# kmurf1999/RustSolver

Hardware: NVIDIA B200
Metric: cfr_iterations_per_sec (higher is better)
Workload: dtype f32

## Files before the change

### include/b200cfr.h

```cpp
#ifndef B200CFR_H
#define B200CFR_H

#include <stddef.h>
#include <stdint.h>

#ifdef __cplusplus
extern "C" {
#endif

#define RS_OK 0
#define RS_ERR_INVALID -1
#define RS_ERR_CUDA -2
#define RS_ERR_NCCL -3
#define RS_ERR_CAPACITY -4
#define RS_ERR_UNSUPPORTED -5

#define RS_NODE_ACTION 0
#define RS_NODE_TERMINAL 1
#define RS_NODE_PUBLIC_CHANCE 2
#define RS_NODE_PRIVATE_CHANCE 3
#define RS_TERM_ALLIN 0
#define RS_TERM_SHOWDOWN 1
#define RS_TERM_UNCONTESTED 2
#define RS_ROUND_FLOP 0
#define RS_ROUND_TURN 1
#define RS_ROUND_RIVER 2

typedef struct rs_tree {
    uint32_t n_nodes;
    const uint8_t* type;
    const int32_t* parent;
    const uint32_t* child_offset;
    const uint32_t* children;
    const uint8_t* player;
    const uint32_t* an_index;
    const uint8_t* round_idx;
    const uint32_t* value;
    const uint8_t* ttype;
    const uint8_t* last_to_act;
} rs_tree;

typedef struct rs_ranges {
    uint32_t n_hands[2];
    const uint8_t* hands[2];
} rs_ranges;

#define RS_ABS_NONE 0
#define RS_ABS_ISOMORPHIC 1
#define RS_ABS_CLUSTER_ARR 2
#define RS_ABS_BUCKET_TABLE 3
typedef struct rs_round_abstraction {
    uint32_t kind;
    const uint32_t* cluster_arr;
    uint64_t cluster_arr_len;
    const uint32_t* bucket_table[2];
} rs_round_abstraction;
typedef struct rs_abstraction {
    uint32_t n_rounds;
    rs_round_abstraction rounds[3];
} rs_abstraction;

#define RS_NCCL_ID_BYTES 128
typedef struct rs_config {
    uint64_t board_mask;
    int32_t device;
    int32_t rank;
    int32_t world_size;
    uint8_t nccl_id[RS_NCCL_ID_BYTES];
    uint32_t flags;
    uint32_t threads_per_block;
    uint64_t discount_interval;
    uint64_t discount_cap;
} rs_config;
#define RS_FLAG_NO_GRAPH 1u
#define RS_FLAG_NO_CHAIN_SPLIT 2u
#define RS_FLAG_STREET_KERNEL 4u
#define RS_FLAG_SHARD_ISOLATED 8u
#define RS_FLAG_ALL (RS_FLAG_NO_GRAPH | RS_FLAG_NO_CHAIN_SPLIT | RS_FLAG_STREET_KERNEL | RS_FLAG_SHARD_ISOLATED)

typedef struct rs_engine rs_engine;

typedef struct rs_stats {
    uint64_t iterations;
    uint64_t updates_per_iteration;
    uint64_t updates_per_iteration_global;
    double device_ms;
    uint64_t kernel_launches;
    uint64_t table_bytes;
    uint32_t n_rounds;
    uint32_t n_boards[3];
    uint32_t n_boards_local[3];
    uint32_t n_hands[2];
    uint64_t n_combos;
} rs_stats;

const char* rs_last_error(void);
int rs_version(void);
int rs_device_count(void);
int rs_nccl_unique_id(uint8_t* out);

int rs_gpu_index_hands(uint32_t n_board_cards, const uint8_t* cards, size_t n, uint64_t* out, float* kernel_ms);

#define RS_DIST_EMD_1D 0u
#define RS_DIST_L2 1u
int rs_kmeans_assign(const float* points, size_t n, uint32_t dim, const float* centers, uint32_t k, uint32_t dist_kind,
                     uint32_t* cluster, float* min_dist, double* inertia, float* kernel_ms);
int rs_histogram_distances(const float* p, const float* q, size_t n, uint32_t dim, uint32_t dist_kind, float* out);
int rs_kmeans_fit_regular(const float* points, size_t n, uint32_t dim, float* centers, uint32_t k, uint32_t dist_kind,
                          uint32_t rounds, uint32_t* cluster, float* inertia);
int rs_generate_histograms(uint32_t round, uint64_t first_index, size_t count, uint32_t samples, uint32_t bins, uint64_t seed,
                           float* out, uint8_t* cards_out, float* kernel_ms);
int rs_kmeans_fit_growbatch(const float* points, size_t n, uint32_t dim, float* centers, uint32_t k, uint32_t dist_kind,
                            uint32_t initial_batch_size, uint64_t seed, uint32_t* batch_index_out, uint32_t* cluster_out,
                            float* stats_out);
int rs_kmeans_update_min_dists(const float* points, size_t n, uint32_t dim, const float* new_center, uint32_t dist_kind,
                               float* min_dists);
int rs_kmeans_init_pp(const float* points, size_t n, uint32_t dim, uint32_t k, uint32_t dist_kind, uint64_t seed, uint32_t* chosen_out,
                      float* centers_out);
int rs_kmeans_init_random(const float* points, size_t n, uint32_t dim, uint32_t k, uint32_t n_restarts, uint32_t dist_kind, uint64_t seed,
                          uint32_t* chosen_out, float* centers_out);

#define RS_EXCHANGE_HANDLE_BYTES 64
int rs_exchange_export(rs_engine* e, uint8_t* out );
int rs_exchange_import(rs_engine* e, const uint8_t* handles , uint32_t n_ranks);
int rs_exchange_disable(rs_engine* e);


int rs_create(const rs_tree* tree, const rs_ranges* ranges, const rs_abstraction* abs,
              const rs_config* cfg, rs_engine** out);
int rs_create_batch(const rs_tree* tree, const rs_ranges* ranges, const rs_abstraction* abs,
                    const rs_config* cfg, const uint64_t* board_masks, uint32_t n_subgames,
                    rs_engine** out);
void rs_destroy(rs_engine* e);

int rs_iterate(rs_engine* e, uint64_t n_iters);
int rs_iterate_sampled(rs_engine* e, const uint8_t* dealt, uint32_t n_paths);
int rs_sample_runouts(uint64_t seed, uint64_t board_mask, uint32_t n_cards, uint32_t n_paths, int distinct_first, uint8_t* dealt_out);
int rs_discount(rs_engine* e, float d);
int rs_set_wait_timeout_ms(rs_engine* e, uint64_t ms);
int rs_abort(rs_engine* e);
int rs_set_prune_threshold(rs_engine* e, float threshold);
#define RS_OPP_FULL 0u
#define RS_OPP_SAMPLE 1u
#define RS_OPP_SAMPLE_TIMES_SIGMA 2u
int rs_set_opponent_sampling(rs_engine* e, uint32_t mode, uint64_t seed);
#define RS_RULE_VANILLA 0u
#define RS_RULE_DCFR 1u
#define RS_RULE_LCFR 2u
#define RS_RULE_CFR_PLUS 3u
typedef struct rs_update_rule {
    uint32_t kind;
    float alpha, beta, gamma;
} rs_update_rule;
int rs_set_update_rule(rs_engine* e, const rs_update_rule* rule);
int rs_get_update_rule(rs_engine* e, rs_update_rule* out, uint64_t* t_out);
int rs_reset(rs_engine* e);

int rs_read_infoset(rs_engine* e, uint32_t an_index, uint32_t board_id, float* regrets,
                    float* strategy_sum, size_t cap_floats, uint32_t* n_rows_out,
                    uint32_t* n_actions_out);
int rs_write_infoset(rs_engine* e, uint32_t an_index, uint32_t board_id, const float* regrets,
                     const float* strategy_sum, size_t n_floats);
int rs_average_strategy(rs_engine* e, uint32_t an_index, uint32_t board_id, float* out,
                        size_t cap_floats, uint32_t* n_rows_out, uint32_t* n_actions_out);
int rs_current_strategy(rs_engine* e, uint32_t an_index, uint32_t board_id, float* out,
                        size_t cap_floats, uint32_t* n_rows_out, uint32_t* n_actions_out);
int rs_dump_average_strategy(rs_engine* e, const char* path, uint64_t* n_floats_out);

int rs_board_id(rs_engine* e, uint32_t round_idx, const uint8_t* dealt, uint32_t n_dealt,
                uint32_t* board_id_out);
int rs_card_table(rs_engine* e, uint32_t round_idx, uint32_t player, uint32_t board_id,
                  uint16_t* rows_out, size_t cap, uint32_t* n_rows_out);

int rs_best_response(rs_engine* e, double out[2]);
int rs_average_value(rs_engine* e, double out[2]);
int rs_root_values(rs_engine* e, uint32_t player, float* out, size_t cap);

int rs_stats_get(rs_engine* e, rs_stats* out);

int rs_set_range_weights(rs_engine* e, uint32_t player, const float* weights, size_t n);

#define RS_KERNEL_TRAVERSAL 0
#define RS_KERNEL_STREET 1
#define RS_KERNEL_ALLREDUCE 3
typedef struct rs_kernel_time {
    uint32_t kind;
    uint32_t phase;
    uint32_t traverser;
    uint32_t grid;
    float ms;
    uint64_t table_bytes;
    uint64_t vector_bytes;
} rs_kernel_time;
int rs_profile_iteration(rs_engine* e, rs_kernel_time* out, size_t cap, uint32_t* n_out);

int rs_debug_task_timing(rs_engine* e, unsigned long long* out32, int reset);

typedef struct rs_plan rs_plan;
int rs_plan_create(const rs_tree* tree, const rs_ranges* ranges, const rs_abstraction* abs,
                   const rs_config* cfg, const uint64_t* board_masks, uint32_t n_subgames,
                   rs_plan** out);
void rs_plan_destroy(rs_plan* p);
int rs_plan_stats(const rs_plan* p, rs_stats* out);
int rs_plan_board_id(const rs_plan* p, uint32_t round_idx, const uint8_t* dealt, uint32_t n_dealt,
                     uint32_t* board_id_out);
int rs_plan_card_table(const rs_plan* p, uint32_t round_idx, uint32_t player, uint32_t board_id,
                       uint16_t* rows_out, size_t cap, uint32_t* n_rows_out);
int rs_plan_infoset_offset(const rs_plan* p, uint32_t an_index, uint32_t board_id,
                           uint64_t* offset_out, uint32_t* n_rows_out, uint32_t* n_actions_out);
int rs_plan_showdown_order(const rs_plan* p, uint32_t player, uint32_t board_id,
                           uint16_t* order_out, uint32_t* class_out, size_t cap,
                           uint32_t* n_live_out);

int rs_plan_local_tables(const rs_plan* p, uint32_t round_idx, uint32_t player, uint32_t board_id, uint32_t* hrec_words_out,
                         uint16_t* cl_pos_out, uint16_t* slot_of_pos_out, uint32_t dims_out[2]);
int rs_plan_check_execution_order(const rs_plan* p, uint32_t traverser, int force_board_major, uint32_t* n_tickets_out,
                                  uint32_t* n_moved_out);
int rs_plan_street_info(const rs_plan* p, uint32_t traverser, uint32_t out[8]);
int rs_plan_street_program(const rs_plan* p, uint32_t traverser, uint32_t board_id, uint32_t* words_out, size_t cap,
                           uint32_t* n_words_out, uint32_t* hinfo_out, size_t hinfo_cap, uint32_t dims_out[4]);

#ifdef __cplusplus
}
#endif
#endif
```

### rustsolver_b200/_lib.py

```python
from __future__ import annotations

import ctypes as C
import os
from pathlib import Path

_HERE = Path(__file__).resolve().parent
LIB_PATH = Path(os.environ.get("RS_ENGINE_LIB", str(_HERE / "libb200cfr.so")))

u8p = C.POINTER(C.c_uint8)
u16p = C.POINTER(C.c_uint16)
u32p = C.POINTER(C.c_uint32)
u64p = C.POINTER(C.c_uint64)
i32p = C.POINTER(C.c_int32)
f32p = C.POINTER(C.c_float)
f64p = C.POINTER(C.c_double)

RS_NCCL_ID_BYTES = 128
RS_EXCHANGE_HANDLE_BYTES = 64


class rs_tree(C.Structure):
    _fields_ = [("n_nodes", C.c_uint32), ("type", u8p), ("parent", i32p), ("child_offset", u32p),
                ("children", u32p), ("player", u8p), ("an_index", u32p), ("round_idx", u8p),
                ("value", u32p), ("ttype", u8p), ("last_to_act", u8p)]


class rs_ranges(C.Structure):
    _fields_ = [("n_hands", C.c_uint32 * 2), ("hands", u8p * 2)]


class rs_round_abstraction(C.Structure):
    _fields_ = [("kind", C.c_uint32), ("cluster_arr", u32p), ("cluster_arr_len", C.c_uint64),
                ("bucket_table", u32p * 2)]


class rs_abstraction(C.Structure):
    _fields_ = [("n_rounds", C.c_uint32), ("rounds", rs_round_abstraction * 3)]


class rs_config(C.Structure):
    _fields_ = [("board_mask", C.c_uint64), ("device", C.c_int32), ("rank", C.c_int32),
                ("world_size", C.c_int32), ("nccl_id", C.c_uint8 * RS_NCCL_ID_BYTES),
                ("flags", C.c_uint32), ("threads_per_block", C.c_uint32),
                ("discount_interval", C.c_uint64), ("discount_cap", C.c_uint64)]


class rs_stats(C.Structure):
    _fields_ = [("iterations", C.c_uint64), ("updates_per_iteration", C.c_uint64),
                ("updates_per_iteration_global", C.c_uint64), ("device_ms", C.c_double),
                ("kernel_launches", C.c_uint64), ("table_bytes", C.c_uint64), ("n_rounds", C.c_uint32),
                ("n_boards", C.c_uint32 * 3), ("n_boards_local", C.c_uint32 * 3),
                ("n_hands", C.c_uint32 * 2), ("n_combos", C.c_uint64)]


class rs_update_rule(C.Structure):
    _fields_ = [("kind", C.c_uint32), ("alpha", C.c_float), ("beta", C.c_float), ("gamma", C.c_float)]


class rs_kernel_time(C.Structure):
    _fields_ = [("kind", C.c_uint32), ("phase", C.c_uint32), ("traverser", C.c_uint32), ("grid", C.c_uint32),
                ("ms", C.c_float), ("table_bytes", C.c_uint64), ("vector_bytes", C.c_uint64)]


VP = C.c_void_p
ENGINE_API = {
    "rs_last_error": (C.c_char_p, []),
    "rs_version": (C.c_int, []),
    "rs_device_count": (C.c_int, []),
    "rs_nccl_unique_id": (C.c_int, [u8p]),
    "rs_kmeans_assign": (C.c_int, [f32p, C.c_size_t, C.c_uint32, f32p, C.c_uint32, C.c_uint32, u32p, f32p, f64p, f32p]),
    "rs_kmeans_fit_regular": (C.c_int, [f32p, C.c_size_t, C.c_uint32, f32p, C.c_uint32, C.c_uint32, C.c_uint32, u32p, f32p]),
    "rs_histogram_distances": (C.c_int, [f32p, f32p, C.c_size_t, C.c_uint32, C.c_uint32, f32p]),
    "rs_kmeans_update_min_dists": (C.c_int, [f32p, C.c_size_t, C.c_uint32, f32p, C.c_uint32, f32p]),
    "rs_kmeans_init_pp": (C.c_int, [f32p, C.c_size_t, C.c_uint32, C.c_uint32, C.c_uint32, C.c_uint64, u32p, f32p]),
    "rs_generate_histograms": (C.c_int, [C.c_uint32, C.c_uint64, C.c_size_t, C.c_uint32, C.c_uint32, C.c_uint64, f32p, u8p, f32p]),
    "rs_kmeans_fit_growbatch": (C.c_int, [f32p, C.c_size_t, C.c_uint32, f32p, C.c_uint32, C.c_uint32, C.c_uint32, C.c_uint64, u32p, u32p, f32p]),
    "rs_kmeans_init_random": (C.c_int, [f32p, C.c_size_t, C.c_uint32, C.c_uint32, C.c_uint32, C.c_uint32, C.c_uint64, u32p, f32p]),
    "rs_gpu_index_hands": (C.c_int, [C.c_uint32, u8p, C.c_size_t, u64p, f32p]),
    "rs_exchange_export": (C.c_int, [VP, u8p]),
    "rs_exchange_import": (C.c_int, [VP, u8p, C.c_uint32]),
    "rs_exchange_disable": (C.c_int, [VP]),
    "rs_create": (C.c_int, [C.POINTER(rs_tree), C.POINTER(rs_ranges), C.POINTER(rs_abstraction),
                            C.POINTER(rs_config), C.POINTER(VP)]),
    "rs_create_batch": (C.c_int, [C.POINTER(rs_tree), C.POINTER(rs_ranges), C.POINTER(rs_abstraction),
                                  C.POINTER(rs_config), u64p, C.c_uint32, C.POINTER(VP)]),
    "rs_destroy": (None, [VP]),
    "rs_iterate": (C.c_int, [VP, C.c_uint64]),
    "rs_iterate_sampled": (C.c_int, [VP, u8p, C.c_uint32]),
    "rs_discount": (C.c_int, [VP, C.c_float]),
    "rs_set_prune_threshold": (C.c_int, [VP, C.c_float]),
    "rs_set_opponent_sampling": (C.c_int, [VP, C.c_uint32, C.c_uint64]),
    "rs_set_wait_timeout_ms": (C.c_int, [VP, C.c_uint64]),
    "rs_abort": (C.c_int, [VP]),
    "rs_sample_runouts": (C.c_int, [C.c_uint64, C.c_uint64, C.c_uint32, C.c_uint32, C.c_int, u8p]),
    "rs_set_update_rule": (C.c_int, [VP, C.POINTER(rs_update_rule)]),
    "rs_get_update_rule": (C.c_int, [VP, C.POINTER(rs_update_rule), u64p]),
    "rs_reset": (C.c_int, [VP]),
    "rs_read_infoset": (C.c_int, [VP, C.c_uint32, C.c_uint32, f32p, f32p, C.c_size_t, u32p, u32p]),
    "rs_write_infoset": (C.c_int, [VP, C.c_uint32, C.c_uint32, f32p, f32p, C.c_size_t]),
    "rs_average_strategy": (C.c_int, [VP, C.c_uint32, C.c_uint32, f32p, C.c_size_t, u32p, u32p]),
    "rs_dump_average_strategy": (C.c_int, [VP, C.c_char_p, u64p]),
    "rs_current_strategy": (C.c_int, [VP, C.c_uint32, C.c_uint32, f32p, C.c_size_t, u32p, u32p]),
    "rs_board_id": (C.c_int, [VP, C.c_uint32, u8p, C.c_uint32, u32p]),
    "rs_card_table": (C.c_int, [VP, C.c_uint32, C.c_uint32, C.c_uint32, u16p, C.c_size_t, u32p]),
    "rs_best_response": (C.c_int, [VP, f64p]),
    "rs_average_value": (C.c_int, [VP, f64p]),
    "rs_root_values": (C.c_int, [VP, C.c_uint32, f32p, C.c_size_t]),
    "rs_stats_get": (C.c_int, [VP, C.POINTER(rs_stats)]),
    "rs_set_range_weights": (C.c_int, [VP, C.c_uint32, f32p, C.c_size_t]),
    "rs_profile_iteration": (C.c_int, [VP, C.POINTER(rs_kernel_time), C.c_size_t, u32p]),
    "rs_debug_task_timing": (C.c_int, [VP, u64p, C.c_int]),
    "rs_plan_create": (C.c_int, [C.POINTER(rs_tree), C.POINTER(rs_ranges), C.POINTER(rs_abstraction),
                                 C.POINTER(rs_config), u64p, C.c_uint32, C.POINTER(VP)]),
    "rs_plan_destroy": (None, [VP]),
    "rs_plan_stats": (C.c_int, [VP, C.POINTER(rs_stats)]),
    "rs_plan_board_id": (C.c_int, [VP, C.c_uint32, u8p, C.c_uint32, u32p]),
    "rs_plan_card_table": (C.c_int, [VP, C.c_uint32, C.c_uint32, C.c_uint32, u16p, C.c_size_t, u32p]),
    "rs_plan_infoset_offset": (C.c_int, [VP, C.c_uint32, C.c_uint32, u64p, u32p, u32p]),
    "rs_plan_showdown_order": (C.c_int, [VP, C.c_uint32, C.c_uint32, u16p, u32p, C.c_size_t, u32p]),
    "rs_plan_local_tables": (C.c_int, [VP, C.c_uint32, C.c_uint32, C.c_uint32, u32p, u16p, u16p, u32p]),
    "rs_plan_check_execution_order": (C.c_int, [VP, C.c_uint32, C.c_int, u32p, u32p]),
    "rs_plan_street_info": (C.c_int, [VP, C.c_uint32, u32p]),
    "rs_plan_street_program": (C.c_int, [VP, C.c_uint32, C.c_uint32, u32p, C.c_size_t, u32p, u32p, C.c_size_t, u32p]),
}
HOST_API = {
    "rsh_options_default_flop": (VP, []),
    "rsh_options_new": (VP, [C.c_uint64, C.c_uint32, C.c_uint32, C.c_uint32]),
    "rsh_options_free": (None, [VP]),
    "rsh_options_set_sizes": (C.c_int, [VP, C.c_uint32, u32p, f64p, u32p, f64p]),
    "rsh_options_set_range": (C.c_int, [VP, C.c_uint32, C.c_char_p]),
    "rsh_options_set_range_hands": (C.c_int, [VP, C.c_uint32, u8p, C.c_uint32]),
    "rsh_options_board_mask": (C.c_uint64, [VP]),
    "rsh_options_range": (C.c_int, [VP, C.c_uint32, u8p, C.c_size_t]),
    "rsh_build_game_tree": (C.c_int, [VP, C.POINTER(VP)]),
    "rsh_tree_free": (None, [VP]),
    "rsh_tree_n_nodes": (C.c_uint32, [VP]),
    "rsh_tree_n_actions": (C.c_uint32, [VP]),
    "rsh_tree_n_edges": (C.c_uint32, [VP]),
    "rsh_tree_view": (C.c_int, [VP, C.POINTER(rs_tree)]),
    "rsh_tree_round": (u8p, [VP]),
    "rsh_tree_action_kind": (u8p, [VP]),
    "rsh_tree_action_amount": (f64p, [VP]),
    "rsh_evaluate": (C.c_uint32, [u8p, C.c_uint32]),
    "rsh_get_card_mask": (C.c_int, [C.c_char_p, u64p]),
    "rsh_range_from_string": (C.c_int, [C.c_char_p, C.c_uint64, u8p, C.c_size_t]),
    "rsh_indexer_new": (VP, [C.c_uint32, u8p]),
    "rsh_indexer_free": (None, [VP]),
    "rsh_indexer_size": (C.c_uint64, [VP, C.c_uint32]),
    "rsh_indexer_index": (C.c_uint64, [VP, u8p]),
    "rsh_indexer_index_many": (None, [VP, u8p, C.c_size_t, u64p]),
    "rsh_indexer_get_hand": (C.c_int, [VP, C.c_uint32, C.c_uint64, u8p]),
}

_lib = None


def load():
    global _lib
    if _lib is not None:
        return _lib
    if not LIB_PATH.exists():
        raise ImportError(
            f"{LIB_PATH} is missing: build it with `python -m rustsolver_b200.build` "
            "(there is no CPU/Python fallback for the engine)")
    if "RS_NCCL_LIB" not in os.environ:
        try:
            import importlib.util
            spec = importlib.util.find_spec("nvidia.nccl")
            if spec and spec.submodule_search_locations:
                cand = Path(list(spec.submodule_search_locations)[0]) / "lib" / "libnccl.so.2"
                if cand.exists():
                    os.environ["RS_NCCL_LIB"] = str(cand)
        except Exception:
            pass
    lib = C.CDLL(str(LIB_PATH))
    for table in (ENGINE_API, HOST_API):
        for name, (res, args) in table.items():
            fn = getattr(lib, name)
            fn.restype = res
            fn.argtypes = args
    _lib = lib
    return lib


class EngineError(RuntimeError):
    def __init__(self, code: int, msg: str):
        super().__init__(f"b200cfr error {code}: {msg}")
        self.code = code


def check(rc: int):
    if rc != 0:
        raise EngineError(rc, load().rs_last_error().decode())
```

### rustsolver_b200/csrc/engine.cu

```cuda
#include <cuda_runtime.h>
#include <dlfcn.h>

#include <cmath>
#include <cstdio>
#include <cstdlib>
#include <cstring>
#include <map>
#include <memory>
#include <string>
#include <vector>

#include "../../include/b200cfr.h"
#include <cmath>

#include "abstraction_kernels.h"
#include "histogram_kernel.h"
#include "indexer_kernel.h"
#include "kernels.cuh"
#include "plan.h"
#include "street_kernel.cuh"

namespace rs {

thread_local std::string g_last_error;

static int set_err(int code, const std::string& msg) {
    g_last_error = msg;
    return code;
}

namespace nccl {
typedef struct {
    char internal[128];
} UniqueId;
typedef void* Comm;
typedef int (*GetUniqueId_t)(UniqueId*);
typedef int (*CommInitRank_t)(Comm*, int, UniqueId, int);
typedef int (*AllReduce_t)(const void*, void*, size_t, int, int, Comm, cudaStream_t);
typedef int (*CommDestroy_t)(Comm);
typedef const char* (*GetErrorString_t)(int);
struct Api {
    void* lib = nullptr;
    GetUniqueId_t GetUniqueId = nullptr;
    CommInitRank_t CommInitRank = nullptr;
    AllReduce_t AllReduce = nullptr;
    CommDestroy_t CommDestroy = nullptr;
    GetErrorString_t GetErrorString = nullptr;
};
static Api g_api;
constexpr int kFloat32 = 7;
constexpr int kSum = 0;

static bool load(std::string* err) {
    if (g_api.lib) return true;
    const char* env = getenv("RS_NCCL_LIB");
    const char* names[] = {env, "libnccl.so.2", "libnccl.so"};
    void* lib = nullptr;
    for (const char* n : names) {
        if (!n || !*n) continue;
        lib = dlopen(n, RTLD_NOW | RTLD_GLOBAL);
        if (lib) break;
    }
    if (!lib) {
        *err = "cannot dlopen libnccl.so.2 (set RS_NCCL_LIB to its path)";
        return false;
    }
    g_api.lib = lib;
    g_api.GetUniqueId = (GetUniqueId_t)dlsym(lib, "ncclGetUniqueId");
    g_api.CommInitRank = (CommInitRank_t)dlsym(lib, "ncclCommInitRank");
    g_api.AllReduce = (AllReduce_t)dlsym(lib, "ncclAllReduce");
    g_api.CommDestroy = (CommDestroy_t)dlsym(lib, "ncclCommDestroy");
    g_api.GetErrorString = (GetErrorString_t)dlsym(lib, "ncclGetErrorString");
    if (!g_api.GetUniqueId || !g_api.CommInitRank || !g_api.AllReduce || !g_api.CommDestroy) {
        *err = "libnccl is missing expected symbols";
        g_api = Api();
        return false;
    }
    return true;
}
}

#define CU(call)                                                                                   \
    do {                                                                                           \
        cudaError_t e__ = (call);                                                                  \
        if (e__ != cudaSuccess)                                                                    \
            return set_err(RS_ERR_CUDA, std::string(#call) + ": " + cudaGetErrorString(e__));      \
    } while (0)

static bool device_batch_index(const HandIndexer& ix, const uint8_t* cards, size_t n, uint64_t* out, std::string* err) {
    return gpu_index_hands(ix, ix.rounds() - 1, cards, n, out, nullptr, err);
}

template <class T>
struct DevBuf {
    T* p = nullptr;
    size_t n = 0;
    ~DevBuf() {
        if (p) cudaFree(p);
    }
    cudaError_t alloc(size_t count) {
        n = count;
        if (count == 0) count = 1;
        return cudaMalloc(&p, count * sizeof(T));
    }
    cudaError_t upload(const T* src, size_t count) {
        cudaError_t e = alloc(count);
        if (e != cudaSuccess || count == 0) return e;
        return cudaMemcpy(p, src, count * sizeof(T), cudaMemcpyHostToDevice);
    }
    cudaError_t upload(const std::vector<T>& v) { return upload(v.data(), v.size()); }
    cudaError_t zero() { return cudaMemset(p, 0, (n ? n : 1) * sizeof(T)); }
};

struct RoundDev {
    DevBuf<uint16_t> row_of_pos[2], row_start[2], row_pos[2], cl_pos[2], parent_pos[2], child_pos[2], slot_of_pos[2];
    DevBuf<HandRec> hrec[2];
    DevBuf<uint32_t> n_rows[2], n_rows_pad[2], n_live[2];
    DevBuf<uint64_t> board_off[2];
    DevBuf<float> regrets[2], ssum[2];
    DevBuf<float> chance_scale;
    DevBuf<int32_t> parent_board;
    DevBuf<float> rbuf, cbuf, gathered;
    DevBuf<float> sbuf[2];
    uint32_t n_leaves = 0, n_boards = 0;
};

struct TaskSet {
    DevBuf<NodeTask> tasks;
    DevBuf<TaskSrc> srcs;
    DevBuf<uint32_t> tix;
    DevBuf<uint32_t> order;
    uint32_t n_tickets = 0, phase_cut = 0, n_tasks = 0;
    uint32_t street_lo = 0, street_hi = 0;
    uint32_t street_inst = 0;
    struct Run {
        uint32_t t0, t1;
        int threads;
    };
    std::vector<Run> runs;
    uint32_t xch_lo = 0, xch_hi = 0;
    struct Section {
        uint32_t first;
        uint32_t round_k;
        bool up;
    };
    std::vector<Section> sections;
};

struct StreetDev {
    DevBuf<SwSeg> segs;
    DevBuf<SwDown> downs;
    DevBuf<SwUp> ups;
    DevBuf<SwTerm> terms;
    DevBuf<uint32_t> prog, prog_off, l_steps, c_steps, hinfo;
    uint32_t n_segs = 0;
};

struct Engine {
    Plan plan;
    int device = 0;
    int threads = 512;
    cudaStream_t stream = nullptr;
    cudaEvent_t ev0 = nullptr, ev1 = nullptr;
    cudaGraph_t graph = nullptr;
    cudaGraphExec_t graph_exec = nullptr;
    bool use_graph = true;
    nccl::Comm comm = nullptr;
    bool isolated = false;

    RoundDev rd[3];
    DevBuf<float> scratch;
    DevBuf<float> root_weights[2];
    TaskSet full[2];
    std::map<int, std::unique_ptr<TaskSet[]>> sampled_sets;
    DevBuf<int32_t> sample_board[3];
    int sample_cap = 0;
    DevBuf<uint32_t> flags;
    DevBuf<TaskCtl> ctl;
    DevBuf<unsigned long long> timing;
    DevBuf<unsigned char> xch;
    size_t xch_flag_bytes = 0, xch_vectors = 0;
    void* xch_peer_base[RS_MAX_PEERS] = {nullptr};
    bool fused_exchange = false;
    float prune_threshold = -INFINITY;
    int xs_mode = 0;
    uint64_t xs_seed = 0, xs_count = 0;
    uint32_t* abort_host = nullptr;
    uint32_t* abort_dev = nullptr;
    uint64_t wait_timeout_ms = 30000;
    bool aborted = false;
    int check_abort(const char* what);
    int maybe_discount();
    rs_update_rule rule = {RS_RULE_VANILLA, 1.5f, 0.f, 2.f};
    uint64_t rule_t = 0;
    bool rule_on() const { return rule.kind != RS_RULE_VANILLA; }
    int advance_rule();
    uint64_t last_discount_period = 0;
    bool street_on = false;
    StreetDev street[2];
    DevBuf<float> st_scratch;
    size_t st_stride = 0, st_smem = 0;
    int st_XP = 0, st_rows = 0, st_vy_rows = 0, st_vm_rows = 0, st_slots = 0, st_threads = 0, st_blocks_per_sm = 1, st_qs = 1, st_qm = 1;
    int slots = 1;
    size_t smem_bytes = 0;
    size_t smem_small = 0;
    int blocks_per_sm = 1, n_sms = 148;
    int round_threads[3] = {0, 0, 0};
    int bps_small = 0;
    bool wide_for(int thr, uint64_t tickets) const {
        return thr > 288 || bps_small == 0 || getenv("RS_WIDE_ONLY") || (tickets <= uint64_t(n_sms) * blocks_per_sm && !getenv("RS_SMALL_ONLY"));
    }
    std::vector<rs_kernel_time>* prof = nullptr;
    std::vector<std::pair<cudaEvent_t, cudaEvent_t>> prof_events;

    uint64_t iterations = 0;
    double device_ms = 0;
    uint64_t launches = 0;
    uint64_t launches_per_iter = 0;
    uint64_t table_bytes = 0;
    uint64_t updates_global = 0;
    uint64_t discount_interval = 0, discount_cap = 0;

    void close_peers() {
        for (int r = 0; r < RS_MAX_PEERS; ++r) {
            if (xch_peer_base[r] && r != plan.rank) cudaIpcCloseMemHandle(xch_peer_base[r]);
            xch_peer_base[r] = nullptr;
        }
    }

    ~Engine() {
        close_peers();
        if (graph_exec) cudaGraphExecDestroy(graph_exec);
        if (graph) cudaGraphDestroy(graph);
        if (comm && nccl::g_api.CommDestroy) nccl::g_api.CommDestroy(comm);
        if (abort_host) cudaFreeHost(abort_host);
        if (root_stage) cudaFreeHost(root_stage);
        if (ev0) cudaEventDestroy(ev0);
        if (ev1) cudaEventDestroy(ev1);
        if (stream) cudaStreamDestroy(stream);
    }

    int init(const rs_config* cfg);
    void fill_args(TaskArgs* a, int trav, const TaskSet& set) const;
    int materialize(int trav, const uint32_t counts[3], TaskSet* out);
    int enqueue_sampled(int n_paths, int n_paths_global, uint64_t* count);
    int enqueue_traversal(int trav, int mode, uint64_t* count, const TaskSet* set = nullptr, int n_paths = -1, int n_paths_global = 0);
    int init_street();
    int enqueue_street(int trav, int mode, const TaskSet& set, int n_paths);
    int enqueue_iteration(uint64_t* count);
    int iterate(uint64_t n);
    int root_sum(int player, double* out);
    int root_values(int player, std::vector<float>* out);
    int root_values_into(int player, float* dst);
    DevBuf<float> root_out;
    float* root_stage = nullptr;
    size_t root_stage_n = 0;
    int prof_begin();
    int prof_end(uint32_t kind, uint32_t k, int trav, uint32_t grid, uint64_t table_bytes, uint64_t vector_bytes);
};

template <class T>
static std::vector<T> slice(const std::vector<T>& v, size_t lo, size_t hi, size_t stride) {
    if (v.empty()) return {};
    return std::vector<T>(v.begin() + lo * stride, v.begin() + hi * stride);
}

int Engine::init(const rs_config* cfg) {
    int ndev = 0;
    cudaError_t e = cudaGetDeviceCount(&ndev);
    if (e != cudaSuccess || ndev == 0)
        return set_err(RS_ERR_CUDA, std::string("no CUDA device available (the engine has no CPU fallback): ") +
                                        (e != cudaSuccess ? cudaGetErrorString(e) : "device count is 0"));
    device = cfg->device;
    if (device < 0 || device >= ndev) return set_err(RS_ERR_INVALID, "device ordinal out of range");
    CU(cudaSetDevice(device));
    cudaDeviceProp prop;
    CU(cudaGetDeviceProperties(&prop, device));
    if (prop.major < 10) return set_err(RS_ERR_UNSUPPORTED, "kernels are built for sm_100a only; found an older device");
    if (cfg->threads_per_block)
        return set_err(RS_ERR_INVALID, "threads_per_block is derived from the range size (4 hands per thread) and cannot be set");
    if (cfg->flags & ~uint32_t(RS_FLAG_ALL)) return set_err(RS_ERR_INVALID, "unknown bits in rs_config.flags");
    use_graph = !(cfg->flags & RS_FLAG_NO_GRAPH);
    isolated = (cfg->flags & RS_FLAG_SHARD_ISOLATED) != 0;
    discount_interval = cfg->discount_interval;
    discount_cap = cfg->discount_cap;
    CU(cudaStreamCreateWithFlags(&stream, cudaStreamNonBlocking));
    CU(cudaEventCreate(&ev0));
    CU(cudaEventCreate(&ev1));

    const Plan& P = plan;
    for (int q = 0; q < 2; ++q) {
        std::vector<float> ones(P.H[q], 1.0f);
        CU(root_weights[q].upload(ones));
    }
    const int HP[2] = {int((P.H[0] + 3) & ~3u), int((P.H[1] + 3) & ~3u)};
    const size_t maxHP = size_t(std::max(HP[0], HP[1]));
    const bool street_wanted = P.street[0].eligible && P.street[1].eligible;
    threads = int(((maxHP / 4) + 31) / 32 * 32);
    if (threads > MAX_TASK_THREADS) return set_err(RS_ERR_UNSUPPORTED, "range larger than 1326 hands");
    for (uint32_t k = 0; k < P.n_rounds; ++k) {
        round_threads[k] = threads;
        if (!P.board_mask[k].empty() && !getenv("RS_UNIFORM_BLOCK")) {
            const int left = 52 - __builtin_popcountll(P.board_mask[k][0]);
            const size_t live_max = std::min<size_t>(maxHP, size_t(left) * size_t(left - 1) / 2);
            round_threads[k] = std::min(threads, int((((live_max + 3) / 4) + 31) / 32 * 32));
        }
    }
    n_sms = prop.multiProcessorCount;
    if (street_wanted) {
        int rc = init_street();
        if (rc != RS_OK) return rc;
    }
    for (uint32_t k = 0; k < P.n_rounds; ++k) {
        RoundDev& R = rd[k];
        const uint32_t lo = P.local_lo[k], hi = P.local_hi[k], nb = hi - lo;
        R.n_boards = nb;
        R.n_leaves = (k + 1 < P.n_rounds) ? uint32_t(P.segs[k + 1].size()) : 0;
        for (int q = 0; q < 2; ++q) {
            const RoundPlayerTables& T = P.tabs[k][q];
            const LocalTables& L = P.loc[k][q];
            const size_t hp = L.Hpad;
            CU(R.row_of_pos[q].upload(slice(L.row_of_pos, lo, hi, hp)));
            CU(R.row_start[q].upload(slice(L.row_start, lo, hi, hp + 4)));
            CU(R.row_pos[q].upload(slice(L.row_pos, lo, hi, hp)));
            CU(R.cl_pos[q].upload(slice(L.cl_pos, lo, hi, 2 * hp)));
            CU(R.slot_of_pos[q].upload(slice(L.slot_of_pos, lo, hi, hp)));
            {
                std::vector<HandRec> aos = slice(L.hrec, lo, hi, hp);
                std::vector<HandRec> soa(aos.size());
                const uint32_t* src = reinterpret_cast<const uint32_t*>(aos.data());
                uint32_t* dst = reinterpret_cast<uint32_t*>(soa.data());
                for (size_t b = 0; b < size_t(nb); ++b)
                    for (size_t i = 0; i < hp; ++i)
                        for (int wd = 0; wd < 4; ++wd) dst[(b * 4 + wd) * hp + i] = src[(b * hp + i) * 4 + wd];
                CU(R.hrec[q].upload(soa));
            }
            if (k > 0) {
                CU(R.parent_pos[q].upload(slice(L.parent_pos, lo, hi, hp)));
                CU(R.child_pos[q].upload(slice(L.child_pos, lo, hi, size_t(P.loc[k - 1][q].Hpad))));
            }
            CU(R.n_rows[q].upload(slice(T.n_rows, lo, hi, 1)));
            CU(R.n_rows_pad[q].upload(slice(L.n_rows_pad, lo, hi, 1)));
            CU(R.n_live[q].upload(slice(L.n_live, lo, hi, 1)));
            CU(R.board_off[q].upload(slice(T.board_off, lo, hi, 1)));
            const size_t cells = size_t(T.board_off[P.n_boards[k]]);
            CU(R.regrets[q].alloc(cells));
            CU(R.ssum[q].alloc(cells));
            CU(R.regrets[q].zero());
            CU(R.ssum[q].zero());
            table_bytes += 2 * cells * sizeof(float);
        }
        CU(R.chance_scale.upload(slice(P.chance_scale[k], lo, hi, 1)));
        std::vector<int32_t> pb(nb, -1);
        if (k > 0)
            for (uint32_t b = 0; b < nb; ++b) pb[b] = P.board_parent[k][lo + b] - int32_t(P.local_lo[k - 1]);
        CU(R.parent_board.upload(pb));
        const bool fused_round = street_on && k + 1 == P.n_rounds;
        const size_t n_r = fused_round ? 0 : std::max(P.tl[0].n_rbuf[k], P.tl[1].n_rbuf[k]);
        const size_t n_c = (fused_round && k > 0) ? 0 : std::max(P.tl[0].n_cbuf[k], P.tl[1].n_cbuf[k]);
        CU(R.rbuf.alloc(n_r * nb * maxHP));
        CU(R.cbuf.alloc(n_c * nb * maxHP));
        CU(R.gathered.alloc(size_t(R.n_leaves) * nb * maxHP));
        for (int p = 0; p < 2; ++p) {
            CU(R.sbuf[p].alloc(size_t(P.tl[p].n_sbuf[k]) * nb * maxHP));
            CU(R.sbuf[p].zero());
        }
        CU(R.rbuf.zero());
        CU(R.cbuf.zero());
        CU(R.gathered.zero());
    }
    uint32_t max_tickets = 0;
    for (int p = 0; p < 2; ++p) {
        uint32_t counts[3] = {0, 0, 0};
        for (uint32_t k = 0; k < P.n_rounds; ++k) counts[k] = rd[k].n_boards;
        int rc = materialize(p, counts, &full[p]);
        if (rc != RS_OK) return rc;
        max_tickets = std::max(max_tickets, full[p].n_tickets);
        slots = std::max(slots, int(std::max(P.tl[p].max_terminal, 1 + P.tl[p].max_children)));
    }
    CU(timing.alloc(96));
    CU(timing.zero());
    CU(flags.alloc(max_tickets));
    CU(flags.zero());
    {
        TaskCtl c0{};
        c0.ticket = 0;
        c0.exited = 0;
        c0.xch_seq = 1;
        c0.epoch = 1;
        c0.rule[0] = c0.rule[1] = c0.rule[2] = 1.f;
        c0.rule[3] = -INFINITY;
        CU(ctl.upload(&c0, 1));
        CU(cudaHostAlloc(reinterpret_cast<void**>(&abort_host), sizeof(uint32_t), cudaHostAllocMapped));
        *abort_host = 0;
        CU(cudaHostGetDevicePointer(reinterpret_cast<void**>(&abort_dev), abort_host, 0));
    }
    size_t smem_need = std::max(task_kernel_smem_bytes(true, slots, HP[0], HP[1]), task_kernel_smem_bytes(true, slots, HP[1], HP[0]));
    int max_optin = 0;
    CU(cudaDeviceGetAttribute(&max_optin, cudaDevAttrMaxSharedMemoryPerBlockOptin, device));
    if (smem_need > size_t(max_optin))
        return set_err(RS_ERR_UNSUPPORTED, "node too wide for one CTA's shared memory: need " +
                                               std::to_string(smem_need) + " B, device allows " + std::to_string(max_optin));
    smem_bytes = smem_need;
    CU(configure_task_kernels(smem_need, threads, true, &blocks_per_sm));
    if (blocks_per_sm < 1) return set_err(RS_ERR_UNSUPPORTED, "task kernel does not fit on an SM");
    for (uint32_t k = 0; k < P.n_rounds; ++k)
        if (round_threads[k] <= 288 && bps_small == 0) {
            smem_small = std::max(task_kernel_smem_bytes(false, slots, HP[0], HP[1]), task_kernel_smem_bytes(false, slots, HP[1], HP[0]));
            CU(configure_task_kernels(smem_small, 288, false, &bps_small));
            if (bps_small < 1) return set_err(RS_ERR_UNSUPPORTED, "task kernel does not fit on an SM");
        }
    n_sms = prop.multiProcessorCount;
    CU(scratch.alloc(size_t(1326) * MAX_ACTIONS));

    updates_global = P.updates_per_iter_local;
    if (P.world > 1 && !isolated) {
        std::string err;
        if (!nccl::load(&err)) return set_err(RS_ERR_NCCL, err);
        nccl::UniqueId id;
        static_assert(sizeof(id) == RS_NCCL_ID_BYTES, "nccl id size");
        memcpy(&id, cfg->nccl_id, sizeof(id));
        int rc = nccl::g_api.CommInitRank(&comm, P.world, id, P.rank);
        if (rc != 0)
            return set_err(RS_ERR_NCCL, std::string("ncclCommInitRank: ") +
                                            (nccl::g_api.GetErrorString ? nccl::g_api.GetErrorString(rc) : "error"));
        DevBuf<float> tmp;
        CU(tmp.alloc(4));
        uint64_t u = P.updates_per_iter_local;
        if (P.rank > 0)
            for (uint32_t k = 0; k < P.shard_round; ++k)
                for (int q = 0; q < 2; ++q) u -= P.tabs[k][q].board_off[P.n_boards[k]];
        float parts[4] = {float(u & 0xFFFFF), float((u >> 20) & 0xFFFFF), float((u >> 40) & 0xFFFFF), 0.f};
        CU(cudaMemcpy(tmp.p, parts, sizeof(parts), cudaMemcpyHostToDevice));
        rc = nccl::g_api.AllReduce(tmp.p, tmp.p, 4, nccl::kFloat32, nccl::kSum, comm, stream);
        if (rc != 0) return set_err(RS_ERR_NCCL, "ncclAllReduce failed");
        CU(cudaStreamSynchronize(stream));
        CU(cudaMemcpy(parts, tmp.p, sizeof(parts), cudaMemcpyDeviceToHost));
        updates_global = uint64_t(parts[0]) + (uint64_t(parts[1]) << 20) + (uint64_t(parts[2]) << 40);
    }
    if (P.world > 1 && P.shard_round >= 1 && !isolated) {
        const RoundDev& Par = rd[P.shard_round - 1];
        xch_vectors = size_t(Par.n_leaves) * Par.n_boards * size_t(P.world);
        xch_flag_bytes = (2 * xch_vectors * sizeof(uint32_t) + 255) & ~size_t(255);
        CU(xch.alloc(xch_flag_bytes + 2 * xch_vectors * maxHP * sizeof(float)));
        CU(xch.zero());
    }
    CU(cudaDeviceSynchronize());
    return RS_OK;
}


int Engine::init_street() {
    const Plan& P = plan;
    uint32_t max_rows = 1, max_slots = 1, max_q_sd = 1, max_q_mo = 1;
    for (int p = 0; p < 2; ++p) {
        const StreetPlan& S = P.street[p];
        StreetDev& D = street[p];
        CU(D.segs.upload(S.segs));
        CU(D.downs.upload(S.downs));
        CU(D.ups.upload(S.ups));
        CU(D.terms.upload(S.terms));
        CU(D.prog.upload(S.prog));
        CU(D.prog_off.upload(S.prog_off));
        CU(D.l_steps.upload(S.l_steps));
        CU(D.c_steps.upload(S.c_steps));
        CU(D.hinfo.upload(S.hinfo));
        D.n_segs = uint32_t(S.segs.size());
        max_rows = std::max(max_rows, S.max_rows);
        max_slots = std::max(max_slots, S.max_slots);
        max_q_sd = std::max(max_q_sd, S.max_q_sd);
        max_q_mo = std::max(max_q_mo, S.max_q_mo);
    }
    const int HP[2] = {int((P.H[0] + 3) & ~3u), int((P.H[1] + 3) & ~3u)};
    const int HPmax = std::max(HP[0], HP[1]);
    st_XP = (HPmax + 31) & ~31;
    st_rows = int(max_rows);
    st_vy_rows = 4 * int(max_q_sd);
    st_vm_rows = 4 * int(max_q_sd + max_q_mo);
    st_slots = int(max_slots);
    st_stride = size_t(st_rows) * st_XP + size_t(st_vy_rows + st_vm_rows + st_slots) * HPmax;
    st_threads = threads;
    if (const char* e = getenv("RS_STREET_THREADS")) st_threads = std::max(64, std::min(352, atoi(e) / 32 * 32));
    size_t budget = 72 * 1024;
    if (const char* e = getenv("RS_STREET_SMEM_KB")) budget = size_t(std::max(16, atoi(e))) * 1024;
    st_qs = st_qm = 1;
    const int max_q = st_threads / 32;
    while (st_qs < int(max_q_sd) && st_qs < max_q && street_smem_bytes(st_qs + 1, st_qm, HPmax, HPmax) <= budget) ++st_qs;
    while (st_qm < int(max_q_mo) && st_qm < max_q && street_smem_bytes(st_qs, st_qm + 1, HPmax, HPmax) <= budget) ++st_qm;
    st_smem = street_smem_bytes(st_qs, st_qm, HPmax, HPmax);
    int max_optin = 0;
    CU(cudaDeviceGetAttribute(&max_optin, cudaDevAttrMaxSharedMemoryPerBlockOptin, device));
    if (st_smem > size_t(max_optin)) return RS_OK;
    CU(configure_street_kernels(st_smem, st_threads, &st_blocks_per_sm));
    if (st_blocks_per_sm < 1) return RS_OK;
    if (const char* e = getenv("RS_STREET_BLOCKS")) st_blocks_per_sm = std::max(1, std::min(st_blocks_per_sm, atoi(e)));
    CU(st_scratch.alloc(st_stride * size_t(n_sms) * st_blocks_per_sm));
    CU(st_scratch.zero());
    street_on = true;
    return RS_OK;
}

int Engine::enqueue_street(int trav, int mode, const TaskSet& set, int n_paths) {
    const Plan& P = plan;
    const uint32_t k = P.n_rounds - 1;
    const RoundDev& R = rd[k];
    const StreetDev& D = street[trav];
    StreetArgs a;
    memset(&a, 0, sizeof(a));
    for (int q = 0; q < 2; ++q) {
        DevRoundPlayer& d = a.rp[q];
        d.row_of_pos = R.row_of_pos[q].p;
        d.row_start = R.row_start[q].p;
        d.row_pos = R.row_pos[q].p;
        d.cl_pos = R.cl_pos[q].p;
        d.parent_pos = R.parent_pos[q].p;
        d.child_pos = R.child_pos[q].p;
        d.slot_of_pos = R.slot_of_pos[q].p;
        d.hrec = R.hrec[q].p;
        d.n_rows = R.n_rows[q].p;
        d.n_rows_pad = R.n_rows_pad[q].p;
        d.n_live = R.n_live[q].p;
        d.board_off = R.board_off[q].p;
        d.regrets = R.regrets[q].p;
        d.ssum = R.ssum[q].p;
        d.identity = 1;
    }
    a.chance_scale = R.chance_scale.p;
    a.parent_board = R.parent_board.p;
    a.parent_rbuf = k > 0 ? rd[k - 1].rbuf.p : nullptr;
    a.parent_n_boards = k > 0 ? int(rd[k - 1].n_boards) : 0;
    a.n_boards = int(R.n_boards);
    a.root_weights = root_weights[1 - trav].p;
    a.out_buf = k > 0 ? R.sbuf[trav].p : R.cbuf.p;
    a.out_scatter = k > 0 ? 1 : 0;
    a.n_segs = int(D.n_segs);
    a.segs = D.segs.p;
    a.downs = D.downs.p;
    a.ups = D.ups.p;
    a.terms = D.terms.p;
    a.prog = D.prog.p;
    a.prog_off = D.prog_off.p;
    a.l_steps = D.l_steps.p;
    a.c_steps = D.c_steps.p;
    a.hinfo = D.hinfo.p;
    a.scratch = st_scratch.p;
    a.scratch_stride = st_stride;
    a.XP = st_XP;
    a.max_rows = st_rows;
    a.vy_rows = st_vy_rows;
    a.vm_rows = st_vm_rows;
    a.max_slots = st_slots;
    a.qs = st_qs;
    a.qm = st_qm;
    a.trav = trav;
    a.HpP = int((P.H[trav] + 3) & ~3u);
    a.HoP = int((P.H[1 - trav] + 3) & ~3u);
    a.n_units = set.street_inst * D.n_segs;
    a.sample_board = (n_paths >= 0 && k > 0) ? sample_board[k].p : nullptr;
    a.prune_threshold = prune_threshold;
    const int grid = int(std::min<uint64_t>(a.n_units, uint64_t(n_sms) * st_blocks_per_sm));
    CU(launch_street_kernel(a, mode, grid, st_threads, st_smem, stream));
    return RS_OK;
}

int Engine::materialize(int trav, const uint32_t counts[3], TaskSet* out) {
    MaterializedTasks mt;
    materialize_tasks(plan, trav, counts, &mt);
    std::vector<NodeTask>& t = mt.tasks;
    std::vector<TaskSrc>& sr = mt.srcs;
    const uint32_t first = mt.n_tickets;
    out->phase_cut = mt.phase_cut;
    out->n_tickets = first;
    out->n_tasks = uint32_t(t.size());
    out->street_lo = out->street_hi = 0;
    out->street_inst = counts[plan.n_rounds - 1];
    if (street_on) {
        bool seen = false, closed = false;
        for (const NodeTask& x : t) {
            const bool fin = uint32_t(x.round_k) + 1 == plan.n_rounds;
            if (fin && closed) return set_err(RS_ERR_INVALID, "internal: final-round tasks are not contiguous");
            if (fin && !seen) {
                seen = true;
                out->street_lo = x.first;
            }
            if (fin) out->street_hi = x.first + x.count;
            if (!fin && seen) closed = true;
        }
    }
    out->runs.clear();
    out->sections.clear();
    out->xch_lo = out->xch_hi = 0;
    for (const NodeTask& x : t) {
        if (x.count == 0) continue;
        if (x.kind == TK_GATHER && plan.world > 1 && plan.shard_round >= 1 && uint32_t(x.round_k) + 1 == plan.shard_round) {
            if (out->xch_hi == out->xch_lo) out->xch_lo = x.first;
            out->xch_hi = x.first + x.count;
        }
        const int thr = round_threads[x.round_k];
        if (out->runs.empty() || out->runs.back().threads != thr) out->runs.push_back({x.first, x.first + x.count, thr});
        else out->runs.back().t1 = x.first + x.count;
        const bool up = x.kind == TK_UP_TRAV, down = x.kind == TK_DOWN;
        if (up || down) {
            bool seen = false;
            for (const TaskSet::Section& sc : out->sections) seen |= (sc.round_k == x.round_k && sc.up == up);
            if (!seen) out->sections.push_back({x.first, uint32_t(x.round_k), up});
        }
    }
    std::vector<uint32_t> tix(first);
    for (size_t j = 0; j < t.size(); ++j)
        for (uint32_t i = 0; i < t[j].count; ++i) tix[t[j].first + i] = uint32_t(j);
    CU(out->tasks.upload(t));
    CU(out->srcs.upload(sr));
    CU(out->tix.upload(tix));
    if (!getenv("RS_TASK_MAJOR")) {
        std::vector<uint32_t> ord;
        std::string oerr;
        if (!build_execution_order(plan, trav, mt, counts, getenv("RS_BOARD_MAJOR") != nullptr, &ord, &oerr)) return set_err(RS_ERR_INVALID, oerr);
        if (!ord.empty()) CU(out->order.upload(ord));
    }
    return RS_OK;
}

void Engine::fill_args(TaskArgs* a, int trav, const TaskSet& set) const {
    const Plan& P = plan;
    memset(a, 0, sizeof(*a));
    for (int q = 0; q < 2; ++q) {
        a->H[q] = int(P.H[q]);
        a->Hpad[q] = int((P.H[q] + 3) & ~3u);
        a->root_weights[q] = root_weights[q].p;
    }
    for (uint32_t k = 0; k < P.n_rounds; ++k) {
        const RoundDev& R = rd[k];
        RoundArgs& ra = a->rounds[k];
        for (int q = 0; q < 2; ++q) {
            DevRoundPlayer& d = ra.rp[q];
            d.row_of_pos = R.row_of_pos[q].p;
            d.row_start = R.row_start[q].p;
            d.row_pos = R.row_pos[q].p;
            d.cl_pos = R.cl_pos[q].p;
            d.parent_pos = R.parent_pos[q].p;
            d.child_pos = R.child_pos[q].p;
            d.slot_of_pos = R.slot_of_pos[q].p;
            d.hrec = R.hrec[q].p;
            d.n_rows = R.n_rows[q].p;
            d.n_rows_pad = R.n_rows_pad[q].p;
            d.n_live = R.n_live[q].p;
            d.board_off = R.board_off[q].p;
            d.regrets = R.regrets[q].p;
            d.ssum = R.ssum[q].p;
            d.identity = P.loc[k][q].identity ? 1 : 0;
        }
        ra.chance_scale = R.chance_scale.p;
        ra.parent_board = R.parent_board.p;
        ra.rbuf = R.rbuf.p;
        ra.cbuf = R.cbuf.p;
        ra.sbuf = R.sbuf[trav].p;
        ra.gathered = R.gathered.p;
        ra.n_boards = int(R.n_boards);
        ra.board_base = int(P.local_lo[k]);
        if (k + 1 < P.n_rounds) {
            const bool sharded_next = (P.world > 1 && k + 1 == P.shard_round);
            ra.per_parent = sharded_next ? 0 : int(P.deal_count[k + 1]);
            ra.n_boards_next = int(rd[k + 1].n_boards);
        }
    }
    a->tasks = set.tasks.p;
    a->srcs = set.srcs.p;
    a->task_of_ticket = set.tix.p;
    a->order = set.order.n ? set.order.p : nullptr;
    a->n_tasks = set.n_tasks;
    a->flags = flags.p;
    a->ctl = ctl.p;
    a->trav = trav;
    a->HpP = a->Hpad[trav];
    a->HoP = a->Hpad[1 - trav];
    a->Hx = std::max(a->HpP, a->HoP);
    if (fused_exchange) {
        a->xch_world = P.world;
        a->xch_rank = P.rank;
        a->xch_round = int(P.shard_round);
        a->xch_leaves = int(rd[P.shard_round - 1].n_leaves);
        for (int r = 0; r < P.world; ++r) {
            a->xflag_peer[r] = reinterpret_cast<uint32_t*>(xch_peer_base[r]);
            a->xch_peer[r] = reinterpret_cast<float*>(static_cast<unsigned char*>(xch_peer_base[r]) + xch_flag_bytes);
        }
    }
    a->slots = slots;
    a->prune_threshold = prune_threshold;
    a->host_abort = abort_dev;
    a->wait_timeout_ns = wait_timeout_ms * 1000000ull;
    a->timing = timing.p;
}

int Engine::prof_begin() {
    if (!prof) return RS_OK;
    cudaEvent_t a, b;
    CU(cudaEventCreate(&a));
    CU(cudaEventCreate(&b));
    prof_events.emplace_back(a, b);
    CU(cudaEventRecord(a, stream));
    return RS_OK;
}

int Engine::prof_end(uint32_t kind, uint32_t phase, int trav, uint32_t grid, uint64_t tb, uint64_t vb) {
    if (!prof) return RS_OK;
    CU(cudaEventRecord(prof_events.back().second, stream));
    rs_kernel_time t;
    memset(&t, 0, sizeof(t));
    t.kind = kind;
    t.phase = phase;
    t.traverser = uint32_t(trav);
    t.grid = grid;
    t.table_bytes = tb;
    t.vector_bytes = vb;
    prof->push_back(t);
    return RS_OK;
}

int Engine::enqueue_traversal(int trav, int mode, uint64_t* count, const TaskSet* set, int n_paths, int n_paths_global) {
    const Plan& P = plan;
    const TaskList& tl = P.tl[trav];
    if (!set) set = &full[trav];
    TaskArgs a;
    fill_args(&a, trav, *set);
    if (n_paths >= 0) {
        a.n_paths = n_paths;
        for (uint32_t k = 1; k < P.n_rounds; ++k) {
            a.sample_board[k] = sample_board[k].p;
            a.gather_scale[k - 1] = float(P.deal_count[k]) / float(k == 1 ? n_paths_global : 1);
        }
    }
    if (mode == KM_CFR && xs_mode) {
        uint64_t z = xs_seed + 0x9E3779B97F4A7C15ull * (++xs_count);
        z = (z ^ (z >> 30)) * 0xBF58476D1CE4E5B9ull;
        z = (z ^ (z >> 27)) * 0x94D049BB133111EBull;
        a.xs_key = z ^ (z >> 31);
        a.xs_mode = xs_mode;
        mode = KM_CFR_XS;
    }
    if (rule_on() && (mode == KM_CFR || mode == KM_CFR_XS)) mode = mode == KM_CFR ? KM_CFR_DR : KM_CFR_XS_DR;
    int rc;
    struct Step {
        int kind;
        uint32_t t0, t1, phase;
    };
    std::vector<Step> steps;
    const bool use_street = street_on && set->street_hi > set->street_lo;
    uint32_t at = 0;
    if (use_street) {
        if (set->street_lo > 0) steps.push_back({0, 0, set->street_lo, 0});
        steps.push_back({1, 0, 0, 0});
        at = set->street_hi;
    }
    const bool split = !fused_exchange && !isolated && set->phase_cut < set->n_tickets;
    const uint32_t cut = split ? std::max(set->phase_cut, at) : set->n_tickets;
    if (cut > at) steps.push_back({0, at, cut, use_street ? 1u : 0u});
    if (split) {
        steps.push_back({2, 0, 0, 0});
        steps.push_back({0, cut, set->n_tickets, 2});
    }
    uint64_t vec = 0;
    for (uint32_t k = 0; k < P.n_rounds; ++k)
        vec += (uint64_t(tl.n_rbuf[k]) * P.H[1 - trav] + uint64_t(tl.n_cbuf[k]) * P.H[trav]) * rd[k].n_boards * 8;
    for (const Step& sp : steps) {
        if ((rc = prof_begin()) != RS_OK) return rc;
        if (sp.kind == 0) {
            struct Piece {
                uint32_t t0, t1;
                int threads;
            };
            std::vector<Piece> pieces;
            for (const TaskSet::Run& r : set->runs) {
                const uint32_t lo = std::max(sp.t0, r.t0), hi = std::min(sp.t1, r.t1);
                if (lo < hi) pieces.push_back({lo, hi, r.threads});
            }
            size_t longest = 0;
            for (size_t i = 1; i < pieces.size(); ++i)
                if (pieces[i].t1 - pieces[i].t0 > pieces[longest].t1 - pieces[longest].t0) longest = i;
            for (size_t i = 0; i < pieces.size(); ++i) {
                if (i > 0 && (rc = prof_begin()) != RS_OK) return rc;
                a.t0 = pieces[i].t0;
                a.t1 = pieces[i].t1;
                a.xch_bump = (fused_exchange && set->xch_lo < set->xch_hi && a.t0 <= set->xch_lo && set->xch_lo < a.t1) ? 1 : 0;
                const int thr = pieces[i].threads;
                const bool wide = wide_for(thr, a.t1 - a.t0);
                const int grid = int(std::min<uint64_t>(uint64_t(a.t1 - a.t0), uint64_t(n_sms) * (wide ? blocks_per_sm : bps_small)));
                CU(launch_task_kernel(a, mode, grid, thr, wide, wide ? smem_bytes : smem_small, stream));
                uint64_t bytes = 0;
                for (const TaskSet::Section& sc : set->sections)
                    if (sc.first >= a.t0 && sc.first < a.t1) {
                        const uint64_t own = P.tabs[sc.round_k][trav].board_off[P.n_boards[sc.round_k]];
                        const uint64_t opp = P.tabs[sc.round_k][1 - trav].board_off[P.n_boards[sc.round_k]];
                        bytes += sc.up ? own * 16 : opp * 4;
                    }
                if ((rc = prof_end(RS_KERNEL_TRAVERSAL, sp.phase + (i == longest ? 0u : 8u), trav, uint32_t(grid), bytes, i == longest ? vec : 0)) != RS_OK)
                    return rc;
                if (i + 1 < pieces.size()) ++*count;
            }
        } else if (sp.kind == 1) {
            if ((rc = enqueue_street(trav, mode, *set, n_paths)) != RS_OK) return rc;
            const uint32_t k = P.n_rounds - 1;
            const uint64_t own = P.tabs[k][trav].board_off[P.n_boards[k]], opp = P.tabs[k][1 - trav].board_off[P.n_boards[k]];
            const uint32_t grid = uint32_t(std::min<uint64_t>(uint64_t(set->street_inst) * street[trav].n_segs, uint64_t(n_sms) * st_blocks_per_sm));
            if ((rc = prof_end(RS_KERNEL_STREET, 0, trav, grid, own * 16 + opp * 4, 0)) != RS_OK) return rc;
        } else {
            RoundDev& Par = rd[P.shard_round - 1];
            const size_t n = size_t(Par.n_leaves) * Par.n_boards * ((P.H[trav] + 3) & ~3u);
            int nrc = nccl::g_api.AllReduce(Par.gathered.p, Par.gathered.p, n, nccl::kFloat32, nccl::kSum, comm, stream);
            if (nrc != 0) return set_err(RS_ERR_NCCL, "ncclAllReduce failed");
            if ((rc = prof_end(RS_KERNEL_ALLREDUCE, 0, trav, 0, 0, n * 4)) != RS_OK) return rc;
        }
        ++*count;
    }
    return RS_OK;
}

int Engine::enqueue_sampled(int n_paths, int n_paths_global, uint64_t* count) {
    auto it = sampled_sets.find(n_paths);
    if (it == sampled_sets.end()) {
        std::unique_ptr<TaskSet[]> sets(new TaskSet[2]);
        for (int p = 0; p < 2; ++p) {
            uint32_t counts[3] = {rd[0].n_boards, uint32_t(n_paths), uint32_t(n_paths)};
            int rc = materialize(p, counts, &sets[p]);
            if (rc != RS_OK) return rc;
        }
        it = sampled_sets.emplace(n_paths, std::move(sets)).first;
    }
    for (int p = 0; p < 2; ++p) {
        int rc = enqueue_traversal(p, KM_CFR, count, &it->second[p], n_paths, n_paths_global);
        if (rc != RS_OK) return rc;
    }
    return RS_OK;
}

int Engine::enqueue_iteration(uint64_t* count) {
    for (int p = 0; p < 2; ++p) {
        int rc = enqueue_traversal(p, KM_CFR, count);
        if (rc != RS_OK) return rc;
    }
    return RS_OK;
}

int Engine::iterate(uint64_t n) {
    CU(cudaSetDevice(device));
    if (n == 0) return RS_OK;
    if (aborted) return set_err(RS_ERR_CUDA, "an earlier traversal was aborted: the tables are partly updated, create a new engine");
    const bool use_graph = this->use_graph && !xs_mode;
    if (use_graph && !graph_exec) {
        uint64_t cnt = 0;
        CU(cudaStreamBeginCapture(stream, cudaStreamCaptureModeThreadLocal));
        int rc = enqueue_iteration(&cnt);
        cudaError_t e = cudaStreamEndCapture(stream, &graph);
        if (rc != RS_OK) return rc;
        if (e != cudaSuccess) return set_err(RS_ERR_CUDA, std::string("graph capture: ") + cudaGetErrorString(e));
        CU(cudaGraphInstantiate(&graph_exec, graph, 0));
        launches_per_iter = cnt;
    }
    CU(cudaEventRecord(ev0, stream));
    for (uint64_t i = 0; i < n; ++i) {
        {
            int rc = advance_rule();
            if (rc != RS_OK) return rc;
        }
        if (use_graph) {
            CU(cudaGraphLaunch(graph_exec, stream));
            launches += launches_per_iter;
        } else {
            uint64_t cnt = 0;
            int rc = enqueue_iteration(&cnt);
            if (rc != RS_OK) return rc;
            launches += cnt;
            launches_per_iter = cnt;
        }
        ++iterations;
        {
            int rc = maybe_discount();
            if (rc != RS_OK) return rc;
        }
    }
    CU(cudaEventRecord(ev1, stream));
    CU(cudaStreamSynchronize(stream));
    float ms = 0.f;
    CU(cudaEventElapsedTime(&ms, ev0, ev1));
    device_ms += ms;
    return check_abort("rs_iterate");
}

static void update_rule_factors(const rs_update_rule& r, uint64_t t, float f[4]) {
    f[0] = f[1] = f[2] = 1.f;
    f[3] = r.kind == RS_RULE_CFR_PLUS ? 0.f : -INFINITY;
    if (t <= 1) return;
    const double s = double(t - 1);
    if (r.kind == RS_RULE_DCFR || r.kind == RS_RULE_LCFR) {
        const bool lin = r.kind == RS_RULE_LCFR;
        const double a = lin ? 1.0 : double(r.alpha), b = lin ? 1.0 : double(r.beta), g = lin ? 1.0 : double(r.gamma);
        f[0] = float(1.0 / (1.0 + std::pow(s, -a)));
        f[1] = float(1.0 / (1.0 + std::pow(s, -b)));
        f[2] = float(std::pow(s / double(t), g));
    } else if (r.kind == RS_RULE_CFR_PLUS) {
        f[2] = float(s / double(t));
    }
}

int Engine::advance_rule() {
    if (!rule_on()) return RS_OK;
    float f[4];
    update_rule_factors(rule, ++rule_t, f);
    CU(launch_set_rule(ctl.p, f, stream));
    ++launches;
    return RS_OK;
}

int Engine::maybe_discount() {
    if (!discount_interval) return RS_OK;
    const uint64_t period = iterations / discount_interval;
    if (period == last_discount_period) return RS_OK;
    last_discount_period = period;
    if (discount_cap && iterations > discount_cap) return RS_OK;
    const float pf = float(period);
    const float d = pf / (pf + 1.0f);
    for (uint32_t k = 0; k < plan.n_rounds; ++k)
        for (int q = 0; q < 2; ++q) {
            CU(launch_scale(rd[k].regrets[q].p, rd[k].regrets[q].n, d, stream));
            CU(launch_scale(rd[k].ssum[q].p, rd[k].ssum[q].n, d, stream));
            launches += 2;
        }
    return RS_OK;
}

int Engine::check_abort(const char* what) {
    if (!fused_exchange && !(abort_host && *abort_host)) return RS_OK;
    TaskCtl c;
    CU(cudaMemcpy(&c, ctl.p, sizeof(c), cudaMemcpyDeviceToHost));
    if (!c.abort) return RS_OK;
    aborted = true;
    return set_err(RS_ERR_CUDA, std::string(what) + ": the traversal kernel gave up waiting (" +
                                    ((abort_host && *abort_host) ? "rs_abort was called" : "a wait exceeded the bound of " + std::to_string(wait_timeout_ms) +
                                                                                               " ms: a peer rank did not launch the same traversal") +
                                    "); the tables are partly updated, create a new engine");
}

int Engine::root_values_into(int player, float* dst) {
    const Plan& P = plan;
    const RoundDev& R = rd[0];
    const uint32_t hp = (P.H[player] + 3) & ~3u, H = P.H[player];
    const size_t n = size_t(R.n_boards) * H;
    if (root_out.n < n) CU(root_out.alloc(n));
    if (root_stage_n < n) {
        if (root_stage) cudaFreeHost(root_stage);
        root_stage = nullptr;
        CU(cudaHostAlloc(reinterpret_cast<void**>(&root_stage), n * sizeof(float), cudaHostAllocDefault));
        root_stage_n = n;
    }
    CU(cudaMemsetAsync(root_out.p, 0, n * sizeof(float), stream));
    CU(launch_unpermute(R.cbuf.p + size_t(P.tl[player].root_cbuf) * R.n_boards * hp, R.slot_of_pos[player].p, R.n_live[player].p, root_out.p,
                        R.n_boards, hp, H, stream));
// ... 434 lines not shown
        return z ^ (z >> 31);
    };
    const uint64_t zone = (~0ull / 52ull) * 52ull;
    auto card = [&]() {
        for (;;) {
            const uint64_t z = next();
            if (z < zone) return int(z % 52ull);
        }
    };
    uint64_t firsts = 0;
    for (uint32_t s = 0; s < n_paths; ++s) {
        uint64_t used = board_mask;
        for (uint32_t i = 0; i < n_cards;) {
            const int c = card();
            if (used & (1ull << c)) continue;
            if (i == 0 && distinct_first && (firsts & (1ull << c))) continue;
            if (i == 0) firsts |= 1ull << c;
            used |= 1ull << c;
            dealt_out[size_t(s) * n_cards + i] = uint8_t(c);
            ++i;
        }
    }
    return RS_OK;
}

int rs_discount(rs_engine* e, float d) {
    if (!e) return set_err(RS_ERR_INVALID, "null engine");
    Engine& E = e->e;
    CU(cudaSetDevice(E.device));
    for (uint32_t k = 0; k < E.plan.n_rounds; ++k)
        for (int q = 0; q < 2; ++q) {
            CU(launch_scale(E.rd[k].regrets[q].p, E.rd[k].regrets[q].n, d, E.stream));
            CU(launch_scale(E.rd[k].ssum[q].p, E.rd[k].ssum[q].n, d, E.stream));
        }
    CU(cudaStreamSynchronize(E.stream));
    return RS_OK;
}

int rs_set_update_rule(rs_engine* e, const rs_update_rule* rule) {
    if (!rule) return set_err(RS_ERR_INVALID, "null rule");
    if (rule->kind > RS_RULE_CFR_PLUS)
        return set_err(RS_ERR_INVALID, "kind must be RS_RULE_VANILLA (0), RS_RULE_DCFR (1), RS_RULE_LCFR (2) or RS_RULE_CFR_PLUS (3)");
    if (!std::isfinite(rule->alpha) || !std::isfinite(rule->beta) || !std::isfinite(rule->gamma))
        return set_err(RS_ERR_INVALID, "alpha, beta and gamma must be finite");
    if (!e) return set_err(RS_ERR_INVALID, "null engine");
    Engine& E = e->e;
    if (rule->kind != RS_RULE_VANILLA && E.street_on)
        return set_err(RS_ERR_UNSUPPORTED, "update rules other than RS_RULE_VANILLA are not available with RS_FLAG_STREET_KERNEL");
    CU(cudaSetDevice(E.device));
    CU(cudaStreamSynchronize(E.stream));
    const bool was_on = E.rule_on();
    E.rule = *rule;
    E.rule_t = 0;
    if (was_on != E.rule_on()) {
        if (E.graph_exec) {
            cudaGraphExecDestroy(E.graph_exec);
            E.graph_exec = nullptr;
        }
        if (E.graph) {
            cudaGraphDestroy(E.graph);
            E.graph = nullptr;
        }
    }
    return RS_OK;
}

int rs_get_update_rule(rs_engine* e, rs_update_rule* out, uint64_t* t_out) {
    if (!e) return set_err(RS_ERR_INVALID, "null engine");
    if (out) *out = e->e.rule;
    if (t_out) *t_out = e->e.rule_t;
    return RS_OK;
}

int rs_reset(rs_engine* e) {
    if (!e) return set_err(RS_ERR_INVALID, "null engine");
    Engine& E = e->e;
    CU(cudaSetDevice(E.device));
    for (uint32_t k = 0; k < E.plan.n_rounds; ++k)
        for (int q = 0; q < 2; ++q) {
            CU(E.rd[k].regrets[q].zero());
            CU(E.rd[k].ssum[q].zero());
        }
    E.iterations = 0;
    E.device_ms = 0;
    E.launches = 0;
    E.rule_t = 0;
    return RS_OK;
}

static int locate(const Plan& P, uint32_t an_index, uint32_t board_id, uint32_t* k_out, int* q_out, uint64_t* off,
                  uint32_t* n_rows, uint32_t* n_act) {
    if (an_index >= P.an_to_pnode.size() || P.an_to_pnode[an_index] < 0) return set_err(RS_ERR_INVALID, "unknown ActionNode.index");
    const PNode& n = P.nodes[P.an_to_pnode[an_index]];
    const uint32_t k = n.round_k;
    const int q = n.player;
    if (board_id >= P.n_boards[k]) return set_err(RS_ERR_INVALID, "board_id out of range for the node's round");
    if (board_id < P.local_lo[k] || board_id >= P.local_hi[k]) return set_err(RS_ERR_INVALID, "board is owned by another rank");
    const RoundPlayerTables& T = P.tabs[k][q];
    *k_out = k;
    *q_out = q;
    *n_rows = T.n_rows[board_id];
    *n_act = uint32_t(n.children.size());
    *off = T.board_off[board_id] + uint64_t(P.loc[k][q].n_rows_pad[board_id]) * n.cum_a;
    return RS_OK;
}

int rs_plan_infoset_offset(const rs_plan* p, uint32_t an_index, uint32_t board_id, uint64_t* offset_out,
                           uint32_t* n_rows_out, uint32_t* n_actions_out) {
    if (!p) return set_err(RS_ERR_INVALID, "null plan");
    uint32_t k, nr, na;
    int q;
    uint64_t off;
    int rc = locate(p->p, an_index, board_id, &k, &q, &off, &nr, &na);
    if (rc != RS_OK) return rc;
    if (offset_out) *offset_out = off;
    if (n_rows_out) *n_rows_out = nr;
    if (n_actions_out) *n_actions_out = na;
    return RS_OK;
}

int rs_read_infoset(rs_engine* e, uint32_t an_index, uint32_t board_id, float* regrets, float* strategy_sum,
                    size_t cap_floats, uint32_t* n_rows_out, uint32_t* n_actions_out) {
    if (!e) return set_err(RS_ERR_INVALID, "null engine");
    Engine& E = e->e;
    uint32_t k, nr, na;
    int q;
    uint64_t off;
    int rc = locate(E.plan, an_index, board_id, &k, &q, &off, &nr, &na);
    if (rc != RS_OK) return rc;
    if (n_rows_out) *n_rows_out = nr;
    if (n_actions_out) *n_actions_out = na;
    const size_t n = size_t(nr) * na;
    if ((regrets || strategy_sum) && cap_floats < n) return set_err(RS_ERR_CAPACITY, "output buffer too small");
    CU(cudaSetDevice(E.device));
    if (regrets) CU(cudaMemcpy(regrets, E.rd[k].regrets[q].p + off, n * sizeof(float), cudaMemcpyDeviceToHost));
    if (strategy_sum) CU(cudaMemcpy(strategy_sum, E.rd[k].ssum[q].p + off, n * sizeof(float), cudaMemcpyDeviceToHost));
    return RS_OK;
}

int rs_write_infoset(rs_engine* e, uint32_t an_index, uint32_t board_id, const float* regrets, const float* strategy_sum,
                     size_t n_floats) {
    if (!e) return set_err(RS_ERR_INVALID, "null engine");
    Engine& E = e->e;
    uint32_t k, nr, na;
    int q;
    uint64_t off;
    int rc = locate(E.plan, an_index, board_id, &k, &q, &off, &nr, &na);
    if (rc != RS_OK) return rc;
    const size_t n = size_t(nr) * na;
    if (n_floats != n) return set_err(RS_ERR_INVALID, "slab size mismatch");
    CU(cudaSetDevice(E.device));
    if (regrets) CU(cudaMemcpy(E.rd[k].regrets[q].p + off, regrets, n * sizeof(float), cudaMemcpyHostToDevice));
    if (strategy_sum) CU(cudaMemcpy(E.rd[k].ssum[q].p + off, strategy_sum, n * sizeof(float), cudaMemcpyHostToDevice));
    return RS_OK;
}

static int strategy_impl(rs_engine* e, uint32_t an_index, uint32_t board_id, float* out, size_t cap, uint32_t* n_rows_out,
                         uint32_t* n_actions_out, bool average) {
    if (!e) return set_err(RS_ERR_INVALID, "null engine");
    Engine& E = e->e;
    uint32_t k, nr, na;
    int q;
    uint64_t off;
    int rc = locate(E.plan, an_index, board_id, &k, &q, &off, &nr, &na);
    if (rc != RS_OK) return rc;
    if (n_rows_out) *n_rows_out = nr;
    if (n_actions_out) *n_actions_out = na;
    const size_t n = size_t(nr) * na;
    if (!out) return RS_OK;
    if (cap < n) return set_err(RS_ERR_CAPACITY, "output buffer too small");
    CU(cudaSetDevice(E.device));
    const float* src = (average ? E.rd[k].ssum[q].p : E.rd[k].regrets[q].p) + off;
    CU(launch_normalize(src, E.scratch.p, nr, na, E.stream));
    CU(cudaStreamSynchronize(E.stream));
    CU(cudaMemcpy(out, E.scratch.p, n * sizeof(float), cudaMemcpyDeviceToHost));
    return RS_OK;
}

int rs_average_strategy(rs_engine* e, uint32_t an_index, uint32_t board_id, float* out, size_t cap_floats,
                        uint32_t* n_rows_out, uint32_t* n_actions_out) {
    return strategy_impl(e, an_index, board_id, out, cap_floats, n_rows_out, n_actions_out, true);
}
int rs_current_strategy(rs_engine* e, uint32_t an_index, uint32_t board_id, float* out, size_t cap_floats,
                        uint32_t* n_rows_out, uint32_t* n_actions_out) {
    return strategy_impl(e, an_index, board_id, out, cap_floats, n_rows_out, n_actions_out, false);
}

int rs_dump_average_strategy(rs_engine* e, const char* path, uint64_t* n_floats_out) {
    if (!e || !path) return set_err(RS_ERR_INVALID, "null argument");
    Engine& E = e->e;
    const Plan& P = E.plan;
    FILE* f = fopen(path, "wb");
    if (!f) return set_err(RS_ERR_INVALID, std::string("cannot open ") + path);
    uint64_t total = 0;
    std::vector<float> buf;
    int rc = RS_OK;
    for (uint32_t an = 0; an < P.an_to_pnode.size() && rc == RS_OK; ++an) {
        if (P.an_to_pnode[an] < 0) continue;
        const uint32_t k = P.nodes[P.an_to_pnode[an]].round_k;
        for (uint32_t b = P.local_lo[k]; b < P.local_hi[k]; ++b) {
            uint32_t nr = 0, na = 0;
            if ((rc = strategy_impl(e, an, b, nullptr, 0, &nr, &na, true)) != RS_OK) break;
            buf.resize(size_t(nr) * na);
            if (buf.empty()) continue;
            if ((rc = strategy_impl(e, an, b, buf.data(), buf.size(), &nr, &na, true)) != RS_OK) break;
            if (fwrite(buf.data(), sizeof(float), buf.size(), f) != buf.size()) {
                rc = set_err(RS_ERR_INVALID, std::string("short write to ") + path);
                break;
            }
            total += buf.size();
        }
    }
    fclose(f);
    if (rc == RS_OK && n_floats_out) *n_floats_out = total;
    return rc;
}

static int board_id_impl(const Plan& P, uint32_t round_idx, const uint8_t* dealt, uint32_t n_dealt, uint32_t* out) {
    if (round_idx >= P.n_rounds) return set_err(RS_ERR_INVALID, "round_idx out of range");
    if (n_dealt != round_idx) return set_err(RS_ERR_INVALID, "need exactly round_idx dealt cards");
    if (P.n_sub != 1) return set_err(RS_ERR_UNSUPPORTED, "board lookup by dealt cards needs a single root board; batch boards are their own ids");
    uint32_t id = 0;
    uint64_t mask = P.board_mask[0][0];
    for (uint32_t k = 1; k <= round_idx; ++k) {
        const int c = dealt[k - 1];
        if (c >= 52 || (mask & (1ull << c))) return set_err(RS_ERR_INVALID, "dealt card already on the board");
        const uint32_t idx = uint32_t(__builtin_popcountll(~mask & ((1ull << c) - 1)));
        id = id * P.deal_count[k] + idx;
        mask |= 1ull << c;
    }
    *out = id;
    return RS_OK;
}

int rs_plan_board_id(const rs_plan* p, uint32_t round_idx, const uint8_t* dealt, uint32_t n_dealt, uint32_t* board_id_out) {
    if (!p || !board_id_out) return set_err(RS_ERR_INVALID, "null argument");
    return board_id_impl(p->p, round_idx, dealt, n_dealt, board_id_out);
}
int rs_board_id(rs_engine* e, uint32_t round_idx, const uint8_t* dealt, uint32_t n_dealt, uint32_t* board_id_out) {
    if (!e || !board_id_out) return set_err(RS_ERR_INVALID, "null argument");
    return board_id_impl(e->e.plan, round_idx, dealt, n_dealt, board_id_out);
}

static int card_table_impl(const Plan& P, uint32_t round_idx, uint32_t player, uint32_t board_id, uint16_t* rows_out,
                           size_t cap, uint32_t* n_rows_out) {
    if (round_idx >= P.n_rounds || player > 1) return set_err(RS_ERR_INVALID, "round/player out of range");
    if (board_id >= P.n_boards[round_idx]) return set_err(RS_ERR_INVALID, "board_id out of range");
    if (board_id < P.local_lo[round_idx] || board_id >= P.local_hi[round_idx])
        return set_err(RS_ERR_INVALID, "board is owned by another rank");
    const RoundPlayerTables& T = P.tabs[round_idx][player];
    const uint32_t H = P.H[player];
    if (n_rows_out) *n_rows_out = T.n_rows[board_id];
    if (rows_out) {
        if (cap < H) return set_err(RS_ERR_CAPACITY, "output buffer too small");
        memcpy(rows_out, &T.row_of_hand[size_t(board_id) * H], H * sizeof(uint16_t));
    }
    return RS_OK;
}
int rs_plan_card_table(const rs_plan* p, uint32_t round_idx, uint32_t player, uint32_t board_id, uint16_t* rows_out,
                       size_t cap, uint32_t* n_rows_out) {
    if (!p) return set_err(RS_ERR_INVALID, "null plan");
    return card_table_impl(p->p, round_idx, player, board_id, rows_out, cap, n_rows_out);
}
int rs_card_table(rs_engine* e, uint32_t round_idx, uint32_t player, uint32_t board_id, uint16_t* rows_out, size_t cap,
                  uint32_t* n_rows_out) {
    if (!e) return set_err(RS_ERR_INVALID, "null engine");
    return card_table_impl(e->e.plan, round_idx, player, board_id, rows_out, cap, n_rows_out);
}

int rs_plan_showdown_order(const rs_plan* p, uint32_t player, uint32_t board_id, uint16_t* order_out, uint32_t* class_out,
                           size_t cap, uint32_t* n_live_out) {
    if (!p || player > 1) return set_err(RS_ERR_INVALID, "bad argument");
    const Plan& P = p->p;
    const uint32_t k = P.n_rounds - 1;
    const ShowdownTables& S = P.sd[player];
    if (S.n_live.empty()) return set_err(RS_ERR_INVALID, "tree has no showdown terminals");
    if (board_id >= P.n_boards[k]) return set_err(RS_ERR_INVALID, "board_id out of range");
    const uint32_t H = P.H[player];
    const uint32_t nl = S.n_live[board_id];
    if (n_live_out) *n_live_out = nl;
    if (cap < nl) return set_err(RS_ERR_CAPACITY, "output buffer too small");
    for (uint32_t i = 0; i < nl; ++i) {
        if (order_out) order_out[i] = S.sorted[size_t(board_id) * H + i];
        if (class_out) class_out[i] = S.cls[size_t(board_id) * H + i];
    }
    return RS_OK;
}

int rs_plan_local_tables(const rs_plan* p, uint32_t round_idx, uint32_t player, uint32_t board_id, uint32_t* hrec_words_out, uint16_t* cl_pos_out,
                         uint16_t* slot_of_pos_out, uint32_t dims_out[2]) {
    if (!p || player > 1 || !dims_out) return set_err(RS_ERR_INVALID, "bad argument");
    const Plan& P = p->p;
    if (round_idx >= P.n_rounds || board_id >= P.n_boards[round_idx]) return set_err(RS_ERR_INVALID, "round or board out of range");
    if (board_id < P.local_lo[round_idx] || board_id >= P.local_hi[round_idx]) return set_err(RS_ERR_INVALID, "board belongs to another rank");
    const LocalTables& L = P.loc[round_idx][player];
    dims_out[0] = L.Hpad;
    dims_out[1] = L.n_live[board_id];
    if (hrec_words_out) memcpy(hrec_words_out, &L.hrec[size_t(board_id) * L.Hpad], size_t(L.Hpad) * sizeof(HandRec));
    if (cl_pos_out) memcpy(cl_pos_out, &L.cl_pos[size_t(board_id) * 2 * L.Hpad], size_t(2) * L.Hpad * sizeof(uint16_t));
    if (slot_of_pos_out) memcpy(slot_of_pos_out, &L.slot_of_pos[size_t(board_id) * L.Hpad], size_t(L.Hpad) * sizeof(uint16_t));
    return RS_OK;
}

int rs_plan_check_execution_order(const rs_plan* p, uint32_t traverser, int force_board_major, uint32_t* n_tickets_out, uint32_t* n_moved_out) {
    if (!p || traverser > 1) return set_err(RS_ERR_INVALID, "bad argument");
    const Plan& P = p->p;
    uint32_t counts[3] = {0, 0, 0};
    for (uint32_t k = 0; k < P.n_rounds; ++k) counts[k] = P.boards_local(k);
    MaterializedTasks mt;
    materialize_tasks(P, int(traverser), counts, &mt);
    std::vector<uint32_t> ord;
    std::string err;
    if (!build_execution_order(P, int(traverser), mt, counts, force_board_major > 0, &ord, &err)) return set_err(RS_ERR_INVALID, err);
    if (force_board_major < 0) {
        ord.resize(mt.n_tickets);
        for (uint32_t i = 0; i < mt.n_tickets; ++i) ord[i] = mt.n_tickets - 1 - i;
    }
    err = check_execution_order(P, int(traverser), mt, counts, ord);
    if (!err.empty()) return set_err(RS_ERR_INVALID, "execution order: " + err);
    if (n_tickets_out) *n_tickets_out = mt.n_tickets;
    if (n_moved_out) {
        uint32_t moved = 0;
        for (uint32_t i = 0; i < ord.size(); ++i) moved += ord[i] != i;
        *n_moved_out = moved;
    }
    return RS_OK;
}

int rs_plan_street_info(const rs_plan* p, uint32_t traverser, uint32_t out[8]) {
    if (!p || !out || traverser > 1) return set_err(RS_ERR_INVALID, "bad argument");
    const StreetPlan& S = p->p.street[traverser];
    out[0] = S.eligible ? 1u : 0u;
    out[1] = uint32_t(S.segs.size());
    out[2] = S.max_rows;
    out[3] = S.max_slots;
    out[4] = S.max_q_sd;
    out[5] = S.max_q_mo;
    out[6] = uint32_t(S.downs.size());
    out[7] = uint32_t(S.ups.size());
    if (!S.eligible) g_last_error = S.why;
    return RS_OK;
}

int rs_plan_street_program(const rs_plan* p, uint32_t traverser, uint32_t board_id, uint32_t* words_out, size_t cap,
                           uint32_t* n_words_out, uint32_t* hinfo_out, size_t hinfo_cap, uint32_t dims_out[4]) {
    if (!p || !n_words_out || !dims_out || traverser > 1) return set_err(RS_ERR_INVALID, "bad argument");
    const Plan& P = p->p;
    const StreetPlan& S = P.street[traverser];
    if (!S.eligible) return set_err(RS_ERR_INVALID, "the final round does not run on the street kernel: " + S.why);
    const uint32_t k = P.n_rounds - 1;
    if (board_id < P.local_lo[k] || board_id >= P.local_hi[k]) return set_err(RS_ERR_INVALID, "board is owned by another rank");
    const uint32_t lb = board_id - P.local_lo[k];
    const uint32_t n = S.prog_off[lb + 1] - S.prog_off[lb];
    const uint32_t HpP = P.loc[k][traverser].Hpad;
    *n_words_out = n;
    dims_out[0] = S.l_steps[lb];
    dims_out[1] = S.c_steps[lb];
    dims_out[2] = HpP;
    dims_out[3] = P.loc[k][1 - traverser].Hpad;
    if (words_out) {
        if (cap < n) return set_err(RS_ERR_CAPACITY, "output buffer too small");
        memcpy(words_out, S.prog.data() + S.prog_off[lb], size_t(n) * sizeof(uint32_t));
    }
    if (hinfo_out) {
        if (hinfo_cap < 2 * size_t(HpP)) return set_err(RS_ERR_CAPACITY, "hinfo buffer too small");
        memcpy(hinfo_out, S.hinfo.data() + size_t(lb) * HpP * 2, size_t(HpP) * 2 * sizeof(uint32_t));
    }
    return RS_OK;
}

static int score_impl(rs_engine* e, int mode, double out[2]) {
    if (!e || !out) return set_err(RS_ERR_INVALID, "null argument");
    Engine& E = e->e;
    if (E.aborted) return set_err(RS_ERR_CUDA, "an earlier traversal was aborted: create a new engine");
    CU(cudaSetDevice(E.device));
    for (int p = 0; p < 2; ++p) {
        uint64_t cnt = 0;
        int rc = E.enqueue_traversal(p, mode, &cnt);
        if (rc != RS_OK) return rc;
        CU(cudaStreamSynchronize(E.stream));
        if ((rc = E.check_abort(mode == KM_BR ? "rs_best_response" : "rs_average_value")) != RS_OK) return rc;
        double s = 0;
        rc = E.root_sum(p, &s);
        if (rc != RS_OK) return rc;
        out[p] = s;
    }
    return RS_OK;
}

int rs_best_response(rs_engine* e, double out[2]) { return score_impl(e, KM_BR, out); }
int rs_average_value(rs_engine* e, double out[2]) { return score_impl(e, KM_EVAL, out); }

int rs_root_values(rs_engine* e, uint32_t player, float* out, size_t cap) {
    if (!e || !out || player > 1) return set_err(RS_ERR_INVALID, "bad argument");
    Engine& E = e->e;
    const size_t n = size_t(E.rd[0].n_boards) * E.plan.H[player];
    if (cap < n) return set_err(RS_ERR_CAPACITY, "output buffer too small");
    CU(cudaSetDevice(E.device));
    return E.root_values_into(int(player), out);
}

int rs_set_range_weights(rs_engine* e, uint32_t player, const float* weights, size_t n) {
    if (!e || !weights || player > 1) return set_err(RS_ERR_INVALID, "bad argument");
    Engine& E = e->e;
    if (n != E.plan.H[player]) return set_err(RS_ERR_INVALID, "weights length must equal the range size");
    CU(cudaSetDevice(E.device));
    CU(cudaMemcpyAsync(E.root_weights[player].p, weights, n * sizeof(float), cudaMemcpyHostToDevice, E.stream));
    return RS_OK;
}

int rs_profile_iteration(rs_engine* e, rs_kernel_time* out, size_t cap, uint32_t* n_out) {
    if (!e || !n_out) return set_err(RS_ERR_INVALID, "null argument");
    Engine& E = e->e;
    CU(cudaSetDevice(E.device));
    std::vector<rs_kernel_time> rec;
    int rc = E.advance_rule();
    if (rc != RS_OK) return rc;
    E.prof = &rec;
    uint64_t cnt = 0;
    rc = E.enqueue_iteration(&cnt);
    E.prof = nullptr;
    cudaError_t se = cudaStreamSynchronize(E.stream);
    for (size_t i = 0; i < E.prof_events.size(); ++i) {
        if (rc == RS_OK && se == cudaSuccess && i < rec.size())
            cudaEventElapsedTime(&rec[i].ms, E.prof_events[i].first, E.prof_events[i].second);
        cudaEventDestroy(E.prof_events[i].first);
        cudaEventDestroy(E.prof_events[i].second);
    }
    E.prof_events.clear();
    if (rc != RS_OK) return rc;
    if (se != cudaSuccess) return set_err(RS_ERR_CUDA, cudaGetErrorString(se));
    E.iterations += 1;
    E.launches += cnt;
    *n_out = uint32_t(rec.size());
    if (out) {
        if (cap < rec.size()) return set_err(RS_ERR_CAPACITY, "output buffer too small");
        memcpy(out, rec.data(), rec.size() * sizeof(rs_kernel_time));
    }
    return RS_OK;
}

int rs_debug_task_timing(rs_engine* e, unsigned long long* out32, int reset) {
    if (!e || !out32) return set_err(RS_ERR_INVALID, "null argument");
    Engine& E = e->e;
    CU(cudaSetDevice(E.device));
    CU(cudaStreamSynchronize(E.stream));
    CU(cudaMemcpy(out32, E.timing.p, 96 * sizeof(unsigned long long), cudaMemcpyDeviceToHost));
    if (reset) {
        std::vector<unsigned long long> init(96, 0);
        for (int i = 0; i < 32; ++i) init[32 + 2 * i] = ~0ull;
        CU(cudaMemcpy(E.timing.p, init.data(), 96 * sizeof(unsigned long long), cudaMemcpyHostToDevice));
    }
    return RS_OK;
}

static void fill_stats(const Plan& P, rs_stats* s) {
    memset(s, 0, sizeof(*s));
    s->updates_per_iteration = P.updates_per_iter_local;
    s->updates_per_iteration_global = P.updates_per_iter_global;
    s->n_rounds = P.n_rounds;
    for (uint32_t k = 0; k < P.n_rounds; ++k) {
        s->n_boards[k] = P.n_boards[k];
        s->n_boards_local[k] = P.local_hi[k] - P.local_lo[k];
    }
    s->n_hands[0] = P.H[0];
    s->n_hands[1] = P.H[1];
    s->n_combos = P.n_combos.empty() ? 0 : P.n_combos[0];
}

int rs_plan_stats(const rs_plan* p, rs_stats* out) {
    if (!p || !out) return set_err(RS_ERR_INVALID, "null argument");
    fill_stats(p->p, out);
    return RS_OK;
}

int rs_stats_get(rs_engine* e, rs_stats* out) {
    if (!e || !out) return set_err(RS_ERR_INVALID, "null argument");
    fill_stats(e->e.plan, out);
    out->iterations = e->e.iterations;
    out->device_ms = e->e.device_ms;
    out->kernel_launches = e->e.launches;
    out->table_bytes = e->e.table_bytes;
    out->updates_per_iteration_global = e->e.updates_global;
    return RS_OK;
}

}
```

### rustsolver_b200/csrc/kernels.cu

```cuda
#include "kernels.cuh"

#ifndef RS_MIN_BLOCKS_288
#define RS_MIN_BLOCKS_288 3
#endif
#ifndef RS_MIN_BLOCKS_352
#define RS_MIN_BLOCKS_352 2
#endif

#ifndef RS_POLL_SLEEP_NS
#define RS_POLL_SLEEP_NS 64
#endif

namespace rs {

namespace {

__device__ __forceinline__ uint32_t ld_acquire_u32(const uint32_t* p) {
    uint32_t v;
    asm volatile("ld.acquire.gpu.global.u32 %0, [%1];" : "=r"(v) : "l"(p) : "memory");
    return v;
}
__device__ __forceinline__ uint32_t ld_acquire_sys_u32(const uint32_t* p) {
    uint32_t v;
    asm volatile("ld.acquire.sys.global.u32 %0, [%1];" : "=r"(v) : "l"(p) : "memory");
    return v;
}
__device__ __forceinline__ void st_release_sys_u32(uint32_t* p, uint32_t v) {
    asm volatile("st.release.sys.global.u32 [%0], %1;" ::"l"(p), "r"(v) : "memory");
}
__device__ __forceinline__ void st_release_u32(uint32_t* p, uint32_t v) {
    asm volatile("st.release.gpu.global.u32 [%0], %1;" ::"l"(p), "r"(v) : "memory");
}
__device__ __forceinline__ void prefetch_l2_bulk(const void* p, uint32_t bytes) {
    if (bytes) asm volatile("cp.async.bulk.prefetch.L2.global [%0], %1;" ::"l"(p), "r"(bytes) : "memory");
}
__device__ __forceinline__ float4 ldcg4(const float* p) { return __ldcg(reinterpret_cast<const float4*>(p)); }
__device__ __forceinline__ void stcg4(float* p, float4 v) { __stcg(reinterpret_cast<float4*>(p), v); }
__device__ __forceinline__ float4 f4zero() { return make_float4(0.f, 0.f, 0.f, 0.f); }
__device__ __forceinline__ float4 f4add(float4 a, float4 b) { return make_float4(a.x + b.x, a.y + b.y, a.z + b.z, a.w + b.w); }
__device__ __forceinline__ float f4get(const float4& v, int i) { return i == 0 ? v.x : (i == 1 ? v.y : (i == 2 ? v.z : v.w)); }
__device__ __forceinline__ void f4set(float4& v, int i, float x) {
    if (i == 0) v.x = x;
    else if (i == 1) v.y = x;
    else if (i == 2) v.z = x;
    else v.w = x;
}
__device__ __forceinline__ void unpack4(uint2 u, uint32_t (&o)[4]) {
    o[0] = u.x & 0xffffu;
    o[1] = u.x >> 16;
    o[2] = u.y & 0xffffu;
    o[3] = u.y >> 16;
}

__device__ __forceinline__ void csync(int n_compute) { asm volatile("bar.sync 2, %0;" ::"r"(n_compute) : "memory"); }
__device__ __forceinline__ void hsync(int n_all) { asm volatile("bar.sync 1, %0;" ::"r"(n_all) : "memory"); }

__device__ __forceinline__ void mbar_init(uint64_t* bar, uint32_t count) {
    asm volatile("mbarrier.init.shared::cta.b64 [%0], %1;" ::"r"(uint32_t(__cvta_generic_to_shared(bar))), "r"(count) : "memory");
}
__device__ __forceinline__ void mbar_arrive(uint64_t* bar) {
    asm volatile("mbarrier.arrive.release.cta.shared::cta.b64 _, [%0];" ::"r"(uint32_t(__cvta_generic_to_shared(bar))) : "memory");
}
__device__ __forceinline__ bool mbar_test(uint64_t* bar, uint32_t parity) {
    uint32_t ok;
    asm volatile(
        "{\n\t.reg .pred p;\n\tmbarrier.test_wait.parity.acquire.cta.shared::cta.b64 p, [%1], %2;\n\tselp.u32 %0, 1, 0, p;\n\t}"
        : "=r"(ok)
        : "r"(uint32_t(__cvta_generic_to_shared(bar))), "r"(parity)
        : "memory");
    return ok != 0;
}

__device__ __forceinline__ bool wait_gives_up(const TaskArgs& A, unsigned long long t_start, uint32_t& spins) {
    if ((++spins & 255u) != 0) return false;
    if (*reinterpret_cast<const volatile unsigned int*>(&A.ctl->abort)) return true;
    bool trip = false;
    if ((spins & 4095u) == 0 && A.host_abort && *A.host_abort) trip = true;
    if (A.wait_timeout_ns) {
        unsigned long long now;
        asm volatile("mov.u64 %0, %globaltimer;" : "=l"(now));
        if (now - t_start > A.wait_timeout_ns) trip = true;
    }
    if (trip) atomicExch(&A.ctl->abort, 1u);
    return trip;
}
__device__ __forceinline__ unsigned long long global_ns() {
    unsigned long long now;
    asm volatile("mov.u64 %0, %globaltimer;" : "=l"(now));
    return now;
}

struct Ctx {
    int nc;
    int tid, lane, warp, nwarps;
    int pos4;
    int p, o, Hp, Ho, HpP, HoP, Hx;
};

extern __shared__ __align__(16) float smem_raw[];
#define SM_RS (smem_raw)
#define SM_P (smem_raw + HC)
#define SM_GB (smem_raw + 2 * HC + 4)
#define SM_WSA (smem_raw + 4 * HC + 12)
#define SM_WSB (smem_raw + 4 * HC + 44)
#define SM_B (smem_raw + 4 * HC + 76)
#define SM_WSC (smem_raw + 4 * HC + 140)
#define SM_WSD (smem_raw + 4 * HC + 172)
#define SM_BF (smem_raw + 4 * HC + 204)
#define SM_REC (reinterpret_cast<uint32_t*>(smem_raw + 4 * HC + 268))
#define SM_CL (reinterpret_cast<uint32_t*>(smem_raw + 8 * HC + 268))
#define SM_X (smem_raw + 9 * HC + 268)
constexpr int smem_fixed_floats(int HC) { return 9 * HC + 268; }

template <int HC>
__device__ __forceinline__ void stage_lists_raw(int tid, int HoP, const uint16_t* __restrict__ cl_pos_b) {
    if (8 * tid < 2 * HoP)
        asm volatile("cp.async.cg.shared.global [%0], [%1], 16;" ::"r"(uint32_t(__cvta_generic_to_shared(SM_CL + 4 * tid))), "l"(cl_pos_b + 8 * tid)
                     : "memory");
    asm volatile("cp.async.commit_group;" ::: "memory");
}

template <int HC, bool FOLD>
__device__ __forceinline__ float scan_reach(const Ctx& c, const float* r, const float* rf = nullptr, float* total_f = nullptr) {
    csync(c.nc);
    const int hend = HC >= 4 * MAX_TASK_THREADS ? c.HoP : min(c.HoP, 4 * c.nc);
    float4 x = f4zero();
    float lc = 0.f;
    if (c.pos4 < c.HoP) {
        x = *reinterpret_cast<const float4*>(r + c.pos4);
        if (FOLD) {
            const float4 xf = *reinterpret_cast<const float4*>(rf + c.pos4);
            lc = (xf.x + xf.y) + (xf.z + xf.w);
        }
    }
    float y[8], yf[8];
    uint32_t w[4];
    {
        asm volatile("cp.async.wait_group 0;" ::: "memory");
        uint4 u = make_uint4(0x07ff07ffu, 0x07ff07ffu, 0x07ff07ffu, 0x07ff07ffu);
        if (8 * c.tid < 2 * c.HoP) u = *reinterpret_cast<const uint4*>(SM_CL + 4 * c.tid);
        w[0] = u.x;
        w[1] = u.y;
        w[2] = u.z;
        w[3] = u.w;
#pragma unroll
        for (int i = 0; i < 4; ++i) {
            const uint32_t a = w[i] & CL_POS_MASK, b = (w[i] >> 16) & CL_POS_MASK;
            y[2 * i] = a != CL_POS_NONE ? r[a] : 0.f;
            y[2 * i + 1] = b != CL_POS_NONE ? r[b] : 0.f;
            if (FOLD) {
                yf[2 * i] = a != CL_POS_NONE ? rf[a] : 0.f;
                yf[2 * i + 1] = b != CL_POS_NONE ? rf[b] : 0.f;
            }
        }
    }
    const float la = (x.x + x.y) + (x.z + x.w);
    float lb = 0.f, ld = 0.f;
#pragma unroll
    for (int i = 0; i < 8; ++i) {
        lb += y[i];
        if (FOLD) ld += yf[i];
    }
    float ia = la, ib = lb, ic = lc, id = ld;
#pragma unroll
    for (int d = 1; d < 32; d <<= 1) {
        const float ta = __shfl_up_sync(0xffffffffu, ia, d);
        const float tb = __shfl_up_sync(0xffffffffu, ib, d);
        float tc = 0.f, td = 0.f;
        if (FOLD) {
            tc = __shfl_up_sync(0xffffffffu, ic, d);
            td = __shfl_up_sync(0xffffffffu, id, d);
        }
        if (c.lane >= d) {
            ia += ta;
            ib += tb;
            if (FOLD) {
                ic += tc;
                id += td;
            }
        }
    }
    if (c.lane == 31) {
        SM_WSA[c.warp] = ia;
        SM_WSB[c.warp] = ib;
        if (FOLD) {
            SM_WSC[c.warp] = ic;
            SM_WSD[c.warp] = id;
        }
    }
    csync(c.nc);
    float wa = c.lane < c.nwarps ? SM_WSA[c.lane] : 0.f;
    float wb = c.lane < c.nwarps ? SM_WSB[c.lane] : 0.f;
    float wc = 0.f, wd = 0.f;
    if (FOLD) {
        wc = c.lane < c.nwarps ? SM_WSC[c.lane] : 0.f;
        wd = c.lane < c.nwarps ? SM_WSD[c.lane] : 0.f;
    }
#pragma unroll
    for (int d = 1; d < 16; d <<= 1) {
        const float ta = __shfl_up_sync(0xffffffffu, wa, d);
        const float tb = __shfl_up_sync(0xffffffffu, wb, d);
        float tc = 0.f, td = 0.f;
        if (FOLD) {
            tc = __shfl_up_sync(0xffffffffu, wc, d);
            td = __shfl_up_sync(0xffffffffu, wd, d);
        }
        if (c.lane >= d) {
            wa += ta;
            wb += tb;
            if (FOLD) {
                wc += tc;
                wd += td;
            }
        }
    }
    const float total = __shfl_sync(0xffffffffu, wa, c.nwarps - 1);
    const float total_b = __shfl_sync(0xffffffffu, wb, c.nwarps - 1);
    const float base_a = c.warp > 0 ? __shfl_sync(0xffffffffu, wa, c.warp - 1) : 0.f;
    const float base_b = c.warp > 0 ? __shfl_sync(0xffffffffu, wb, c.warp - 1) : 0.f;
    float ea = base_a + ia - la, eb = base_b + ib - lb;
    float total_d = 0.f, ed = 0.f;
    if (FOLD) {
        *total_f = __shfl_sync(0xffffffffu, wc, c.nwarps - 1);
        total_d = __shfl_sync(0xffffffffu, wd, c.nwarps - 1);
        const float base_d = c.warp > 0 ? __shfl_sync(0xffffffffu, wd, c.warp - 1) : 0.f;
        ed = base_d + id - ld;
    }
    if (c.pos4 < c.HoP) {
        float4 o;
        o.x = ea;
        o.y = ea + x.x;
        o.z = o.y + x.y;
        o.w = o.z + x.z;
        *reinterpret_cast<float4*>(SM_P + c.pos4) = o;
    }
    if (8 * c.tid < 2 * c.HoP) {
        float4 o0, o1;
        o0.x = eb;
        o0.y = o0.x + y[0];
        o0.z = o0.y + y[1];
        o0.w = o0.z + y[2];
        o1.x = o0.w + y[3];
        o1.y = o1.x + y[4];
        o1.z = o1.y + y[5];
        o1.w = o1.z + y[6];
        *reinterpret_cast<float4*>(SM_GB + 8 * c.tid) = o0;
        *reinterpret_cast<float4*>(SM_GB + 8 * c.tid + 4) = o1;
        const uint32_t ord0 = ((w[0] >> 11) & 7u) | (((w[0] >> 27) & 7u) << 3);
        const uint32_t b0 = c.tid == 0 ? 0u : ord0;
        float* bp = SM_B + b0;
        const float ex[8] = {o0.x, o0.y, o0.z, o0.w, o1.x, o1.y, o1.z, o1.w};
#pragma unroll
        for (int i = 0; i < 8; ++i) {
            const bool first = ((w[i >> 1] >> ((i & 1) * 16)) & CL_FIRST) != 0;
            if (first) *bp++ = ex[i];
        }
        if (c.tid == 0) SM_B[ord0] = total_b;
        if (FOLD) {
            float* bf = SM_BF + b0;
            float e = ed;
#pragma unroll
            for (int i = 0; i < 8; ++i) {
                const bool first = ((w[i >> 1] >> ((i & 1) * 16)) & CL_FIRST) != 0;
                if (first) *bf++ = e;
                e += yf[i];
            }
            if (c.tid == 0) SM_BF[ord0] = total_d;
        }
    }
    if (c.tid == 0) {
        SM_P[hend] = total;
        SM_GB[2 * hend] = total_b;
    }
    csync(c.nc);
    return total;
}

template <int HC>
__device__ __forceinline__ void stage_recs(const Ctx& c, const uint32_t* __restrict__ planes) {
    if (c.pos4 < c.HpP) {
#pragma unroll
        for (int w = 0; w < 4; ++w)
            asm volatile("cp.async.cg.shared.global [%0], [%1], 16;" ::"r"(uint32_t(__cvta_generic_to_shared(SM_REC + w * HC + c.pos4))),
                         "l"(planes + size_t(w) * c.HpP + c.pos4)
                         : "memory");
    }
    asm volatile("cp.async.commit_group;" ::: "memory");
}
__device__ __forceinline__ void staged_recs_wait() { asm volatile("cp.async.wait_group 0;" ::: "memory"); }
template <int HC>
__device__ __forceinline__ void staged_recs4(const Ctx& c, uint4 (&rec)[4]) {
    const uint4 w0 = *reinterpret_cast<const uint4*>(SM_REC + c.pos4);
    const uint4 w1 = *reinterpret_cast<const uint4*>(SM_REC + HC + c.pos4);
    const uint4 w2 = *reinterpret_cast<const uint4*>(SM_REC + 2 * HC + c.pos4);
    const uint4 w3 = *reinterpret_cast<const uint4*>(SM_REC + 3 * HC + c.pos4);
    rec[0] = make_uint4(w0.x, w1.x, w2.x, w3.x);
    rec[1] = make_uint4(w0.y, w1.y, w2.y, w3.y);
    rec[2] = make_uint4(w0.z, w1.z, w2.z, w3.z);
    rec[3] = make_uint4(w0.w, w1.w, w2.w, w3.w);
}

__device__ __forceinline__ float ldsb(const float* base, uint32_t byte_off) {
    return *reinterpret_cast<const float*>(reinterpret_cast<const char*>(base) + byte_off);
}
template <int HC>
__device__ __forceinline__ void hand_terms(const Ctx& c, const float* r, float total, const uint4& rec, float& mass, float& sd) {
    const uint32_t k0 = rec.w & 0x1ffu, k1 = (rec.w >> 9) & 0x1ffu, same4 = rec.w >> 18;
    const float g0s = ldsb(SM_B, k0), g0e = ldsb(SM_B + 1, k0), g1s = ldsb(SM_B, k1), g1e = ldsb(SM_B + 1, k1);
    mass = total - (g0e - g0s) - (g1e - g1s) + (same4 != HREC_SAME_NONE ? ldsb(r, same4) : 0.f);
    sd = ldsb(SM_P, rec.x & 0xffffu) + ldsb(SM_P, rec.x >> 16) - total - ldsb(SM_GB, rec.y & 0xffffu) - ldsb(SM_GB, rec.y >> 16) + g0s + g0e -
         ldsb(SM_GB, rec.z & 0xffffu) - ldsb(SM_GB, rec.z >> 16) + g1s + g1e;
}
__device__ __forceinline__ float hand_mass(const float* B, const float* r, float total, const uint4& rec) {
    const uint32_t k0 = rec.w & 0x1ffu, k1 = (rec.w >> 9) & 0x1ffu, same4 = rec.w >> 18;
    return total - (ldsb(B + 1, k0) - ldsb(B, k0)) - (ldsb(B + 1, k1) - ldsb(B, k1)) + (same4 != HREC_SAME_NONE ? ldsb(r, same4) : 0.f);
}

__device__ __forceinline__ float4 load_reach4(const TaskArgs& A, const Ctx& c, const NodeTask& nt, const RoundArgs& Rk, int k, int b) {
    float4 r = f4zero();
    if (c.pos4 >= c.HoP) return r;
    if (nt.r_in == RIN_INITIAL) {
        const uint32_t nl = Rk.rp[c.o].n_live[b];
        uint32_t s[4];
        unpack4(__ldg(reinterpret_cast<const uint2*>(Rk.rp[c.o].slot_of_pos + size_t(b) * c.HoP + c.pos4)), s);
        const float* __restrict__ w = A.root_weights[c.o];
#pragma unroll
        for (int i = 0; i < 4; ++i) f4set(r, i, uint32_t(c.pos4 + i) < nl ? __ldg(w + s[i]) : 0.f);
    } else if (nt.rin_parent_round) {
        const RoundArgs& Rp = A.rounds[k - 1];
        const float* src = Rp.rbuf + (size_t(nt.r_in) * Rp.n_boards + Rk.parent_board[b]) * c.HoP;
        uint32_t pp[4];
        unpack4(__ldg(reinterpret_cast<const uint2*>(Rk.rp[c.o].parent_pos + size_t(b) * c.HoP + c.pos4)), pp);
#pragma unroll
        for (int i = 0; i < 4; ++i) f4set(r, i, pp[i] != 0xffffu ? __ldcg(src + pp[i]) : 0.f);
    } else {
        r = ldcg4(Rk.rbuf + (size_t(nt.r_in) * Rk.n_boards + b) * c.HoP + c.pos4);
    }
    return r;
}

__device__ __forceinline__ float4 child_value4(const TaskArgs& A, const Ctx& c, const RoundArgs& Rk, const TaskChild& ch, int b) {
    float4 v = f4zero();
    if (c.pos4 >= c.HpP) return v;
    for (int s = 0; s < ch.n_src; ++s) {
        const TaskSrc sr = A.srcs[ch.src_first + s];
        const float* base = (sr.kind == SK_CBUF ? Rk.cbuf : Rk.gathered) + (size_t(sr.buf) * Rk.n_boards + b) * c.HpP;
        v = f4add(v, ldcg4(base + c.pos4));
    }
    return v;
}

__device__ __forceinline__ void store_value4(const Ctx& c, const NodeTask& nt, const RoundArgs& Rk, int b, float* out, float4 v) {
    if (!nt.root_scatter) {
        stcg4(out + c.pos4, v);
        return;
    }
    uint32_t pp[4];
    unpack4(__ldg(reinterpret_cast<const uint2*>(Rk.rp[c.p].parent_pos + size_t(b) * c.HpP + c.pos4)), pp);
    if (pp[0] != 0xffffu) __stcg(out + pp[0], v.x);
    if (pp[1] != 0xffffu) __stcg(out + pp[1], v.y);
    if (pp[2] != 0xffffu) __stcg(out + pp[2], v.z);
    if (pp[3] != 0xffffu) __stcg(out + pp[3], v.w);
}
__device__ __forceinline__ void store_value1(const Ctx& c, const NodeTask& nt, const RoundArgs& Rk, int b, float* out, int pos, float v) {
    if (!nt.root_scatter) {
        __stcg(out + pos, v);
        return;
    }
    const uint32_t pp = Rk.rp[c.p].parent_pos[size_t(b) * c.HpP + pos];
    if (pp != 0xffffu) __stcg(out + pp, v);
}

template <int NA>
__device__ __forceinline__ void sigma_row(const float (&g)[4 * NA], int i, float (&sg)[NA]) {
    float norm = 0.f;
#pragma unroll
    for (int a = 0; a < NA; ++a) {
        sg[a] = fmaxf(g[i * NA + a], 0.f);
        norm += sg[a];
    }
    const float inv = __fdividef(1.0f, norm);
#pragma unroll
    for (int a = 0; a < NA; ++a) sg[a] = norm > 0.f ? sg[a] * inv : 1.0f / float(NA);
}

template <int NA>
__device__ __forceinline__ void load_rows(const float* __restrict__ slab, bool identity, int pos4, uint32_t n_rows_pad,
                                          const uint32_t (&rows)[4], float (&g)[4 * NA]) {
    if (identity) {
        if (uint32_t(pos4) < n_rows_pad) {
#pragma unroll
            for (int v = 0; v < NA; ++v) {
                const float4 t = *reinterpret_cast<const float4*>(slab + size_t(pos4) * NA + 4 * v);
                g[4 * v] = t.x;
                g[4 * v + 1] = t.y;
                g[4 * v + 2] = t.z;
                g[4 * v + 3] = t.w;
            }
        } else {
#pragma unroll
            for (int e = 0; e < 4 * NA; ++e) g[e] = 0.f;
        }
    } else {
#pragma unroll
        for (int i = 0; i < 4; ++i)
#pragma unroll
            for (int a = 0; a < NA; ++a) g[i * NA + a] = rows[i] != 0xffffu ? slab[size_t(rows[i]) * NA + a] : 0.f;
    }
}

template <int NA>
__device__ __forceinline__ void xs_pick(const TaskArgs& A, float u, float (&sg)[NA]) {
    int pick = NA - 1;
    bool found = false;
    float cum = 0.f;
#pragma unroll
    for (int a = 0; a + 1 < NA; ++a) {
        cum += sg[a];
        if (!found && u < cum) {
            pick = a;
            found = true;
        }
    }
#pragma unroll
    for (int a = 0; a < NA; ++a) sg[a] = (a == pick) ? (A.xs_mode == 2 ? sg[a] : 1.0f) : 0.f;
}

template <int HC>
__device__ __forceinline__ void down_terminals(const Ctx& c, const NodeTask& nt, const RoundArgs& Rk, int b, int n_act) {
    const uint32_t nl_p = Rk.rp[c.p].n_live[b];
    const float scale = Rk.chance_scale[b];
    int n_fold = 0, n_sd = 0, a_fold = 0, a_sd = 0;
    for (int a = 0; a < n_act; ++a) {
        const int ck = nt.child[a].kind;
        if (ck == CK_FOLD) {
            ++n_fold;
            a_fold = a;
        } else if (ck == CK_SHOWDOWN) {
            ++n_sd;
            a_sd = a;
        }
    }
    float4 acc = f4zero();
    if (n_fold == 1 && n_sd == 1) {
        const bool fold_first = a_fold < a_sd;
        const float* rf = SM_X + (fold_first ? 0 : c.Hx);
        const float* rs = SM_X + (fold_first ? c.Hx : 0);
        float total_f;
        const float total = scan_reach<HC, true>(c, rs, rf, &total_f);
        const float cf = nt.child[a_fold].coef * scale, cs = nt.child[a_sd].coef * scale;
        const float c0 = fold_first ? cf : cs, c1 = fold_first ? cs : cf;
        staged_recs_wait();
        if (c.pos4 < c.HpP) {
            uint4 rec[4];
            staged_recs4<HC>(c, rec);
#pragma unroll
            for (int i = 0; i < 4; ++i) {
                if (uint32_t(c.pos4 + i) < nl_p) {
                    float m_sd, sd;
                    hand_terms<HC>(c, rs, total, rec[i], m_sd, sd);
                    const float m = hand_mass(SM_BF, rf, total_f, rec[i]);
                    const float t0 = fold_first ? m : sd, t1 = fold_first ? sd : m;
                    f4set(acc, i, f4get(acc, i) + c0 * t0);
                    f4set(acc, i, f4get(acc, i) + c1 * t1);
                }
            }
        }
    } else {
        int slot = 0;
        for (int a = 0; a < n_act; ++a) {
            const int ck = nt.child[a].kind;
            if (ck != CK_FOLD && ck != CK_SHOWDOWN) continue;
            const float* r = SM_X + slot * c.Hx;
            ++slot;
            const float cf = nt.child[a].coef * scale;
            const float total = scan_reach<HC, false>(c, r);
            staged_recs_wait();
            if (c.pos4 < c.HpP) {
                uint4 rec[4];
                staged_recs4<HC>(c, rec);
#pragma unroll
                for (int i = 0; i < 4; ++i) {
                    if (uint32_t(c.pos4 + i) < nl_p) {
                        float m, sd;
                        if (ck == CK_FOLD) {
                            m = hand_mass(SM_B, r, total, rec[i]);
                            f4set(acc, i, f4get(acc, i) + cf * m);
                        } else {
                            hand_terms<HC>(c, r, total, rec[i], m, sd);
                            f4set(acc, i, f4get(acc, i) + cf * sd);
                        }
                    }
                }
            }
        }
    }
    if (c.pos4 < c.HpP) stcg4(Rk.cbuf + (size_t(nt.out) * Rk.n_boards + b) * c.HpP + c.pos4, acc);
}

template <int HC, int MODE, int NA, bool XS>
__device__ __forceinline__ void task_down(const TaskArgs& A, const Ctx& c, const NodeTask& nt, const RoundArgs& Rk, int k, int b) {
    const DevRoundPlayer& O = Rk.rp[c.o];
    const uint32_t nrp = O.n_rows_pad[b];
    const float* __restrict__ slab = (MODE == KM_CFR ? O.regrets : O.ssum) + O.board_off[b] + size_t(nrp) * nt.cum_a;
    if (nt.out >= 0) {
        stage_lists_raw<HC>(c.tid, c.HoP, O.cl_pos + size_t(b) * 2 * c.HoP);
        stage_recs<HC>(c, reinterpret_cast<const uint32_t*>(Rk.rp[c.p].hrec) + size_t(b) * 4 * c.HpP);
    }
    const float4 r4 = load_reach4(A, c, nt, Rk, k, b);
    uint32_t rows[4] = {0xffffu, 0xffffu, 0xffffu, 0xffffu};
    if (!O.identity && c.pos4 < c.HoP) unpack4(__ldg(reinterpret_cast<const uint2*>(O.row_of_pos + size_t(b) * c.HoP + c.pos4)), rows);
    float g[4 * NA];
    load_rows<NA>(slab, O.identity != 0, c.pos4, nrp, rows, g);
    float4 v[NA];
    uint32_t xs_slot[4] = {0, 0, 0, 0};
    if (XS && c.pos4 < c.HoP) unpack4(__ldg(reinterpret_cast<const uint2*>(O.slot_of_pos + size_t(b) * c.HoP + c.pos4)), xs_slot);
#pragma unroll
    for (int i = 0; i < 4; ++i) {
        float sg[NA];
        sigma_row<NA>(g, i, sg);
        if (XS) xs_pick<NA>(A, xs_uniform(A.xs_key, nt.an_index, uint32_t(Rk.board_base + b), xs_slot[i]), sg);
        const float r = f4get(r4, i);
#pragma unroll
        for (int a = 0; a < NA; ++a) f4set(v[a], i, r * sg[a]);
    }
    int slot = 0;
#pragma unroll
    for (int a = 0; a < NA; ++a) {
        const int ck = nt.child[a].kind;
        if (c.pos4 < c.HoP) {
            if (ck == CK_FOLD || ck == CK_SHOWDOWN) *reinterpret_cast<float4*>(SM_X + slot * c.Hx + c.pos4) = v[a];
            else if (nt.child[a].buf >= 0) stcg4(Rk.rbuf + (size_t(nt.child[a].buf) * Rk.n_boards + b) * c.HoP + c.pos4, v[a]);
        }
        if (ck == CK_FOLD || ck == CK_SHOWDOWN) ++slot;
    }
    if (nt.out < 0) return;
    down_terminals<HC>(c, nt, Rk, b, NA);
}

template <int HC, int MODE, bool XS>
__device__ __forceinline__ void task_down_generic(const TaskArgs& A, const Ctx& c, const NodeTask& nt, const RoundArgs& Rk, int k, int b) {
    const DevRoundPlayer& O = Rk.rp[c.o];
    const uint32_t nrp = O.n_rows_pad[b];
    const float* __restrict__ slab = (MODE == KM_CFR ? O.regrets : O.ssum) + O.board_off[b] + size_t(nrp) * nt.cum_a;
    const float4 r4 = load_reach4(A, c, nt, Rk, k, b);
    const int n_act = nt.n_act;
    const uint32_t nl_o = O.n_live[b];
    uint32_t rows[4] = {0xffffu, 0xffffu, 0xffffu, 0xffffu};
    if (c.pos4 < c.HoP) unpack4(__ldg(reinterpret_cast<const uint2*>(O.row_of_pos + size_t(b) * c.HoP + c.pos4)), rows);
    if (c.pos4 < c.HoP) {
        for (int i = 0; i < 4; ++i) {
            const bool live = uint32_t(c.pos4 + i) < nl_o && rows[i] != 0xffffu;
            const float r = live ? f4get(r4, i) : 0.f;
            float norm = 0.f;
            if (live)
                for (int a = 0; a < n_act; ++a) norm += fmaxf(slab[size_t(rows[i]) * n_act + a], 0.f);
            int pick = -1;
            if (XS && live) {
                const float u = xs_uniform(A.xs_key, nt.an_index, uint32_t(Rk.board_base + b), O.slot_of_pos[size_t(b) * c.HoP + c.pos4 + i]);
                pick = n_act - 1;
                float cum = 0.f;
                for (int a = 0; a + 1 < n_act; ++a) {
                    cum += norm > 0.f ? fmaxf(slab[size_t(rows[i]) * n_act + a], 0.f) / norm : 1.0f / float(n_act);
                    if (u < cum) {
                        pick = a;
                        break;
                    }
                }
            }
            int slot = 0;
            for (int a = 0; a < n_act; ++a) {
                float v = 0.f;
                if (live) v = norm > 0.f ? r * fmaxf(slab[size_t(rows[i]) * n_act + a], 0.f) / norm : r / float(n_act);
                if (XS && live) v = (a == pick) ? (A.xs_mode == 2 ? v : r) : 0.f;
                const int ck = nt.child[a].kind;
                if (ck == CK_FOLD || ck == CK_SHOWDOWN) SM_X[(slot++) * c.Hx + c.pos4 + i] = v;
                else if (nt.child[a].buf >= 0) __stcg(Rk.rbuf + (size_t(nt.child[a].buf) * Rk.n_boards + b) * c.HoP + c.pos4 + i, v);
            }
        }
    }
    if (nt.out < 0) return;
    stage_lists_raw<HC>(c.tid, c.HoP, O.cl_pos + size_t(b) * 2 * c.HoP);
    stage_recs<HC>(c, reinterpret_cast<const uint32_t*>(Rk.rp[c.p].hrec) + size_t(b) * 4 * c.HpP);
    down_terminals<HC>(c, nt, Rk, b, n_act);
}

template <int HC>
__device__ __forceinline__ void trav_terms(const TaskArgs& A, const Ctx& c, const NodeTask& nt, const RoundArgs& Rk, int k, int b,
                                           bool need_sd, float4& mass, float4& sd) {
    const DevRoundPlayer& Pp = Rk.rp[c.p];
    stage_lists_raw<HC>(c.tid, c.HoP, Rk.rp[c.o].cl_pos + size_t(b) * 2 * c.HoP);
    stage_recs<HC>(c, reinterpret_cast<const uint32_t*>(Pp.hrec) + size_t(b) * 4 * c.HpP);
    const float4 r4 = load_reach4(A, c, nt, Rk, k, b);
    if (c.pos4 < c.HoP) *reinterpret_cast<float4*>(SM_RS + c.pos4) = r4;
    const float total = scan_reach<HC, false>(c, SM_RS);
    mass = f4zero();
    sd = f4zero();
    const uint32_t nl_p = Pp.n_live[b];
    staged_recs_wait();
    if (c.pos4 < c.HpP) {
        uint4 rec[4];
        staged_recs4<HC>(c, rec);
#pragma unroll
        for (int i = 0; i < 4; ++i) {
            if (uint32_t(c.pos4 + i) < nl_p) {
                float m, s = 0.f;
                if (need_sd) hand_terms<HC>(c, SM_RS, total, rec[i], m, s);
                else m = hand_mass(SM_B, SM_RS, total, rec[i]);
                f4set(mass, i, m);
                f4set(sd, i, s);
            }
        }
    }
}

template <int HC>
__device__ __forceinline__ void trav_terms_or_load(const TaskArgs& A, const Ctx& c, const NodeTask& nt, const RoundArgs& Rk, int k, int b,
                                                   bool need_sd, float4& mass, float4& sd) {
    if (!nt.pre_terms) {
        trav_terms<HC>(A, c, nt, Rk, k, b, need_sd, mass, sd);
        return;
    }
    mass = f4zero();
    sd = f4zero();
    if (c.pos4 < c.HpP) {
        const float* m = Rk.cbuf + (size_t(nt.aux) * Rk.n_boards + b) * c.HpP + c.pos4;
        mass = ldcg4(m);
        if (need_sd) sd = ldcg4(m + size_t(Rk.n_boards) * c.HpP);
    }
}

__device__ __forceinline__ float4 rule_factors(const TaskArgs& A) { return ldcg4(A.ctl->rule); }
__device__ __forceinline__ float rule_regret(const float4& f, float r, float d) { return fmaxf((r > 0.f ? f.x : f.y) * r + d, f.w); }

template <int HC, int MODE, int NA, bool DR>
__device__ __forceinline__ void task_trav(const TaskArgs& A, const Ctx& c, const NodeTask& nt, const RoundArgs& Rk, int k, int b) {
    const DevRoundPlayer& Pp = Rk.rp[c.p];
    const float scale = Rk.chance_scale[b];
    float4 dr;
    if (DR) dr = rule_factors(A);
    float4 v[NA];
    bool need_sd = false;
#pragma unroll
    for (int a = 0; a < NA; ++a) {
        v[a] = f4zero();
        need_sd |= (nt.child[a].kind == CK_SHOWDOWN);
    }
    float4 mass, sd;
    trav_terms_or_load<HC>(A, c, nt, Rk, k, b, need_sd, mass, sd);
#pragma unroll
    for (int a = 0; a < NA; ++a)
        if (nt.child[a].kind == CK_VALUE) v[a] = child_value4(A, c, Rk, nt.child[a], b);
#pragma unroll
    for (int a = 0; a < NA; ++a) {
        const int ck = nt.child[a].kind;
        const float cf = nt.child[a].coef * scale;
        if (ck == CK_FOLD) v[a] = make_float4(cf * mass.x, cf * mass.y, cf * mass.z, cf * mass.w);
        else if (ck == CK_SHOWDOWN) v[a] = make_float4(cf * sd.x, cf * sd.y, cf * sd.z, cf * sd.w);
    }
    const uint32_t nrp = Pp.n_rows_pad[b];
    const uint32_t nl_p = Pp.n_live[b];
    float* out = (nt.root_scatter ? Rk.sbuf : Rk.cbuf) + (size_t(nt.out) * Rk.n_boards + b) * c.HpP;
    float* tabR = Pp.regrets + Pp.board_off[b] + size_t(nrp) * nt.cum_a;
    float* tabS = Pp.ssum + Pp.board_off[b] + size_t(nrp) * nt.cum_a;
    if (Pp.identity) {
        if (uint32_t(c.pos4) >= nrp) {
            if (c.pos4 < c.HpP && !nt.root_scatter) stcg4(out + c.pos4, f4zero());
            return;
        }
        const uint32_t none[4] = {0, 0, 0, 0};
        float g[4 * NA], ss[4 * NA];
        if (MODE == KM_CFR) load_rows<NA>(tabR, true, c.pos4, nrp, none, g);
        if (MODE != KM_BR) load_rows<NA>(tabS, true, c.pos4, nrp, none, ss);
        float4 vn4 = f4zero();
#pragma unroll
        for (int i = 0; i < 4; ++i) {
            float sg[NA];
            float vn;
            if (MODE == KM_BR) {
                vn = -3.0e38f;
#pragma unroll
                for (int a = 0; a < NA; ++a) vn = fmaxf(vn, f4get(v[a], i));
            } else {
                if (MODE == KM_CFR) sigma_row<NA>(g, i, sg);
                else sigma_row<NA>(ss, i, sg);
                vn = 0.f;
#pragma unroll
                for (int a = 0; a < NA; ++a) vn += sg[a] * f4get(v[a], i);
            }
            const bool live = uint32_t(c.pos4 + i) < nl_p;
            f4set(vn4, i, live ? vn : 0.f);
            if (MODE == KM_CFR) {
                const float w = f4get(mass, i) * scale;
#pragma unroll
                for (int a = 0; a < NA; ++a) {
                    if (DR) {
                        const float r = g[i * NA + a];
                        if (live) {
                            g[i * NA + a] = rule_regret(dr, r, r > A.prune_threshold ? f4get(v[a], i) - vn : 0.f);
                            ss[i * NA + a] = dr.z * ss[i * NA + a] + sg[a] * w;
                        }
                    } else {
                        g[i * NA + a] += (live && g[i * NA + a] > A.prune_threshold) ? f4get(v[a], i) - vn : 0.f;
                        ss[i * NA + a] += live ? sg[a] * w : 0.f;
                    }
                }
            }
        }
        if (MODE == KM_CFR) {
#pragma unroll
            for (int q = 0; q < NA; ++q) {
                *reinterpret_cast<float4*>(tabR + size_t(c.pos4) * NA + 4 * q) = make_float4(g[4 * q], g[4 * q + 1], g[4 * q + 2], g[4 * q + 3]);
                *reinterpret_cast<float4*>(tabS + size_t(c.pos4) * NA + 4 * q) = make_float4(ss[4 * q], ss[4 * q + 1], ss[4 * q + 2], ss[4 * q + 3]);
            }
        }
        store_value4(c, nt, Rk, b, out, vn4);
        return;
    }
    float* M = SM_X;
    if (c.pos4 < c.HpP) {
        *reinterpret_cast<float4*>(M + c.pos4) = mass;
#pragma unroll
        for (int a = 0; a < NA; ++a) *reinterpret_cast<float4*>(SM_X + (1 + a) * c.Hx + c.pos4) = v[a];
        if (!nt.root_scatter) stcg4(out + c.pos4, f4zero());
    }
    csync(c.nc);
    const uint32_t n_rows = Pp.n_rows[b];
    const uint16_t* __restrict__ rstart = Pp.row_start + size_t(b) * (c.HpP + 4);
    const uint16_t* __restrict__ rpos = Pp.row_pos + size_t(b) * c.HpP;
    const float* V1 = SM_X + c.Hx;
    for (uint32_t row = c.tid; row < n_rows; row += c.nc) {
        float rg[NA], sr[NA], sg[NA], d[NA];
        float norm = 0.f;
#pragma unroll
        for (int a = 0; a < NA; ++a) {
            rg[a] = MODE == KM_CFR ? tabR[size_t(row) * NA + a] : 0.f;
            sr[a] = MODE != KM_BR ? tabS[size_t(row) * NA + a] : 0.f;
            sg[a] = fmaxf(MODE == KM_CFR ? rg[a] : sr[a], 0.f);
            norm += sg[a];
            d[a] = 0.f;
        }
        const float inv = norm > 0.f ? 1.0f / norm : 0.f;
#pragma unroll
        for (int a = 0; a < NA; ++a) sg[a] = norm > 0.f ? sg[a] * inv : 1.0f / float(NA);
        float msum = 0.f;
        const int hs = rstart[row], he = rstart[row + 1];
        for (int q = hs; q < he; ++q) {
            const int h = rpos[q];
            float va[NA];
            float vn = (MODE == KM_BR) ? -3.0e38f : 0.f;
#pragma unroll
            for (int a = 0; a < NA; ++a) {
                va[a] = V1[a * c.Hx + h];
                if (MODE == KM_BR) vn = fmaxf(vn, va[a]);
                else vn += sg[a] * va[a];
            }
            if (MODE == KM_CFR) {
#pragma unroll
                for (int a = 0; a < NA; ++a) d[a] += va[a] - vn;
                msum += M[h];
            }
            store_value1(c, nt, Rk, b, out, h, vn);
        }
        if (MODE == KM_CFR) {
            const float w = msum * scale;
#pragma unroll
            for (int a = 0; a < NA; ++a) {
                if (DR) {
                    tabR[size_t(row) * NA + a] = rule_regret(dr, rg[a], rg[a] > A.prune_threshold ? d[a] : 0.f);
                    tabS[size_t(row) * NA + a] = dr.z * sr[a] + sg[a] * w;
                } else {
                    tabR[size_t(row) * NA + a] = rg[a] + (rg[a] > A.prune_threshold ? d[a] : 0.f);
                    tabS[size_t(row) * NA + a] = sr[a] + sg[a] * w;
                }
            }
        }
    }
}

template <int HC, int MODE, bool DR>
__device__ __forceinline__ void task_trav_generic(const TaskArgs& A, const Ctx& c, const NodeTask& nt, const RoundArgs& Rk, int k, int b) {
    const DevRoundPlayer& Pp = Rk.rp[c.p];
    const float scale = Rk.chance_scale[b];
    float4 dr;
    if (DR) dr = rule_factors(A);
    const int n_act = nt.n_act;
    bool need_sd = false;
    for (int a = 0; a < n_act; ++a) {
        const int ck = nt.child[a].kind;
        if (ck == CK_VALUE && c.pos4 < c.HpP) *reinterpret_cast<float4*>(SM_X + (1 + a) * c.Hx + c.pos4) = child_value4(A, c, Rk, nt.child[a], b);
        need_sd |= (ck == CK_SHOWDOWN);
    }
    float4 mass, sd;
    trav_terms_or_load<HC>(A, c, nt, Rk, k, b, need_sd, mass, sd);
    float* out = (nt.root_scatter ? Rk.sbuf : Rk.cbuf) + (size_t(nt.out) * Rk.n_boards + b) * c.HpP;
    if (c.pos4 < c.HpP) {
        *reinterpret_cast<float4*>(SM_X + c.pos4) = mass;
        for (int a = 0; a < n_act; ++a) {
            const int ck = nt.child[a].kind;
            const float cf = nt.child[a].coef * scale;
            if (ck == CK_FOLD) *reinterpret_cast<float4*>(SM_X + (1 + a) * c.Hx + c.pos4) = make_float4(cf * mass.x, cf * mass.y, cf * mass.z, cf * mass.w);
            else if (ck == CK_SHOWDOWN) *reinterpret_cast<float4*>(SM_X + (1 + a) * c.Hx + c.pos4) = make_float4(cf * sd.x, cf * sd.y, cf * sd.z, cf * sd.w);
        }
        if (!nt.root_scatter) stcg4(out + c.pos4, f4zero());
    }
    csync(c.nc);
    const uint32_t nrp = Pp.n_rows_pad[b];
    const uint32_t n_rows = Pp.n_rows[b];
    float* tabR = Pp.regrets + Pp.board_off[b] + size_t(nrp) * nt.cum_a;
    float* tabS = Pp.ssum + Pp.board_off[b] + size_t(nrp) * nt.cum_a;
    const uint16_t* __restrict__ rstart = Pp.row_start + size_t(b) * (c.HpP + 4);
    const uint16_t* __restrict__ rpos = Pp.row_pos + size_t(b) * c.HpP;
    const float* M = SM_X;
    const float* V1 = SM_X + c.Hx;
    for (uint32_t row = c.tid; row < n_rows; row += c.nc) {
        const float* tsrc = (MODE == KM_EVAL ? tabS : tabR) + size_t(row) * n_act;
        float norm = 0.f;
        if (MODE != KM_BR)
            for (int a = 0; a < n_act; ++a) norm += fmaxf(tsrc[a], 0.f);
        const float inv = norm > 0.f ? 1.0f / norm : 0.f;
        const float uni = 1.0f / float(n_act);
        float msum = 0.f, vsum = 0.f;
        const int hs = rstart[row], he = rstart[row + 1];
        for (int q = hs; q < he; ++q) {
            const int h = rpos[q];
            float vn = (MODE == KM_BR) ? -3.0e38f : 0.f;
            for (int a = 0; a < n_act; ++a) {
                const float va = V1[a * c.Hx + h];
                if (MODE == KM_BR) vn = fmaxf(vn, va);
                else vn += (norm > 0.f ? fmaxf(tsrc[a], 0.f) * inv : uni) * va;
            }
            vsum += vn;
            msum += M[h];
            store_value1(c, nt, Rk, b, out, h, vn);
        }
        if (MODE == KM_CFR) {
            const float w = msum * scale;
            for (int a = 0; a < n_act; ++a) {
                float da = -vsum;
                for (int q = hs; q < he; ++q) da += V1[a * c.Hx + rpos[q]];
                const float old = tabR[size_t(row) * n_act + a];
                const float sga = norm > 0.f ? fmaxf(old, 0.f) * inv : uni;
                if (DR) {
                    tabS[size_t(row) * n_act + a] = dr.z * tabS[size_t(row) * n_act + a] + sga * w;
                    tabR[size_t(row) * n_act + a] = rule_regret(dr, old, old > A.prune_threshold ? da : 0.f);
                } else {
                    tabS[size_t(row) * n_act + a] += sga * w;
                    tabR[size_t(row) * n_act + a] = old + (old > A.prune_threshold ? da : 0.f);
                }
            }
        }
    }
}

__device__ __forceinline__ int board_of(const TaskArgs& A, int k, int inst) {
    return (k > 0 && A.sample_board[k] != nullptr) ? A.sample_board[k][inst] : inst;
}
__device__ __forceinline__ int parent_instance(const TaskArgs& A, const RoundArgs& Rk, int k, int inst, int b) {
    if (A.sample_board[k] == nullptr) return Rk.parent_board[b];
    return k - 1 == 0 ? Rk.parent_board[b] : inst;
}

template <int MODE>
__device__ __forceinline__ void prefetch_task_tables(const TaskArgs& A, uint32_t tk, uint32_t j) {
    const NodeTask* g = A.tasks + j;
    const int kind = g->kind;
    if (kind != TK_DOWN && kind != TK_UP_TRAV) return;
    const RoundArgs& Rk = A.rounds[g->round_k];
    const int b = board_of(A, g->round_k, int(tk - g->first));
    const int q = kind == TK_DOWN ? 1 - A.trav : A.trav;
    const DevRoundPlayer& D = Rk.rp[q];
    const uint32_t nrp = D.n_rows_pad[b];
    const size_t off = D.board_off[b] + size_t(nrp) * g->cum_a;
    const uint32_t bytes = nrp * uint32_t(g->n_act) * 4u;
    if (kind == TK_DOWN) {
        prefetch_l2_bulk((MODE == KM_CFR ? D.regrets : D.ssum) + off, bytes);
    } else {
        if (MODE == KM_CFR) prefetch_l2_bulk(D.regrets + off, bytes);
        if (MODE != KM_BR) prefetch_l2_bulk(D.ssum + off, bytes);
    }
}

struct TaskSlot {
    uint32_t ticket;
    uint32_t epoch;
    uint32_t xseq;
    uint32_t pad;
    NodeTask nt;
};

template <int KM, int MAXT, int MINB, bool XS>
__global__ void __launch_bounds__(MAXT + 32, MINB) task_kernel(const __grid_constant__ TaskArgs A) {
    constexpr bool DR = KM == KM_CFR_DR;
    constexpr int MODE = DR ? int(KM_CFR) : KM;
    constexpr int HC = 4 * MAXT;
    __shared__ __align__(16) TaskSlot s_slot[2];

    __shared__ __align__(8) uint64_t s_done;

    const int NC = blockDim.x - 32;
    const int tid = threadIdx.x;
    if (tid == 0) mbar_init(&s_done, uint32_t(NC >> 5));
    if (tid < 2) SM_B[54 + tid] = SM_BF[54 + tid] = 0.f;
    __syncthreads();

    if (tid >= NC) {
        const int lane = tid - NC;
        uint32_t epoch = 0, xseq = 0;
        if (lane == 0) {
            epoch = ld_acquire_u32(&A.ctl->epoch);
            xseq = *reinterpret_cast<const volatile unsigned int*>(&A.ctl->xch_seq);
        }
        epoch = __shfl_sync(0xffffffffu, epoch, 0);
        uint32_t prev_tk = 0xffffffffu, parity = 0;
        int buf = 0;
        uint32_t tk_next = 0;
        if (lane == 0) tk_next = A.t0 + uint32_t(atomicAdd(&A.ctl->ticket, 1ull));
        tk_next = __shfl_sync(0xffffffffu, tk_next, 0);
        for (;;) {
            bool published = (prev_tk == 0xffffffffu);
            auto try_publish = [&]() {
                if (lane == 0 && !published && mbar_test(&s_done, parity)) {
#ifndef RS_NO_PUBLISH_FENCE
                    __threadfence();
#endif
                    st_release_u32(A.flags + prev_tk, epoch);
                    published = true;
                }
            };
            uint32_t tk = tk_next;
            uint32_t sl = A.t1;
            if (tk < A.t1) {
                unsigned long long pend = 0;
                if (lane == 0) pend = atomicAdd(&A.ctl->ticket, 1ull);
                sl = A.order ? __ldg(A.order + tk) : tk;
                const uint32_t j = __ldg(A.task_of_ticket + sl);
                const NodeTask* gt = A.tasks + j;
                NodeTask& st = s_slot[buf].nt;
                for (int i = lane; i < int(sizeof(NodeTask) / 4); i += 32)
                    reinterpret_cast<uint32_t*>(&st)[i] = __ldg(reinterpret_cast<const uint32_t*>(gt) + i);
                __syncwarp();
                const int kind = st.kind;
                const int k = st.round_k;
                const int inst = int(sl - st.first);
                const int b = board_of(A, k, inst);
                const RoundArgs& Rk = A.rounds[k];
                const int nd = st.n_dep;
                const bool sampled = A.sample_board[1] != nullptr;
                int total;
                uint32_t gfirst = 0;
                if (kind == TK_GATHER) {
                    if (sampled) {
                        gfirst = uint32_t(st.dep[0]) + uint32_t(k == 0 ? 0 : inst);
                        total = k == 0 ? A.n_paths : 1;
                    } else {
                        gfirst = uint32_t(st.dep[0]) + uint32_t(Rk.per_parent > 0 ? b * Rk.per_parent : 0);
                        total = Rk.per_parent > 0 ? Rk.per_parent : Rk.n_boards_next;
                    }
                } else {
                    total = nd + st.n_src_all;
                }
                auto flag_index = [&](int i, bool& has) -> uint32_t {
                    has = true;
                    if (kind == TK_GATHER) return gfirst + uint32_t(i);
                    int dfirst, dk = DK_SAME_BOARD;
                    if (i < nd) {
                        dfirst = st.dep[i];
                        dk = st.dep_kind[i];
                    } else {
                        dfirst = __ldg(&A.srcs[st.src_all_first + (i - nd)].dep);
                    }
                    has = dfirst >= 0;
                    return uint32_t(dfirst) + uint32_t(dk == DK_PARENT_BOARD ? parent_instance(A, Rk, k, inst, b) : inst);
                };
                int i = lane;
                bool has = false;
                uint32_t idx = 0;
                if (i < total) idx = flag_index(i, has);
                if (lane == 0) prefetch_task_tables<MODE>(A, sl, j);
                if (kind == TK_UP_TRAV || kind == TK_UP_OPP)
                    for (int q = lane; q < int(st.n_src_all); q += 32) {
                        const TaskSrc sr = A.srcs[st.src_all_first + q];
                        prefetch_l2_bulk((sr.kind == SK_CBUF ? Rk.cbuf : Rk.gathered) + (size_t(sr.buf) * Rk.n_boards + b) * A.HpP, uint32_t(A.HpP) * 4u);
                    }
                if (lane == 1 && st.r_in != RIN_INITIAL && !st.rin_parent_round && (kind == TK_DOWN || kind == TK_TRAV_TERMS || (kind == TK_UP_TRAV && !st.pre_terms)))
                    prefetch_l2_bulk(Rk.rbuf + (size_t(st.r_in) * Rk.n_boards + b) * A.HoP, uint32_t(A.HoP) * 4u);
                try_publish();
                (void)b;
                const unsigned long long t_wait = global_ns();
                uint32_t spins = 0;
                bool gave_up = false;
                for (;;) {
                    if (i < total) {
                        if (!has || idx < A.t0 || ld_acquire_u32(A.flags + idx) == epoch) {
                            i += 32;
                            if (i < total) idx = flag_index(i, has);
                        }
                    }
                    try_publish();
                    if (__all_sync(0xffffffffu, i >= total)) break;
                    __nanosleep(RS_POLL_SLEEP_NS);
                    if (__any_sync(0xffffffffu, lane == 0 && wait_gives_up(A, t_wait, spins))) {
                        gave_up = true;
                        break;
                    }
                }
                tk_next = A.t0 + uint32_t(__shfl_sync(0xffffffffu, pend, 0));
                if (gave_up) tk = tk_next = sl = A.t1;
            }
            if (lane == 0) {
                s_slot[buf].ticket = sl;
                s_slot[buf].epoch = epoch;
                s_slot[buf].xseq = xseq;
            }
            __syncwarp();
            hsync(NC + 32);
            if (lane == 0 && !published) {
#ifndef RS_NO_PUBLISH_FENCE
                __threadfence();
#endif
                st_release_u32(A.flags + prev_tk, epoch);
            }
            if (prev_tk != 0xffffffffu) parity ^= 1;
            if (tk >= A.t1) break;
            prev_tk = sl;
            buf ^= 1;
        }
        if (lane == 0) {
            __threadfence();
            const unsigned int e = atomicAdd(&A.ctl->exited, 1u);
            if (e == gridDim.x - 1) {
                A.ctl->ticket = 0ull;
                A.ctl->exited = 0u;
                if (A.xch_bump) A.ctl->xch_seq = xseq + 1;
                __threadfence();
                st_release_u32(&A.ctl->epoch, epoch + 1);
            }
        }
        return;
    }

    Ctx c;
    c.nc = NC;
    c.tid = tid;
    c.lane = tid & 31;
    c.warp = tid >> 5;
    c.nwarps = NC >> 5;
    c.pos4 = 4 * tid;
    c.p = A.trav;
    c.o = 1 - c.p;
    c.Hp = A.H[c.p];
    c.Ho = A.H[c.o];
    c.HpP = A.HpP;
    c.HoP = A.HoP;
    c.Hx = A.Hx;

    int buf = 0;
    for (;;) {
        hsync(NC + 32);
        const uint32_t t = s_slot[buf].ticket;
        if (t >= A.t1) break;
        const NodeTask& nt = s_slot[buf].nt;
        const int kind = nt.kind;
        const int k = nt.round_k;
        const int inst = int(t - nt.first);
        const int b = board_of(A, k, inst);
        const RoundArgs& Rk = A.rounds[k];
#ifdef RS_TASK_TIMING
        const long long tm1 = clock64();
        if (tid == 0 && A.timing) {
            unsigned long long gt0;
            asm volatile("mov.u64 %0, %globaltimer;" : "=l"(gt0));
            atomicMin(A.timing + 32 + (kind * 3 + k) * 2, gt0);
        }
#endif
        switch (kind) {
            case TK_DOWN: {
                switch (nt.n_act) {
                    case 2: task_down<HC, MODE, 2, XS>(A, c, nt, Rk, k, b); break;
                    case 3: task_down<HC, MODE, 3, XS>(A, c, nt, Rk, k, b); break;
                    case 4: task_down<HC, MODE, 4, XS>(A, c, nt, Rk, k, b); break;
                    case 5: task_down<HC, MODE, 5, XS>(A, c, nt, Rk, k, b); break;
                    default: task_down_generic<HC, MODE, XS>(A, c, nt, Rk, k, b); break;
                }
                break;
            }
            case TK_UP_TRAV: {
                switch (nt.n_act) {
                    case 2: task_trav<HC, MODE, 2, DR>(A, c, nt, Rk, k, b); break;
                    case 3: task_trav<HC, MODE, 3, DR>(A, c, nt, Rk, k, b); break;
                    case 4: task_trav<HC, MODE, 4, DR>(A, c, nt, Rk, k, b); break;
                    case 5: task_trav<HC, MODE, 5, DR>(A, c, nt, Rk, k, b); break;
                    default: task_trav_generic<HC, MODE, DR>(A, c, nt, Rk, k, b); break;
                }
                break;
            }
            case TK_UP_OPP: {
                if (c.pos4 < c.HpP) {
                    float4 v = nt.aux >= 0 ? ldcg4(Rk.cbuf + (size_t(nt.aux) * Rk.n_boards + b) * c.HpP + c.pos4) : f4zero();
                    for (int a = 0; a < nt.n_act; ++a)
                        if (nt.child[a].kind == CK_VALUE) v = f4add(v, child_value4(A, c, Rk, nt.child[a], b));
                    store_value4(c, nt, Rk, b, (nt.root_scatter ? Rk.sbuf : Rk.cbuf) + (size_t(nt.out) * Rk.n_boards + b) * c.HpP, v);
                }
                break;
            }
            case TK_GATHER: {
                if (c.pos4 < c.HpP) {
                    const RoundArgs& Rn = A.rounds[k + 1];
                    const float* base = Rn.sbuf + size_t(nt.aux) * Rn.n_boards * c.HpP + c.pos4;
                    float4 acc = f4zero();
                    if (A.sample_board[k + 1] != nullptr) {
                        const int32_t* sb = A.sample_board[k + 1];
                        const int s0 = k == 0 ? 0 : inst, ns = k == 0 ? A.n_paths : 1;
                        for (int i = 0; i < ns; ++i) acc = f4add(acc, ldcg4(base + size_t(sb[s0 + i]) * c.HpP));
                        const float w = A.gather_scale[k];
                        acc = make_float4(acc.x * w, acc.y * w, acc.z * w, acc.w * w);
                    } else {
                        const int cb0 = Rk.per_parent > 0 ? b * Rk.per_parent : 0;
                        const int ncb = Rk.per_parent > 0 ? Rk.per_parent : Rk.n_boards_next;
                        const float* src = base + size_t(cb0) * c.HpP;
                        for (int i0 = 0; i0 < ncb; i0 += 8) {
                            float4 val[8];
#pragma unroll
                            for (int u = 0; u < 8; ++u) val[u] = (i0 + u < ncb) ? ldcg4(src + size_t(i0 + u) * c.HpP) : f4zero();
#pragma unroll
                            for (int u = 0; u < 8; ++u) acc = f4add(acc, val[u]);
                        }
                    }
                    stcg4(Rk.gathered + (size_t(nt.out) * Rk.n_boards + b) * c.HpP + c.pos4, acc);
                }
                if (A.xch_world > 1 && k + 1 == A.xch_round) {
                    const uint32_t ep = s_slot[buf].xseq;
                    const size_t vec = ((size_t(ep & 1u) * A.xch_leaves + nt.out) * Rk.n_boards + b) * A.xch_world;
                    if (c.pos4 < c.HpP) {
                        const float4 part = ldcg4(Rk.gathered + (size_t(nt.out) * Rk.n_boards + b) * c.HpP + c.pos4);
                        for (int peer = 0; peer < A.xch_world; ++peer)
                            *reinterpret_cast<float4*>(A.xch_peer[peer] + (vec + A.xch_rank) * c.HpP + c.pos4) = part;
                    }
                    __threadfence_system();
                    csync(c.nc);
                    if (tid < A.xch_world) {
                        st_release_sys_u32(A.xflag_peer[tid] + vec + A.xch_rank, ep);
                        const uint32_t* mine = A.xflag_peer[A.xch_rank] + vec + tid;
                        const unsigned long long t_wait = global_ns();
                        uint32_t spins = 0;
                        while (ld_acquire_sys_u32(mine) != ep) {
                            __nanosleep(100);
                            spins += 31;
                            if (wait_gives_up(A, t_wait, spins)) break;
                        }
                    }
                    csync(c.nc);
                    if (c.pos4 < c.HpP) {
                        const float* src = A.xch_peer[A.xch_rank] + vec * c.HpP + c.pos4;
                        float4 acc = f4zero();
                        for (int r = 0; r < A.xch_world; ++r) acc = f4add(acc, ldcg4(src + size_t(r) * c.HpP));
                        stcg4(Rk.gathered + (size_t(nt.out) * Rk.n_boards + b) * c.HpP + c.pos4, acc);
                    }
                }
                break;
            }
            case TK_TRAV_TERMS: {
                bool need_sd = false;
                for (int a = 0; a < nt.n_act; ++a) need_sd |= (nt.child[a].kind == CK_SHOWDOWN);
                float4 mass, sd;
                trav_terms<HC>(A, c, nt, Rk, k, b, need_sd, mass, sd);
                if (c.pos4 < c.HpP) {
                    float* m = Rk.cbuf + (size_t(nt.out) * Rk.n_boards + b) * c.HpP + c.pos4;
                    stcg4(m, mass);
                    stcg4(m + size_t(Rk.n_boards) * c.HpP, sd);
                }
                break;
            }
            case TK_ROOT_SHOWDOWN: {
                float4 mass, sd;
                trav_terms<HC>(A, c, nt, Rk, k, b, true, mass, sd);
                const float cf = nt.child[0].coef * Rk.chance_scale[b];
                if (c.pos4 < c.HpP)
                    store_value4(c, nt, Rk, b, (nt.root_scatter ? Rk.sbuf : Rk.cbuf) + (size_t(nt.out) * Rk.n_boards + b) * c.HpP,
                                 make_float4(cf * sd.x, cf * sd.y, cf * sd.z, cf * sd.w));
                break;
            }
            case TK_CHANCE_DOWN: {
                const float4 r4 = load_reach4(A, c, nt, Rk, k, b);
                if (c.pos4 < c.HoP) stcg4(Rk.rbuf + (size_t(nt.aux) * Rk.n_boards + b) * c.HoP + c.pos4, r4);
                break;
            }
            case TK_CHANCE_UP: {
                if (c.pos4 < c.HpP)
                    store_value4(c, nt, Rk, b, (nt.root_scatter ? Rk.sbuf : Rk.cbuf) + (size_t(nt.out) * Rk.n_boards + b) * c.HpP,
                                 ldcg4(Rk.gathered + (size_t(nt.aux) * Rk.n_boards + b) * c.HpP + c.pos4));
                break;
            }
            default: break;
        }
#ifdef RS_TASK_TIMING
        if (tid == 0 && A.timing) {
            atomicAdd(A.timing + kind * 4 + 0, 1ull);
            atomicAdd(A.timing + kind * 4 + 2, (unsigned long long)(clock64() - tm1));
            unsigned long long gt1;
            asm volatile("mov.u64 %0, %globaltimer;" : "=l"(gt1));
            atomicMax(A.timing + 32 + (kind * 3 + k) * 2 + 1, gt1);
        }
#endif
        __syncwarp();
        if (c.lane == 0) mbar_arrive(&s_done);
// ... 127 lines not shown
```

### rustsolver_b200/csrc/kernels.cuh

```cuda
#pragma once
#include <cuda_runtime.h>
#include <stdint.h>

#include "plan.h"
#include "tasks.h"

namespace rs {

constexpr int MAX_ACTIONS = MAX_TASK_CHILDREN;
constexpr int RS_MAX_PEERS = 8;
constexpr int FAST_ACTIONS = 4;
constexpr int MAX_TASK_THREADS = 352;

enum KernelMode { KM_CFR = 0, KM_BR = 1, KM_EVAL = 2, KM_CFR_XS = 3, KM_CFR_DR = 4, KM_CFR_XS_DR = 5 };

__host__ __device__ inline float xs_uniform(unsigned long long key, uint32_t an_index, uint32_t board, uint32_t slot) {
    unsigned long long z = key ^ ((unsigned long long)an_index << 44) ^ ((unsigned long long)board << 20) ^ (unsigned long long)slot;
    z = (z ^ (z >> 30)) * 0xBF58476D1CE4E5B9ull;
    z = (z ^ (z >> 27)) * 0x94D049BB133111EBull;
    z ^= z >> 31;
    return float(uint32_t(z >> 40)) * (1.0f / 16777216.0f);
}

struct DevRoundPlayer {
    const uint16_t* row_of_pos;
    const uint16_t* row_start;
    const uint16_t* row_pos;
    const uint16_t* cl_pos;
    const uint16_t* parent_pos;
    const uint16_t* child_pos;
    const uint16_t* slot_of_pos;
    const HandRec* hrec;
    const uint32_t* n_rows;
    const uint32_t* n_rows_pad;
    const uint32_t* n_live;
    const uint64_t* board_off;
    float* regrets;
    float* ssum;
    int identity;
    int pad;
};

struct RoundArgs {
    DevRoundPlayer rp[2];
    const float* chance_scale;
    const int32_t* parent_board;
    float* rbuf;
    float* cbuf;
    float* sbuf;
    float* gathered;
    int n_boards;
    int per_parent;
    int n_boards_next;
    int board_base;
};

struct TaskArgs {
    RoundArgs rounds[3];
    const NodeTask* tasks;
    const TaskSrc* srcs;
    const uint32_t* task_of_ticket;
    const uint32_t* order;
    uint32_t n_tasks;
    uint32_t* flags;
    TaskCtl* ctl;
    const float* root_weights[2];
    int H[2], Hpad[2];
    int trav;
    int HpP, HoP, Hx;
    uint32_t t0, t1;
    const int32_t* sample_board[3];
    int n_paths;
    float gather_scale[3];
    int slots;
    float prune_threshold;
    float* xch_peer[RS_MAX_PEERS];
    uint32_t* xflag_peer[RS_MAX_PEERS];
    int xch_world, xch_rank;
    int xch_round;
    int xch_leaves;
    unsigned long long xs_key;
    int xs_mode;
    int xch_bump;
    const volatile uint32_t* host_abort;
    unsigned long long wait_timeout_ns;
    unsigned long long* timing;
};

size_t task_kernel_smem_bytes(bool wide, int slots, int Hp_pad, int Ho_pad);
cudaError_t configure_task_kernels(size_t smem, int threads, bool wide, int* blocks_per_sm);
cudaError_t launch_task_kernel(const TaskArgs& a, int mode, int grid, int threads, bool wide, size_t smem, cudaStream_t st);

cudaError_t launch_scale(float* data, size_t n, float d, cudaStream_t st);
cudaError_t launch_set_rule(TaskCtl* ctl, const float f[4], cudaStream_t st);
cudaError_t launch_normalize(const float* in, float* out, uint32_t n_rows, uint32_t A, cudaStream_t st);
cudaError_t launch_unpermute(const float* in, const uint16_t* slot_of_pos, const uint32_t* n_live, float* out, uint32_t n_boards, uint32_t hp,
                             uint32_t H, cudaStream_t st);

}
```

### rustsolver_b200/solver.py

```python
from __future__ import annotations

import ctypes as C
from dataclasses import dataclass, field
from typing import List, Optional, Sequence

import numpy as np

from . import _lib
from ._lib import (EngineError, check, f32p, f64p, i32p, rs_abstraction, rs_config, rs_ranges,
                   rs_round_abstraction, rs_stats, rs_tree, rs_update_rule, u8p, u16p, u32p, u64p)

RS_ABS_NONE, RS_ABS_ISOMORPHIC, RS_ABS_CLUSTER_ARR, RS_ABS_BUCKET_TABLE = 0, 1, 2, 3
RS_FLAG_NO_GRAPH = 1
RS_FLAG_NO_CHAIN_SPLIT = 2
RS_FLAG_STREET_KERNEL = 4
RS_FLAG_SHARD_ISOLATED = 8
RS_RULE_VANILLA, RS_RULE_DCFR, RS_RULE_LCFR, RS_RULE_CFR_PLUS = 0, 1, 2, 3
NODE_ACTION, NODE_TERMINAL, NODE_PUBLIC_CHANCE, NODE_PRIVATE_CHANCE = 0, 1, 2, 3
TERM_ALLIN, TERM_SHOWDOWN, TERM_UNCONTESTED = 0, 1, 2
ACTION_NAMES = {0: "Bet", 1: "Raise", 2: "Check", 3: "Call", 4: "Fold"}


def _ptr(a: np.ndarray, t):
    return a.ctypes.data_as(t)
# ... 140 lines not shown
                k = {TERM_ALLIN: "L", TERM_SHOWDOWN: "S", TERM_UNCONTESTED: "U"}[int(self.ttype[i])]
                out.append(f"{i} {k} {int(self.value[i])}/{int(self.last_to_act[i])}")
            else:
                acts = []
                for e in range(self.child_offset[i], self.child_offset[i + 1]):
                    kind = int(self.action_kind[e])
                    amt = float(self.action_amount[e])
                    acts.append({2: "X", 3: "C", 4: "F"}.get(kind) or (("B" if kind == 0 else "R") + f"{amt:g}"))
                out.append(f"{i} A {int(self.an_index[i])}/P{int(self.player[i])} [{','.join(acts)}] ->{ch}")
        return out


def build_game_tree(options: Options):
    lib = _lib.load()
    h = options._handle()
    th = C.c_void_p()
    try:
        check(lib.rsh_build_game_tree(h, C.byref(th)))
    finally:
        lib.rsh_options_free(h)
    try:
        v = rs_tree()
        check(lib.rsh_tree_view(th, C.byref(v)))
        n = v.n_nodes
        ne = lib.rsh_tree_n_edges(th)

        def arr(p, count, dt):
            return np.ctypeslib.as_array(p, shape=(count,)).astype(dt, copy=True) if count else np.zeros(0, dt)

        tree = GameTree(arr(v.type, n, np.uint8), arr(v.parent, n, np.int32), arr(v.child_offset, n + 1, np.uint32),
                        arr(v.children, ne, np.uint32), arr(v.player, n, np.uint8), arr(v.an_index, n, np.uint32),
                        arr(v.round_idx, n, np.uint8), arr(v.value, n, np.uint32), arr(v.ttype, n, np.uint8),
                        arr(v.last_to_act, n, np.uint8), arr(lib.rsh_tree_round(th), n, np.uint8),
                        arr(lib.rsh_tree_action_kind(th), ne, np.uint8), arr(lib.rsh_tree_action_amount(th), ne, np.float64))
        return int(lib.rsh_tree_n_actions(th)), tree
    finally:
        lib.rsh_tree_free(th)


RS_DIST_EMD_1D, RS_DIST_L2 = 0, 1


def kmeans_assign(points: np.ndarray, centers: np.ndarray, dist: int = RS_DIST_EMD_1D, return_ms: bool = False):
    lib = _lib.load()
    x = np.ascontiguousarray(points, dtype=np.float32)
    c = np.ascontiguousarray(centers, dtype=np.float32)
    assert x.ndim == 2 and c.ndim == 2 and x.shape[1] == c.shape[1]
    cl = np.zeros(len(x), dtype=np.uint32)
    md = np.zeros(len(x), dtype=np.float32)
    inertia, ms = C.c_double(0.0), C.c_float(0.0)
    check(lib.rs_kmeans_assign(_ptr(x, f32p), len(x), x.shape[1], _ptr(c, f32p), len(c), dist, _ptr(cl, u32p), _ptr(md, f32p),
                               C.byref(inertia), C.byref(ms)))
    return (cl, md, float(inertia.value), float(ms.value)) if return_ms else (cl, md, float(inertia.value))


def kmeans_fit_regular(points: np.ndarray, centers: np.ndarray, dist: int = RS_DIST_EMD_1D, rounds: int = 10):
    lib = _lib.load()
    x = np.ascontiguousarray(points, dtype=np.float32)
    c = np.array(centers, dtype=np.float32, copy=True, order="C")
    assert x.ndim == 2 and c.ndim == 2 and x.shape[1] == c.shape[1]
    cl = np.zeros(len(x), dtype=np.uint32)
    inertia = C.c_float(0.0)
    check(lib.rs_kmeans_fit_regular(_ptr(x, f32p), len(x), x.shape[1], _ptr(c, f32p), len(c), dist, rounds, _ptr(cl, u32p),
                                    C.byref(inertia)))
    return cl, c, float(inertia.value)


def generate_histograms(round_: int, first_index: int, count: int, samples: int, bins: int, seed: int = 1, return_ms: bool = False):
    lib = _lib.load()
    out = np.zeros((count, bins), dtype=np.float32)
    cards = np.zeros((count, 7), dtype=np.uint8)
    ms = C.c_float(0.0)
    check(lib.rs_generate_histograms(round_, first_index, count, samples, bins, seed, _ptr(out, f32p), _ptr(cards, u8p), C.byref(ms)))
    return (out, cards, float(ms.value)) if return_ms else (out, cards)


def kmeans_fit_growbatch(points: np.ndarray, centers: np.ndarray, initial_batch_size: int, dist: int = RS_DIST_EMD_1D, seed: int = 1):
    lib = _lib.load()
    x = np.ascontiguousarray(points, dtype=np.float32)
    c = np.array(centers, dtype=np.float32, copy=True, order="C")
    assert x.ndim == 2 and c.ndim == 2 and x.shape[1] == c.shape[1]
    idx = np.zeros(initial_batch_size, dtype=np.uint32)
    cl = np.zeros(initial_batch_size, dtype=np.uint32)
    stats = np.zeros(2, dtype=np.float32)
    check(lib.rs_kmeans_fit_growbatch(_ptr(x, f32p), len(x), x.shape[1], _ptr(c, f32p), len(c), dist, initial_batch_size, seed,
                                      _ptr(idx, u32p), _ptr(cl, u32p), _ptr(stats, f32p)))
    return idx, cl, c, float(stats[0]), float(stats[1])


def histogram_distances(p: np.ndarray, q: np.ndarray, dist: int = RS_DIST_EMD_1D) -> np.ndarray:
    lib = _lib.load()
    a = np.ascontiguousarray(p, dtype=np.float32)
    b = np.ascontiguousarray(q, dtype=np.float32)
    assert a.shape == b.shape and a.ndim == 2
    out = np.zeros(len(a), dtype=np.float32)
    check(lib.rs_histogram_distances(_ptr(a, f32p), _ptr(b, f32p), len(a), a.shape[1], dist, _ptr(out, f32p)))
    return out


def kmeans_update_min_dists(points: np.ndarray, new_center: np.ndarray, min_dists: np.ndarray, dist: int = RS_DIST_EMD_1D) -> np.ndarray:
    lib = _lib.load()
    x = np.ascontiguousarray(points, dtype=np.float32)
    c = np.ascontiguousarray(new_center, dtype=np.float32)
    md = np.array(min_dists, dtype=np.float32, copy=True)
    check(lib.rs_kmeans_update_min_dists(_ptr(x, f32p), len(x), x.shape[1], _ptr(c, f32p), dist, _ptr(md, f32p)))
    return md


def kmeans_init_pp(points: np.ndarray, k: int, dist: int = RS_DIST_EMD_1D, seed: int = 1):
    lib = _lib.load()
    x = np.ascontiguousarray(points, dtype=np.float32)
    chosen = np.zeros(k, dtype=np.uint32)
    centers = np.zeros((k, x.shape[1]), dtype=np.float32)
    check(lib.rs_kmeans_init_pp(_ptr(x, f32p), len(x), x.shape[1], k, dist, seed, _ptr(chosen, u32p), _ptr(centers, f32p)))
    return chosen, centers


def kmeans_init_random(points: np.ndarray, k: int, n_restarts: int, dist: int = RS_DIST_EMD_1D, seed: int = 1):
    lib = _lib.load()
    x = np.ascontiguousarray(points, dtype=np.float32)
    chosen = np.zeros(k, dtype=np.uint32)
    centers = np.zeros((k, x.shape[1]), dtype=np.float32)
    check(lib.rs_kmeans_init_random(_ptr(x, f32p), len(x), x.shape[1], k, n_restarts, dist, seed, _ptr(chosen, u32p), _ptr(centers, f32p)))
    return chosen, centers


class HandIndexer:

    def __init__(self, cards_per_round: Sequence[int]):
        self._lib = _lib.load()
        cpr = np.asarray(cards_per_round, dtype=np.uint8)
        self.cards_per_round = [int(x) for x in cpr]
        self._h = self._lib.rsh_indexer_new(len(cpr), _ptr(cpr, u8p))
        if not self._h:
            raise EngineError(-1, self._lib.rs_last_error().decode())

    def __del__(self):
        if getattr(self, "_h", None):
            self._lib.rsh_indexer_free(self._h)
            self._h = None

    def size(self, round: int) -> int:
        return int(self._lib.rsh_indexer_size(self._h, round))

    def get_index(self, cards: Sequence[int]) -> int:
        a = np.asarray(cards, dtype=np.uint8)
        return int(self._lib.rsh_indexer_index(self._h, _ptr(a, u8p)))

    def index_many(self, cards: np.ndarray) -> np.ndarray:
        a = np.ascontiguousarray(cards, dtype=np.uint8)
        assert a.ndim == 2 and a.shape[1] == sum(self.cards_per_round)
        out = np.zeros(len(a), dtype=np.uint64)
        self._lib.rsh_indexer_index_many(self._h, _ptr(a, u8p), len(a), _ptr(out, u64p))
        return out

    def index_many_gpu(self, cards: np.ndarray, return_ms: bool = False):
        assert len(self.cards_per_round) == 2 and self.cards_per_round[0] == 2
        a = np.ascontiguousarray(cards, dtype=np.uint8)
        assert a.ndim == 2 and a.shape[1] == sum(self.cards_per_round)
        out = np.zeros(len(a), dtype=np.uint64)
        ms = C.c_float(0.0)
        check(self._lib.rs_gpu_index_hands(self.cards_per_round[1], _ptr(a, u8p), len(a), _ptr(out, u64p), C.byref(ms)))
        return (out, float(ms.value)) if return_ms else out

    def get_hand(self, round: int, index: int) -> List[int]:
        n = sum(self.cards_per_round[:round + 1])
        out = np.zeros(n, dtype=np.uint8)
        check(self._lib.rsh_indexer_get_hand(self._h, round, index, _ptr(out, u8p)))
        return [int(x) for x in out]


@dataclass
class CardAbstraction:
    kind: int = RS_ABS_NONE
    cluster_arr: Optional[np.ndarray] = None
    bucket_table: Optional[List[np.ndarray]] = None

    @staticmethod
    def ISOMORPHIC():
        return CardAbstraction(RS_ABS_ISOMORPHIC)

    @staticmethod
    def NONE():
        return CardAbstraction(RS_ABS_NONE)

    @staticmethod
    def from_file(path: str):
        return CardAbstraction(RS_ABS_CLUSTER_ARR, cluster_arr=np.fromfile(path, dtype="<u4"))


def _abstraction_struct(card_abs: Sequence[CardAbstraction], keep: list) -> rs_abstraction:
    ab = rs_abstraction()
    ab.n_rounds = len(card_abs)
    for k, ca in enumerate(card_abs):
        ra = ab.rounds[k]
        ra.kind = ca.kind
        if ca.kind == RS_ABS_CLUSTER_ARR:
            arr = np.ascontiguousarray(ca.cluster_arr, dtype=np.uint32)
            keep.append(arr)
            ra.cluster_arr = _ptr(arr, u32p)
            ra.cluster_arr_len = len(arr)
        if ca.kind == RS_ABS_BUCKET_TABLE:
            for p in range(2):
                arr = np.ascontiguousarray(ca.bucket_table[p], dtype=np.uint32)
                keep.append(arr)
                ra.bucket_table[p] = _ptr(arr, u32p)
    return ab


def nccl_unique_id() -> bytes:
    buf = (C.c_uint8 * _lib.RS_NCCL_ID_BYTES)()
    check(_lib.load().rs_nccl_unique_id(buf))
    return bytes(buf)


class _PlanOrEngine:
    _prefix = "rs_"

    def _fn(self, name):
        return getattr(self._lib, self._prefix + name)

    def board_id(self, round_idx: int, dealt: Sequence[int]) -> int:
        a = np.asarray(list(dealt) + [0], dtype=np.uint8)
        out = C.c_uint32()
        check(self._fn("board_id")(self._h, round_idx, _ptr(a, u8p), len(dealt), C.byref(out)))
        return out.value

    def card_table(self, round_idx: int, player: int, board_id: int) -> np.ndarray:
        out = np.zeros(self.n_hands[player], dtype=np.uint16)
        nr = C.c_uint32()
        check(self._fn("card_table")(self._h, round_idx, player, board_id, _ptr(out, u16p), len(out), C.byref(nr)))
        return out

    def num_rows(self, round_idx: int, player: int, board_id: int) -> int:
        nr = C.c_uint32()
        check(self._fn("card_table")(self._h, round_idx, player, board_id, None, 0, C.byref(nr)))
        return nr.value


class Plan(_PlanOrEngine):
    _prefix = "rs_plan_"

    def __init__(self, tree: GameTree, ranges: Sequence[np.ndarray], board_mask: int,
                 card_abs: Sequence[CardAbstraction] = (), board_masks: Optional[Sequence[int]] = None,
                 rank: int = 0, world_size: int = 1, flags: int = 0):
        self._lib = _lib.load()
        self._keep = []
        tv = tree.view()
        rr = rs_ranges()
        hs = [np.ascontiguousarray(r, dtype=np.uint8) for r in ranges]
        for p in range(2):
            rr.n_hands[p] = len(hs[p])
            rr.hands[p] = _ptr(hs[p], u8p)
        ab = _abstraction_struct(card_abs, self._keep)
        cfg = rs_config()
        cfg.board_mask = board_mask
        cfg.rank, cfg.world_size = rank, world_size
        cfg.flags = flags
        h = C.c_void_p()
        if board_masks is not None:
            bm = np.asarray(board_masks, dtype=np.uint64)
            check(self._lib.rs_plan_create(C.byref(tv), C.byref(rr), C.byref(ab), C.byref(cfg), _ptr(bm, u64p), len(bm), C.byref(h)))
        else:
            check(self._lib.rs_plan_create(C.byref(tv), C.byref(rr), C.byref(ab), C.byref(cfg), None, 0, C.byref(h)))
        self._h = h
        self.n_hands = [len(hs[0]), len(hs[1])]

    def __del__(self):
        if getattr(self, "_h", None):
            self._lib.rs_plan_destroy(self._h)
            self._h = None

    def stats(self) -> rs_stats:
        s = rs_stats()
        check(self._lib.rs_plan_stats(self._h, C.byref(s)))
        return s

    def infoset_offset(self, an_index: int, board_id: int):
        off, nr, na = C.c_uint64(), C.c_uint32(), C.c_uint32()
        check(self._lib.rs_plan_infoset_offset(self._h, an_index, board_id, C.byref(off), C.byref(nr), C.byref(na)))
        return off.value, nr.value, na.value

    def showdown_order(self, player: int, board_id: int):
        order = np.zeros(self.n_hands[player], dtype=np.uint16)
        cls = np.zeros(self.n_hands[player], dtype=np.uint32)
        nl = C.c_uint32()
        check(self._lib.rs_plan_showdown_order(self._h, player, board_id, _ptr(order, u16p), _ptr(cls, u32p), len(order), C.byref(nl)))
        return order[:nl.value].copy(), cls[:nl.value].copy()

    def check_execution_order(self, traverser: int, force_board_major: bool = False):
        n, moved = C.c_uint32(), C.c_uint32()
        check(self._lib.rs_plan_check_execution_order(self._h, traverser, int(force_board_major), C.byref(n), C.byref(moved)))
        return int(n.value), int(moved.value)

    def local_tables(self, round_idx: int, player: int, board_id: int):
        dims = (C.c_uint32 * 2)()
        check(self._lib.rs_plan_local_tables(self._h, round_idx, player, board_id, None, None, None, dims))
        hp, nl = int(dims[0]), int(dims[1])
        rec = np.zeros((hp, 4), dtype=np.uint32)
        cl = np.zeros(2 * hp, dtype=np.uint16)
        sop = np.zeros(hp, dtype=np.uint16)
        check(self._lib.rs_plan_local_tables(self._h, round_idx, player, board_id, _ptr(rec, u32p), _ptr(cl, u16p), _ptr(sop, u16p), dims))
        return rec, cl, sop, nl

    def street_info(self, traverser: int) -> dict:
        out = (C.c_uint32 * 8)()
        check(self._lib.rs_plan_street_info(self._h, traverser, out))
        keys = ("eligible", "segments", "max_rows", "max_slots", "max_q_sd", "max_q_mo", "down_ops", "up_ops")
        d = dict(zip(keys, [int(x) for x in out]))
        d["why"] = "" if d["eligible"] else self._lib.rs_last_error().decode()
        return d

    def street_program(self, traverser: int, board_id: int) -> dict:
        n = C.c_uint32()
        dims = (C.c_uint32 * 4)()
        check(self._lib.rs_plan_street_program(self._h, traverser, board_id, None, 0, C.byref(n), None, 0, dims))
        words = np.zeros(max(n.value, 1), dtype=np.uint32)
        hinfo = np.zeros(2 * dims[2], dtype=np.uint32)
        check(self._lib.rs_plan_street_program(self._h, traverser, board_id, _ptr(words, u32p), len(words), C.byref(n),
                                               _ptr(hinfo, u32p), len(hinfo), dims))
        ls, cs = int(dims[0]), int(dims[1])
        return {"lists": words[:ls * 208].reshape(ls, 208), "chunks": words[ls * 208:ls * 208 + cs * 128].reshape(cs, 128),
                "hinfo": hinfo.reshape(-1, 2), "HpP": int(dims[2]), "HoP": int(dims[3])}


def sample_runouts(seed: int, board_mask: int, n_cards: int, n_paths: int, distinct_first: bool = True) -> np.ndarray:
    out = np.zeros((n_paths, n_cards), dtype=np.uint8)
    check(_lib.load().rs_sample_runouts(seed, board_mask, n_cards, n_paths, int(distinct_first), _ptr(out, u8p)))
    return out


class Engine(_PlanOrEngine):

    def __init__(self, tree: GameTree, ranges: Sequence[np.ndarray], board_mask: int,
                 card_abs: Sequence[CardAbstraction] = (), board_masks: Optional[Sequence[int]] = None,
                 device: int = 0, rank: int = 0, world_size: int = 1, nccl_id: Optional[bytes] = None,
                 flags: int = 0, threads_per_block: int = 0, discount_interval: int = 0, discount_cap: int = 0):
        self._lib = _lib.load()
        self._keep = []
        self.tree = tree
        tv = tree.view()
        rr = rs_ranges()
        hs = [np.ascontiguousarray(r, dtype=np.uint8) for r in ranges]
        for p in range(2):
            rr.n_hands[p] = len(hs[p])
            rr.hands[p] = _ptr(hs[p], u8p)
        ab = _abstraction_struct(card_abs, self._keep)
        cfg = rs_config()
        cfg.board_mask = board_mask
        cfg.device, cfg.rank, cfg.world_size = device, rank, world_size
        if nccl_id is not None:
            C.memmove(cfg.nccl_id, nccl_id, _lib.RS_NCCL_ID_BYTES)
        cfg.flags = flags
        cfg.threads_per_block = threads_per_block
        cfg.discount_interval, cfg.discount_cap = discount_interval, discount_cap
        h = C.c_void_p()
        if board_masks is not None:
            bm = np.asarray(board_masks, dtype=np.uint64)
            check(self._lib.rs_create_batch(C.byref(tv), C.byref(rr), C.byref(ab), C.byref(cfg), _ptr(bm, u64p), len(bm), C.byref(h)))
        else:
            check(self._lib.rs_create(C.byref(tv), C.byref(rr), C.byref(ab), C.byref(cfg), C.byref(h)))
        self._h = h
        self.n_hands = [len(hs[0]), len(hs[1])]
        self.ranges = hs

    def close(self):
        if getattr(self, "_h", None):
            self._lib.rs_destroy(self._h)
            self._h = None

    __del__ = close

    def iterate(self, n: int = 1):
        check(self._lib.rs_iterate(self._h, n))

    def iterate_sampled(self, paths):
        a = np.ascontiguousarray(paths, dtype=np.uint8)
        if a.ndim == 1:
            a = a.reshape(1, -1)
        check(self._lib.rs_iterate_sampled(self._h, _ptr(a, u8p), a.shape[0]))

    def discount(self, d: float):
        check(self._lib.rs_discount(self._h, d))

    def reset(self):
        check(self._lib.rs_reset(self._h))

    def stats(self) -> rs_stats:
        s = rs_stats()
        check(self._lib.rs_stats_get(self._h, C.byref(s)))
        return s

    def _shape(self, an_index: int, board_id: int):
        nr, na = C.c_uint32(), C.c_uint32()
        check(self._lib.rs_read_infoset(self._h, an_index, board_id, None, None, 0, C.byref(nr), C.byref(na)))
        return nr.value, na.value

    def read_infoset(self, an_index: int, board_id: int = 0):
        nr, na = self._shape(an_index, board_id)
        r = np.zeros((nr, na), dtype=np.float32)
        s = np.zeros((nr, na), dtype=np.float32)
        check(self._lib.rs_read_infoset(self._h, an_index, board_id, _ptr(r, f32p), _ptr(s, f32p), r.size, None, None))
        return r, s

    def write_infoset(self, an_index: int, board_id: int, regrets: np.ndarray, strategy_sum: np.ndarray):
        r = np.ascontiguousarray(regrets, dtype=np.float32)
        s = np.ascontiguousarray(strategy_sum, dtype=np.float32)
        check(self._lib.rs_write_infoset(self._h, an_index, board_id, _ptr(r, f32p), _ptr(s, f32p), r.size))

    def average_strategy(self, an_index: int, board_id: int = 0) -> np.ndarray:
        nr, na = self._shape(an_index, board_id)
        out = np.zeros((nr, na), dtype=np.float32)
        check(self._lib.rs_average_strategy(self._h, an_index, board_id, _ptr(out, f32p), out.size, None, None))
        return out

    def current_strategy(self, an_index: int, board_id: int = 0) -> np.ndarray:
        nr, na = self._shape(an_index, board_id)
        out = np.zeros((nr, na), dtype=np.float32)
        check(self._lib.rs_current_strategy(self._h, an_index, board_id, _ptr(out, f32p), out.size, None, None))
        return out

    def set_range_weights(self, player: int, weights: np.ndarray):
        w = np.ascontiguousarray(weights, dtype=np.float32)
        check(self._lib.rs_set_range_weights(self._h, player, _ptr(w, f32p), w.size))

    def profile_iteration(self):
        cap = 64
        buf = (_lib.rs_kernel_time * cap)()
        n = C.c_uint32()
        check(self._lib.rs_profile_iteration(self._h, buf, cap, C.byref(n)))
        kinds = {0: "traversal", 1: "street", 3: "allreduce"}
        return [dict(kind=kinds[buf[i].kind], phase=buf[i].phase, traverser=buf[i].traverser, grid=buf[i].grid,
                     ms=buf[i].ms, table_bytes=buf[i].table_bytes, vector_bytes=buf[i].vector_bytes) for i in range(n.value)]

    def dump_average_strategy(self, path: str) -> int:
        n = C.c_uint64(0)
        check(self._lib.rs_dump_average_strategy(self._h, str(path).encode(), C.byref(n)))
        return int(n.value)

    def set_prune_threshold(self, threshold: float):
        check(self._lib.rs_set_prune_threshold(self._h, float(threshold)))

    def set_opponent_sampling(self, mode: int, seed: int = 0):
        check(self._lib.rs_set_opponent_sampling(self._h, int(mode), int(seed)))

    def set_update_rule(self, kind: int, alpha: float = 1.5, beta: float = 0.0, gamma: float = 2.0):
        r = rs_update_rule(int(kind), float(alpha), float(beta), float(gamma))
        check(self._lib.rs_set_update_rule(self._h, C.byref(r)))

    def update_rule(self):
        r, t = rs_update_rule(), C.c_uint64()
        check(self._lib.rs_get_update_rule(self._h, C.byref(r), C.byref(t)))
        return r.kind, r.alpha, r.beta, r.gamma, int(t.value)

    def set_wait_timeout_ms(self, ms: int):
        check(self._lib.rs_set_wait_timeout_ms(self._h, int(ms)))

    def abort(self):
        check(self._lib.rs_abort(self._h))

    def exchange_export(self) -> bytes:
        buf = (C.c_uint8 * _lib.RS_EXCHANGE_HANDLE_BYTES)()
        check(self._lib.rs_exchange_export(self._h, buf))
        return bytes(buf)

    def exchange_import(self, handles: Sequence[bytes]):
        blob = b"".join(handles)
        assert len(blob) == len(handles) * _lib.RS_EXCHANGE_HANDLE_BYTES
        arr = (C.c_uint8 * len(blob)).from_buffer_copy(blob)
        check(self._lib.rs_exchange_import(self._h, arr, len(handles)))

    def enable_fused_exchange(self, dist, device):
        import torch
        mine = torch.tensor(list(self.exchange_export()), dtype=torch.uint8, device=device)
        allh = [torch.zeros_like(mine) for _ in range(dist.get_world_size())]
        dist.all_gather(allh, mine)
        ok = 1
        try:
            self.exchange_import([bytes(h.cpu().tolist()) for h in allh])
        except EngineError as e:
            print(f"[rustsolver_b200] in-kernel exchange unavailable on this rank: {e}", flush=True)
            ok = 0
        flag = torch.tensor([ok], dtype=torch.int32, device=device)
        dist.all_reduce(flag, op=dist.ReduceOp.MIN)
        if int(flag.item()) == 0:
            check(self._lib.rs_exchange_disable(self._h))
            return False
        return True

    def best_response(self):
        out = (C.c_double * 2)()
        check(self._lib.rs_best_response(self._h, out))
        return [out[0], out[1]]

    def average_value(self):
        out = (C.c_double * 2)()
        check(self._lib.rs_average_value(self._h, out))
        return [out[0], out[1]]

    def root_values(self, player: int) -> np.ndarray:
        st = self.stats()
        out = np.zeros(st.n_boards_local[0] * self.n_hands[player], dtype=np.float32)
        check(self._lib.rs_root_values(self._h, player, _ptr(out, f32p), out.size))
        return out.reshape(st.n_boards_local[0], self.n_hands[player])


class MCCFRTrainer:

    def __init__(self):
        self.engine: Optional[Engine] = None
        self.game_tree: Optional[GameTree] = None
        self.hand_ranges: List[np.ndarray] = []
        self.initial_board_mask = 0
        self.card_abs: List[CardAbstraction] = []

    @staticmethod
    def init(options: Options, card_abs: Optional[Sequence[CardAbstraction]] = None, **engine_kwargs) -> "MCCFRTrainer":
        t = MCCFRTrainer()
        t.hand_ranges = options.ranges()
        n_actions, t.game_tree = build_game_tree(options)
        t.initial_board_mask = options.board_mask
        n_rounds = int(t.game_tree.round_idx.max()) + 1
        t.card_abs = list(card_abs) if card_abs is not None else [CardAbstraction.ISOMORPHIC() for _ in range(n_rounds)]
        t.engine = Engine(t.game_tree, t.hand_ranges, options.board_mask, t.card_abs, **engine_kwargs)
        return t

    def train(self, iterations: int):
        self.engine.iterate(iterations)

    def get_strategy(self, an_index: int, cluster_idx: int, board_id: int = 0) -> np.ndarray:
        return self.engine.current_strategy(an_index, board_id)[cluster_idx]

    def get_final_strategy(self, an_index: int, cluster_idx: int, board_id: int = 0) -> np.ndarray:
        return self.engine.average_strategy(an_index, board_id)[cluster_idx]

    def calc_br(self) -> List[float]:
        return self.engine.best_response()

    def exploitability(self, bb: float = 1.0) -> dict:
        br = self.engine.best_response()
        chips = 0.5 * (br[0] + br[1])
        return {"chips": chips, "mbb_per_game": 1000.0 * chips / bb, "br": br}
```

Baseline: 21.77.

## Store per-card lists in fixed-stride padded slots so scan needs no segment flags

Card-list positions are now laid out on the host into fixed-stride slots, one per card, with padding. The in-kernel scan can then treat each list as an aligned group of threads and do a segmented prefix over lanes within the stride. This replaces the second global block-wide scan and the CL_FIRST boundary extraction with a per-list carry and a per-list total table (SM_T). Hand records are rewritten to index the padded list layout. The cost is more list storage and possibly more threads per block, since the thread count is now at least the number needed to cover the padded lists.

```diff
diff --git a/include/b200cfr.h b/include/b200cfr.h
--- a/include/b200cfr.h
+++ b/include/b200cfr.h
@@ -214,6 +214,8 @@
 
 int rs_plan_local_tables(const rs_plan* p, uint32_t round_idx, uint32_t player, uint32_t board_id, uint32_t* hrec_words_out,
                          uint16_t* cl_pos_out, uint16_t* slot_of_pos_out, uint32_t dims_out[2]);
+int rs_plan_device_lists(const rs_plan* p, uint32_t round_idx, uint32_t player, uint32_t board_id, uint32_t* hrec_words_out,
+                         uint16_t* cl_out, size_t cl_cap, uint32_t dims_out[4]);
 int rs_plan_check_execution_order(const rs_plan* p, uint32_t traverser, int force_board_major, uint32_t* n_tickets_out,
                                   uint32_t* n_moved_out);
 int rs_plan_street_info(const rs_plan* p, uint32_t traverser, uint32_t out[8]);
diff --git a/rustsolver_b200/_lib.py b/rustsolver_b200/_lib.py
--- a/rustsolver_b200/_lib.py
+++ b/rustsolver_b200/_lib.py
@@ -119,6 +119,7 @@
     "rs_plan_infoset_offset": (C.c_int, [VP, C.c_uint32, C.c_uint32, u64p, u32p, u32p]),
     "rs_plan_showdown_order": (C.c_int, [VP, C.c_uint32, C.c_uint32, u16p, u32p, C.c_size_t, u32p]),
     "rs_plan_local_tables": (C.c_int, [VP, C.c_uint32, C.c_uint32, C.c_uint32, u32p, u16p, u16p, u32p]),
+    "rs_plan_device_lists": (C.c_int, [VP, C.c_uint32, C.c_uint32, C.c_uint32, u32p, u16p, C.c_size_t, u32p]),
     "rs_plan_check_execution_order": (C.c_int, [VP, C.c_uint32, C.c_int, u32p, u32p]),
     "rs_plan_street_info": (C.c_int, [VP, C.c_uint32, u32p]),
     "rs_plan_street_program": (C.c_int, [VP, C.c_uint32, C.c_uint32, u32p, C.c_size_t, u32p, u32p, C.c_size_t, u32p]),
diff --git a/rustsolver_b200/csrc/engine.cu b/rustsolver_b200/csrc/engine.cu
--- a/rustsolver_b200/csrc/engine.cu
+++ b/rustsolver_b200/csrc/engine.cu
@@ -4,6 +4,7 @@
 #include <cmath>
 #include <cstdio>
 #include <cstdlib>
+#include <algorithm>
 #include <cstring>
 #include <map>
 #include <memory>
@@ -112,9 +113,15 @@
     cudaError_t zero() { return cudaMemset(p, 0, (n ? n : 1) * sizeof(T)); }
 };
 
+struct ListLayout {
+    uint32_t stride, slots;
+    uint32_t pitch;
+};
+
 struct RoundDev {
     DevBuf<uint16_t> row_of_pos[2], row_start[2], row_pos[2], cl_pos[2], parent_pos[2], child_pos[2], slot_of_pos[2];
     DevBuf<HandRec> hrec[2];
+    ListLayout lists{8, 0, 8 + CL_PITCH_PAD};
     DevBuf<uint32_t> n_rows[2], n_rows_pad[2], n_live[2];
     DevBuf<uint64_t> board_off[2];
     DevBuf<float> regrets[2], ssum[2];
@@ -259,6 +266,73 @@
     int prof_end(uint32_t kind, uint32_t k, int trav, uint32_t grid, uint64_t table_bytes, uint64_t vector_bytes);
 };
 
+static ListLayout list_layout(const Plan& P, uint32_t k) {
+    uint32_t longest = 0, slots = 0;
+    for (int q = 0; q < 2; ++q) {
+        std::vector<uint32_t> pair(52 * 52, 0);
+        uint32_t with[52] = {0};
+        for (uint32_t h = 0; h < P.H[q]; ++h) {
+            const int c0 = P.hand_cards[q][2 * h], c1 = P.hand_cards[q][2 * h + 1];
+            ++pair[c0 * 52 + c1];
+            ++pair[c1 * 52 + c0];
+            ++with[c0];
+            ++with[c1];
+        }
+        for (const uint64_t m : P.board_mask[k]) {
+            uint32_t n = 0;
+            for (int c = 0; c < 52; ++c) {
+                if ((m >> c) & 1) continue;
+                uint32_t len = with[c];
+                for (int d = 0; d < 52; ++d)
+                    if ((m >> d) & 1) len -= pair[c * 52 + d];
+                longest = std::max(longest, len);
+                n += len > 0;
+            }
+            slots = std::max(slots, n);
+        }
+    }
+    const uint32_t stride = (longest / 8 + 1) * 8;
+    return ListLayout{stride, slots, stride + CL_PITCH_PAD};
+}
+
+static bool device_lists(const Plan& P, uint32_t k, uint32_t q, uint32_t b, const ListLayout& lay, uint16_t* cl_out, HandRec* rec_out) {
+    uint32_t start_o[52] = {0}, len_o[52] = {0};
+    for (int who = 0; who < 2; ++who) {
+        const uint32_t pl = who == 0 ? q : 1 - q;
+        const LocalTables& L = P.loc[k][pl];
+        const uint16_t* cl = &L.cl_pos[size_t(b) * 2 * L.Hpad];
+        if (who == 0) std::fill(cl_out, cl_out + size_t(lay.slots) * lay.stride, uint16_t(CL_POS_NONE));
+        int j = -1;
+        uint32_t d = 0;
+        for (uint32_t e = 0; e < 2 * L.Hpad && (cl[e] & CL_POS_MASK) != CL_POS_NONE; ++e) {
+            if (cl[e] & CL_FIRST) {
+                ++j;
+                d = 0;
+                if (uint32_t(j) >= lay.slots) return false;
+                if (who == 1) start_o[j] = e;
+            }
+            if (j < 0 || d + 1 >= lay.stride) return false;
+            if (who == 0) cl_out[size_t(j) * lay.stride + d] = uint16_t(cl[e] & CL_POS_MASK);
+            ++d;
+            if (who == 1) len_o[j] = d;
+        }
+    }
+    const LocalTables& L = P.loc[k][q];
+    for (uint32_t i = 0; i < L.Hpad; ++i) {
+        HandRec r = L.hrec[size_t(b) * L.Hpad + i];
+        for (int w = 0; w < 2; ++w) {
+            const uint32_t kk = (r.w3 >> (9 * w)) & 0x1ffu;
+            uint32_t& ab = w == 0 ? r.w1 : r.w2;
+            if (kk == HREC_K_NONE) continue;
+            const uint32_t j = kk / 4, lo = (ab & 0xffffu) / 4, hi = (ab >> 16) / 4;
+            if (j >= lay.slots || lo < start_o[j] || hi < lo || hi > start_o[j] + len_o[j]) return false;
+            ab = ((j * lay.pitch + lo - start_o[j]) * 4u) | (((j * lay.pitch + hi - start_o[j]) * 4u) << 16);
+        }
+        rec_out[i] = r;
+    }
+    return true;
+}
+
 template <class T>
 static std::vector<T> slice(const std::vector<T>& v, size_t lo, size_t hi, size_t stride) {
     if (v.empty()) return {};
@@ -298,12 +372,18 @@
     const bool street_wanted = P.street[0].eligible && P.street[1].eligible;
     threads = int(((maxHP / 4) + 31) / 32 * 32);
     if (threads > MAX_TASK_THREADS) return set_err(RS_ERR_UNSUPPORTED, "range larger than 1326 hands");
+    int list_threads[3] = {0, 0, 0};
+    for (uint32_t k = 0; k < P.n_rounds; ++k) {
+        rd[k].lists = list_layout(P, k);
+        list_threads[k] = int((rd[k].lists.slots * rd[k].lists.stride / 8 + 31) / 32 * 32);
+        threads = std::max(threads, list_threads[k]);
+    }
     for (uint32_t k = 0; k < P.n_rounds; ++k) {
         round_threads[k] = threads;
         if (!P.board_mask[k].empty() && !getenv("RS_UNIFORM_BLOCK")) {
             const int left = 52 - __builtin_popcountll(P.board_mask[k][0]);
             const size_t live_max = std::min<size_t>(maxHP, size_t(left) * size_t(left - 1) / 2);
-            round_threads[k] = std::min(threads, int((((live_max + 3) / 4) + 31) / 32 * 32));
+            round_threads[k] = std::max(list_threads[k], std::min(threads, int((((live_max + 3) / 4) + 31) / 32 * 32)));
         }
     }
     n_sms = prop.multiProcessorCount;
@@ -323,10 +403,15 @@
             CU(R.row_of_pos[q].upload(slice(L.row_of_pos, lo, hi, hp)));
             CU(R.row_start[q].upload(slice(L.row_start, lo, hi, hp + 4)));
             CU(R.row_pos[q].upload(slice(L.row_pos, lo, hi, hp)));
-            CU(R.cl_pos[q].upload(slice(L.cl_pos, lo, hi, 2 * hp)));
             CU(R.slot_of_pos[q].upload(slice(L.slot_of_pos, lo, hi, hp)));
             {
-                std::vector<HandRec> aos = slice(L.hrec, lo, hi, hp);
+                const size_t cl_len = size_t(R.lists.slots) * R.lists.stride;
+                std::vector<uint16_t> cl(size_t(nb) * cl_len);
+                std::vector<HandRec> aos(size_t(nb) * hp);
+                for (uint32_t b = 0; b < nb; ++b)
+                    if (!device_lists(P, k, uint32_t(q), lo + b, R.lists, &cl[b * cl_len], &aos[b * hp]))
+                        return set_err(RS_ERR_INVALID, "internal: a card list does not fit its slot");
+                CU(R.cl_pos[q].upload(cl));
                 std::vector<HandRec> soa(aos.size());
                 const uint32_t* src = reinterpret_cast<const uint32_t*>(aos.data());
                 uint32_t* dst = reinterpret_cast<uint32_t*>(soa.data());
@@ -479,7 +564,7 @@
     st_vm_rows = 4 * int(max_q_sd + max_q_mo);
     st_slots = int(max_slots);
     st_stride = size_t(st_rows) * st_XP + size_t(st_vy_rows + st_vm_rows + st_slots) * HPmax;
-    st_threads = threads;
+    st_threads = (HPmax / 4 + 31) / 32 * 32;
     if (const char* e = getenv("RS_STREET_THREADS")) st_threads = std::max(64, std::min(352, atoi(e) / 32 * 32));
     size_t budget = 72 * 1024;
     if (const char* e = getenv("RS_STREET_SMEM_KB")) budget = size_t(std::max(16, atoi(e))) * 1024;
@@ -652,6 +737,8 @@
         }
         ra.chance_scale = R.chance_scale.p;
         ra.parent_board = R.parent_board.p;
+        ra.cl_stride = int(R.lists.stride);
+        ra.cl_len = int(R.lists.slots * R.lists.stride);
         ra.rbuf = R.rbuf.p;
         ra.cbuf = R.cbuf.p;
         ra.sbuf = R.sbuf[trav].p;
@@ -1692,6 +1779,28 @@
     return RS_OK;
 }
 
+int rs_plan_device_lists(const rs_plan* p, uint32_t round_idx, uint32_t player, uint32_t board_id, uint32_t* hrec_words_out, uint16_t* cl_out,
+                         size_t cl_cap, uint32_t dims_out[4]) {
+    if (!p || player > 1 || !dims_out) return set_err(RS_ERR_INVALID, "bad argument");
+    const Plan& P = p->p;
+    if (round_idx >= P.n_rounds || board_id >= P.n_boards[round_idx]) return set_err(RS_ERR_INVALID, "round or board out of range");
+    if (board_id < P.local_lo[round_idx] || board_id >= P.local_hi[round_idx]) return set_err(RS_ERR_INVALID, "board belongs to another rank");
+    const ListLayout lay = list_layout(P, round_idx);
+    const uint32_t hp = P.loc[round_idx][player].Hpad;
+    dims_out[0] = hp;
+    dims_out[1] = lay.stride;
+    dims_out[2] = lay.slots;
+    dims_out[3] = lay.pitch;
+    if (!hrec_words_out && !cl_out) return RS_OK;
+    if (cl_out && cl_cap < size_t(lay.slots) * lay.stride) return set_err(RS_ERR_CAPACITY, "output buffer too small");
+    std::vector<uint16_t> cl(size_t(lay.slots) * lay.stride);
+    std::vector<HandRec> rec(hp);
+    if (!device_lists(P, round_idx, player, board_id, lay, cl.data(), rec.data())) return set_err(RS_ERR_INVALID, "internal: a card list does not fit its slot");
+    if (cl_out) memcpy(cl_out, cl.data(), cl.size() * sizeof(uint16_t));
+    if (hrec_words_out) memcpy(hrec_words_out, rec.data(), rec.size() * sizeof(HandRec));
+    return RS_OK;
+}
+
 int rs_plan_check_execution_order(const rs_plan* p, uint32_t traverser, int force_board_major, uint32_t* n_tickets_out, uint32_t* n_moved_out) {
     if (!p || traverser > 1) return set_err(RS_ERR_INVALID, "bad argument");
     const Plan& P = p->p;
diff --git a/rustsolver_b200/csrc/kernels.cu b/rustsolver_b200/csrc/kernels.cu
--- a/rustsolver_b200/csrc/kernels.cu
+++ b/rustsolver_b200/csrc/kernels.cu
@@ -101,29 +101,35 @@
 #define SM_RS (smem_raw)
 #define SM_P (smem_raw + HC)
 #define SM_GB (smem_raw + 2 * HC + 4)
-#define SM_WSA (smem_raw + 4 * HC + 12)
-#define SM_WSB (smem_raw + 4 * HC + 44)
-#define SM_B (smem_raw + 4 * HC + 76)
-#define SM_WSC (smem_raw + 4 * HC + 140)
-#define SM_WSD (smem_raw + 4 * HC + 172)
-#define SM_BF (smem_raw + 4 * HC + 204)
-#define SM_REC (reinterpret_cast<uint32_t*>(smem_raw + 4 * HC + 268))
-#define SM_CL (reinterpret_cast<uint32_t*>(smem_raw + 8 * HC + 268))
-#define SM_X (smem_raw + 9 * HC + 268)
-constexpr int smem_fixed_floats(int HC) { return 9 * HC + 268; }
+#define SM_WSA (smem_raw + 4 * HC + 108)
+#define SM_WSB (smem_raw + 4 * HC + 140)
+#define SM_T (smem_raw + 4 * HC + 172)
+#define SM_WSC (smem_raw + 4 * HC + 236)
+#define SM_WSD (smem_raw + 4 * HC + 268)
+#define SM_TF (smem_raw + 4 * HC + 300)
+#define SM_REC (reinterpret_cast<uint32_t*>(smem_raw + 4 * HC + 364))
+#define SM_CL (reinterpret_cast<uint32_t*>(smem_raw + 8 * HC + 364))
+#define SM_X (smem_raw + 9 * HC + 364)
+constexpr int smem_fixed_floats(int HC) { return 9 * HC + 364; }
+static_assert(52 * CL_PITCH_PAD <= 104, "SM_GB holds 52 lists at their pitch");
 
 template <int HC>
-__device__ __forceinline__ void stage_lists_raw(int tid, int HoP, const uint16_t* __restrict__ cl_pos_b) {
-    if (8 * tid < 2 * HoP)
+__device__ __forceinline__ void stage_lists_raw(int tid, int cl_len, const uint16_t* __restrict__ cl_pos_b) {
+    if (8 * tid < cl_len)
         asm volatile("cp.async.cg.shared.global [%0], [%1], 16;" ::"r"(uint32_t(__cvta_generic_to_shared(SM_CL + 4 * tid))), "l"(cl_pos_b + 8 * tid)
                      : "memory");
     asm volatile("cp.async.commit_group;" ::: "memory");
 }
 
 template <int HC, bool FOLD>
-__device__ __forceinline__ float scan_reach(const Ctx& c, const float* r, const float* rf = nullptr, float* total_f = nullptr) {
+__device__ __forceinline__ float scan_reach(const Ctx& c, const RoundArgs& Rk, const float* r, const float* rf = nullptr, float* total_f = nullptr) {
     csync(c.nc);
     const int hend = HC >= 4 * MAX_TASK_THREADS ? c.HoP : min(c.HoP, 4 * c.nc);
+    const int tpl = Rk.cl_stride >> 3;
+    const int lst = c.tid / tpl;
+    const int lj = c.tid - lst * tpl;
+    const bool lists = 8 * c.tid < Rk.cl_len;
+    const int t_at = lists && lj == tpl - 1 ? lst : -1;
     float4 x = f4zero();
     float lc = 0.f;
     if (c.pos4 < c.HoP) {
@@ -134,18 +140,14 @@
         }
     }
     float y[8], yf[8];
-    uint32_t w[4];
     {
         asm volatile("cp.async.wait_group 0;" ::: "memory");
         uint4 u = make_uint4(0x07ff07ffu, 0x07ff07ffu, 0x07ff07ffu, 0x07ff07ffu);
-        if (8 * c.tid < 2 * c.HoP) u = *reinterpret_cast<const uint4*>(SM_CL + 4 * c.tid);
-        w[0] = u.x;
-        w[1] = u.y;
-        w[2] = u.z;
-        w[3] = u.w;
+        if (lists) u = *reinterpret_cast<const uint4*>(SM_CL + 4 * c.tid);
+        const uint32_t w[4] = {u.x, u.y, u.z, u.w};
 #pragma unroll
         for (int i = 0; i < 4; ++i) {
-            const uint32_t a = w[i] & CL_POS_MASK, b = (w[i] >> 16) & CL_POS_MASK;
+            const uint32_t a = w[i] & 0xffffu, b = w[i] >> 16;
             y[2 * i] = a != CL_POS_NONE ? r[a] : 0.f;
             y[2 * i + 1] = b != CL_POS_NONE ? r[b] : 0.f;
             if (FOLD) {
@@ -165,19 +167,32 @@
 #pragma unroll
     for (int d = 1; d < 32; d <<= 1) {
         const float ta = __shfl_up_sync(0xffffffffu, ia, d);
-        const float tb = __shfl_up_sync(0xffffffffu, ib, d);
-        float tc = 0.f, td = 0.f;
+        float tb = 0.f, tc = 0.f, td = 0.f;
+        if (d < 8) tb = __shfl_up_sync(0xffffffffu, ib, d);
         if (FOLD) {
             tc = __shfl_up_sync(0xffffffffu, ic, d);
-            td = __shfl_up_sync(0xffffffffu, id, d);
+            if (d < 8) td = __shfl_up_sync(0xffffffffu, id, d);
         }
         if (c.lane >= d) {
             ia += ta;
-            ib += tb;
-            if (FOLD) {
-                ic += tc;
-                id += td;
-            }
+            if (FOLD) ic += tc;
+            if (d < 8 && lj >= d) {
+                ib += tb;
+                if (FOLD) id += td;
+            }
+        }
+    }
+    const int carry_from = lists && lj > c.lane ? c.warp - 1 : -1;
+    float2* const g = reinterpret_cast<float2*>(SM_GB + 8 * c.tid + CL_PITCH_PAD * lst);
+    if (lists) {
+        float e = ib - lb;
+#pragma unroll
+        for (int i = 0; i < 4; ++i) {
+            float2 o;
+            o.x = e;
+            o.y = e + y[2 * i];
+            e = o.y + y[2 * i + 1];
+            g[i] = o;
         }
     }
     if (c.lane == 31) {
@@ -190,88 +205,41 @@
     }
     csync(c.nc);
     float wa = c.lane < c.nwarps ? SM_WSA[c.lane] : 0.f;
-    float wb = c.lane < c.nwarps ? SM_WSB[c.lane] : 0.f;
-    float wc = 0.f, wd = 0.f;
-    if (FOLD) {
-        wc = c.lane < c.nwarps ? SM_WSC[c.lane] : 0.f;
-        wd = c.lane < c.nwarps ? SM_WSD[c.lane] : 0.f;
-    }
+    float wc = 0.f;
+    if (FOLD) wc = c.lane < c.nwarps ? SM_WSC[c.lane] : 0.f;
 #pragma unroll
     for (int d = 1; d < 16; d <<= 1) {
         const float ta = __shfl_up_sync(0xffffffffu, wa, d);
-        const float tb = __shfl_up_sync(0xffffffffu, wb, d);
-        float tc = 0.f, td = 0.f;
-        if (FOLD) {
-            tc = __shfl_up_sync(0xffffffffu, wc, d);
-            td = __shfl_up_sync(0xffffffffu, wd, d);
-        }
+        float tc = 0.f;
+        if (FOLD) tc = __shfl_up_sync(0xffffffffu, wc, d);
         if (c.lane >= d) {
             wa += ta;
-            wb += tb;
-            if (FOLD) {
-                wc += tc;
-                wd += td;
-            }
+            if (FOLD) wc += tc;
         }
     }
     const float total = __shfl_sync(0xffffffffu, wa, c.nwarps - 1);
-    const float total_b = __shfl_sync(0xffffffffu, wb, c.nwarps - 1);
     const float base_a = c.warp > 0 ? __shfl_sync(0xffffffffu, wa, c.warp - 1) : 0.f;
-    const float base_b = c.warp > 0 ? __shfl_sync(0xffffffffu, wb, c.warp - 1) : 0.f;
-    float ea = base_a + ia - la, eb = base_b + ib - lb;
-    float total_d = 0.f, ed = 0.f;
-    if (FOLD) {
-        *total_f = __shfl_sync(0xffffffffu, wc, c.nwarps - 1);
-        total_d = __shfl_sync(0xffffffffu, wd, c.nwarps - 1);
-        const float base_d = c.warp > 0 ? __shfl_sync(0xffffffffu, wd, c.warp - 1) : 0.f;
-        ed = base_d + id - ld;
-    }
+    if (FOLD) *total_f = __shfl_sync(0xffffffffu, wc, c.nwarps - 1);
     if (c.pos4 < c.HoP) {
         float4 o;
-        o.x = ea;
-        o.y = ea + x.x;
+        o.x = base_a + ia - la;
+        o.y = o.x + x.x;
         o.z = o.y + x.y;
         o.w = o.z + x.z;
         *reinterpret_cast<float4*>(SM_P + c.pos4) = o;
     }
-    if (8 * c.tid < 2 * c.HoP) {
-        float4 o0, o1;
-        o0.x = eb;
-        o0.y = o0.x + y[0];
-        o0.z = o0.y + y[1];
-        o0.w = o0.z + y[2];
-        o1.x = o0.w + y[3];
-        o1.y = o1.x + y[4];
-        o1.z = o1.y + y[5];
-        o1.w = o1.z + y[6];
-        *reinterpret_cast<float4*>(SM_GB + 8 * c.tid) = o0;
-        *reinterpret_cast<float4*>(SM_GB + 8 * c.tid + 4) = o1;
-        const uint32_t ord0 = ((w[0] >> 11) & 7u) | (((w[0] >> 27) & 7u) << 3);
-        const uint32_t b0 = c.tid == 0 ? 0u : ord0;
-        float* bp = SM_B + b0;
-        const float ex[8] = {o0.x, o0.y, o0.z, o0.w, o1.x, o1.y, o1.z, o1.w};
-#pragma unroll
-        for (int i = 0; i < 8; ++i) {
-            const bool first = ((w[i >> 1] >> ((i & 1) * 16)) & CL_FIRST) != 0;
-            if (first) *bp++ = ex[i];
-        }
-        if (c.tid == 0) SM_B[ord0] = total_b;
-        if (FOLD) {
-            float* bf = SM_BF + b0;
-            float e = ed;
-#pragma unroll
-            for (int i = 0; i < 8; ++i) {
-                const bool first = ((w[i >> 1] >> ((i & 1) * 16)) & CL_FIRST) != 0;
-                if (first) *bf++ = e;
-                e += yf[i];
-            }
-            if (c.tid == 0) SM_BF[ord0] = total_d;
-        }
-    }
-    if (c.tid == 0) {
-        SM_P[hend] = total;
-        SM_GB[2 * hend] = total_b;
-    }
+    if (carry_from >= 0) {
+        const float carry = SM_WSB[carry_from];
+#pragma unroll
+        for (int i = 0; i < 4; ++i) g[i] = make_float2(g[i].x + carry, g[i].y + carry);
+        ib += carry;
+        if (FOLD) id += SM_WSD[carry_from];
+    }
+    if (t_at >= 0) {
+        SM_T[t_at] = ib;
+        if (FOLD) SM_TF[t_at] = id;
+    }
+    if (c.tid == 0) SM_P[hend] = total;
     csync(c.nc);
     return total;
 }
@@ -306,14 +274,14 @@
 template <int HC>
 __device__ __forceinline__ void hand_terms(const Ctx& c, const float* r, float total, const uint4& rec, float& mass, float& sd) {
     const uint32_t k0 = rec.w & 0x1ffu, k1 = (rec.w >> 9) & 0x1ffu, same4 = rec.w >> 18;
-    const float g0s = ldsb(SM_B, k0), g0e = ldsb(SM_B + 1, k0), g1s = ldsb(SM_B, k1), g1e = ldsb(SM_B + 1, k1);
-    mass = total - (g0e - g0s) - (g1e - g1s) + (same4 != HREC_SAME_NONE ? ldsb(r, same4) : 0.f);
-    sd = ldsb(SM_P, rec.x & 0xffffu) + ldsb(SM_P, rec.x >> 16) - total - ldsb(SM_GB, rec.y & 0xffffu) - ldsb(SM_GB, rec.y >> 16) + g0s + g0e -
-         ldsb(SM_GB, rec.z & 0xffffu) - ldsb(SM_GB, rec.z >> 16) + g1s + g1e;
-}
-__device__ __forceinline__ float hand_mass(const float* B, const float* r, float total, const uint4& rec) {
+    const float t0 = ldsb(SM_T, k0), t1 = ldsb(SM_T, k1);
+    mass = total - t0 - t1 + (same4 != HREC_SAME_NONE ? ldsb(r, same4) : 0.f);
+    sd = ldsb(SM_P, rec.x & 0xffffu) + ldsb(SM_P, rec.x >> 16) - total - ldsb(SM_GB, rec.y & 0xffffu) - ldsb(SM_GB, rec.y >> 16) + t0 -
+         ldsb(SM_GB, rec.z & 0xffffu) - ldsb(SM_GB, rec.z >> 16) + t1;
+}
+__device__ __forceinline__ float hand_mass(const float* T, const float* r, float total, const uint4& rec) {
     const uint32_t k0 = rec.w & 0x1ffu, k1 = (rec.w >> 9) & 0x1ffu, same4 = rec.w >> 18;
-    return total - (ldsb(B + 1, k0) - ldsb(B, k0)) - (ldsb(B + 1, k1) - ldsb(B, k1)) + (same4 != HREC_SAME_NONE ? ldsb(r, same4) : 0.f);
+    return total - ldsb(T, k0) - ldsb(T, k1) + (same4 != HREC_SAME_NONE ? ldsb(r, same4) : 0.f);
 }
 
 __device__ __forceinline__ float4 load_reach4(const TaskArgs& A, const Ctx& c, const NodeTask& nt, const RoundArgs& Rk, int k, int b) {
@@ -447,7 +415,7 @@
         const float* rf = SM_X + (fold_first ? 0 : c.Hx);
         const float* rs = SM_X + (fold_first ? c.Hx : 0);
         float total_f;
-        const float total = scan_reach<HC, true>(c, rs, rf, &total_f);
+        const float total = scan_reach<HC, true>(c, Rk, rs, rf, &total_f);
         const float cf = nt.child[a_fold].coef * scale, cs = nt.child[a_sd].coef * scale;
         const float c0 = fold_first ? cf : cs, c1 = fold_first ? cs : cf;
         staged_recs_wait();
@@ -459,7 +427,7 @@
                 if (uint32_t(c.pos4 + i) < nl_p) {
                     float m_sd, sd;
                     hand_terms<HC>(c, rs, total, rec[i], m_sd, sd);
-                    const float m = hand_mass(SM_BF, rf, total_f, rec[i]);
+                    const float m = hand_mass(SM_TF, rf, total_f, rec[i]);
                     const float t0 = fold_first ? m : sd, t1 = fold_first ? sd : m;
                     f4set(acc, i, f4get(acc, i) + c0 * t0);
                     f4set(acc, i, f4get(acc, i) + c1 * t1);
@@ -474,7 +442,7 @@
             const float* r = SM_X + slot * c.Hx;
             ++slot;
             const float cf = nt.child[a].coef * scale;
-            const float total = scan_reach<HC, false>(c, r);
+            const float total = scan_reach<HC, false>(c, Rk, r);
             staged_recs_wait();
             if (c.pos4 < c.HpP) {
                 uint4 rec[4];
@@ -484,7 +452,7 @@
                     if (uint32_t(c.pos4 + i) < nl_p) {
                         float m, sd;
                         if (ck == CK_FOLD) {
-                            m = hand_mass(SM_B, r, total, rec[i]);
+                            m = hand_mass(SM_T, r, total, rec[i]);
                             f4set(acc, i, f4get(acc, i) + cf * m);
                         } else {
                             hand_terms<HC>(c, r, total, rec[i], m, sd);
@@ -504,7 +472,7 @@
     const uint32_t nrp = O.n_rows_pad[b];
     const float* __restrict__ slab = (MODE == KM_CFR ? O.regrets : O.ssum) + O.board_off[b] + size_t(nrp) * nt.cum_a;
     if (nt.out >= 0) {
-        stage_lists_raw<HC>(c.tid, c.HoP, O.cl_pos + size_t(b) * 2 * c.HoP);
+        stage_lists_raw<HC>(c.tid, Rk.cl_len, O.cl_pos + size_t(b) * Rk.cl_len);
         stage_recs<HC>(c, reinterpret_cast<const uint32_t*>(Rk.rp[c.p].hrec) + size_t(b) * 4 * c.HpP);
     }
     const float4 r4 = load_reach4(A, c, nt, Rk, k, b);
@@ -580,7 +548,7 @@
         }
     }
     if (nt.out < 0) return;
-    stage_lists_raw<HC>(c.tid, c.HoP, O.cl_pos + size_t(b) * 2 * c.HoP);
+    stage_lists_raw<HC>(c.tid, Rk.cl_len, O.cl_pos + size_t(b) * Rk.cl_len);
     stage_recs<HC>(c, reinterpret_cast<const uint32_t*>(Rk.rp[c.p].hrec) + size_t(b) * 4 * c.HpP);
     down_terminals<HC>(c, nt, Rk, b, n_act);
 }
@@ -589,11 +557,11 @@
 __device__ __forceinline__ void trav_terms(const TaskArgs& A, const Ctx& c, const NodeTask& nt, const RoundArgs& Rk, int k, int b,
                                            bool need_sd, float4& mass, float4& sd) {
     const DevRoundPlayer& Pp = Rk.rp[c.p];
-    stage_lists_raw<HC>(c.tid, c.HoP, Rk.rp[c.o].cl_pos + size_t(b) * 2 * c.HoP);
+    stage_lists_raw<HC>(c.tid, Rk.cl_len, Rk.rp[c.o].cl_pos + size_t(b) * Rk.cl_len);
     stage_recs<HC>(c, reinterpret_cast<const uint32_t*>(Pp.hrec) + size_t(b) * 4 * c.HpP);
     const float4 r4 = load_reach4(A, c, nt, Rk, k, b);
     if (c.pos4 < c.HoP) *reinterpret_cast<float4*>(SM_RS + c.pos4) = r4;
-    const float total = scan_reach<HC, false>(c, SM_RS);
+    const float total = scan_reach<HC, false>(c, Rk, SM_RS);
     mass = f4zero();
     sd = f4zero();
     const uint32_t nl_p = Pp.n_live[b];
@@ -606,7 +574,7 @@
             if (uint32_t(c.pos4 + i) < nl_p) {
                 float m, s = 0.f;
                 if (need_sd) hand_terms<HC>(c, SM_RS, total, rec[i], m, s);
-                else m = hand_mass(SM_B, SM_RS, total, rec[i]);
+                else m = hand_mass(SM_T, SM_RS, total, rec[i]);
                 f4set(mass, i, m);
                 f4set(sd, i, s);
             }
@@ -901,7 +869,7 @@
     const int NC = blockDim.x - 32;
     const int tid = threadIdx.x;
     if (tid == 0) mbar_init(&s_done, uint32_t(NC >> 5));
-    if (tid < 2) SM_B[54 + tid] = SM_BF[54 + tid] = 0.f;
+    if (tid == 0) SM_T[54] = SM_TF[54] = 0.f;
     __syncthreads();
 
     if (tid >= NC) {
diff --git a/rustsolver_b200/csrc/kernels.cuh b/rustsolver_b200/csrc/kernels.cuh
--- a/rustsolver_b200/csrc/kernels.cuh
+++ b/rustsolver_b200/csrc/kernels.cuh
@@ -11,6 +11,7 @@
 constexpr int RS_MAX_PEERS = 8;
 constexpr int FAST_ACTIONS = 4;
 constexpr int MAX_TASK_THREADS = 352;
+constexpr int CL_PITCH_PAD = 2;
 
 enum KernelMode { KM_CFR = 0, KM_BR = 1, KM_EVAL = 2, KM_CFR_XS = 3, KM_CFR_DR = 4, KM_CFR_XS_DR = 5 };
 
@@ -53,6 +54,8 @@
     int per_parent;
     int n_boards_next;
     int board_base;
+    int cl_stride;
+    int cl_len;
 };
 
 struct TaskArgs {
diff --git a/rustsolver_b200/solver.py b/rustsolver_b200/solver.py
--- a/rustsolver_b200/solver.py
+++ b/rustsolver_b200/solver.py
@@ -466,6 +466,15 @@
         sop = np.zeros(hp, dtype=np.uint16)
         check(self._lib.rs_plan_local_tables(self._h, round_idx, player, board_id, _ptr(rec, u32p), _ptr(cl, u16p), _ptr(sop, u16p), dims))
         return rec, cl, sop, nl
+
+    def device_lists(self, round_idx: int, player: int, board_id: int):
+        dims = (C.c_uint32 * 4)()
+        check(self._lib.rs_plan_device_lists(self._h, round_idx, player, board_id, None, None, 0, dims))
+        hp, stride, slots, pitch = int(dims[0]), int(dims[1]), int(dims[2]), int(dims[3])
+        rec = np.zeros((hp, 4), dtype=np.uint32)
+        cl = np.zeros(max(slots * stride, 1), dtype=np.uint16)
+        check(self._lib.rs_plan_device_lists(self._h, round_idx, player, board_id, _ptr(rec, u32p), _ptr(cl, u16p), len(cl), dims))
+        return rec, cl[:slots * stride], stride, slots, pitch
 
     def street_info(self, traverser: int) -> dict:
         out = (C.c_uint32 * 8)()
```

Result: faster. 22.16 (median of 6 runs) (+1.8%).
